# Pointcept/Pointcept

Measured on AMD Instinct MI355X. Metric: scenes/sec (fwd+bwd+optimizer) PTv3 ScanNet-semseg @ ~100k pts, higher is better.
Workload: dtype bf16; 1 GPU; PT-v3m1 base (46.2M params) + seg head + CE + Lovasz, fwd+bwd+AdamW, 8 scenes x 102400 voxels per GPU, patch 1024, 4 orders; global_batch=8, parallelism=dp1, params=46167572, amp=bf16 autocast, points_per_gpu=819200, loss=CrossEntropy(ignore_index=-1) + LovaszSoftmax

## Files before the change

include/ptcore.h:

```cpp
#ifndef PTCORE_H
#define PTCORE_H

#include <stddef.h>
#include <stdint.h>

#ifdef __cplusplus
extern "C" {
#endif

typedef void* ptc_stream_t;

enum ptc_status {
  PTC_OK = 0,
  PTC_EINVAL = -1,
  PTC_EUNSUPPORTED = -2,
  PTC_EHIP = -3,
  PTC_EWORKSPACE = -4
};

enum ptc_dtype { PTC_F32 = 0, PTC_F16 = 1, PTC_BF16 = 2 };

enum ptc_order { PTC_ORDER_Z = 0, PTC_ORDER_Z_TRANS = 1, PTC_ORDER_HILBERT = 2, PTC_ORDER_HILBERT_TRANS = 3 };

enum ptc_reduce { PTC_REDUCE_SUM = 0, PTC_REDUCE_MEAN = 1, PTC_REDUCE_MAX = 2, PTC_REDUCE_MIN = 3 };

const char* ptc_version(void);
const char* ptc_last_error(void);

int ptc_serialize_encode(const void* grid_coord, int coord_is_i64, const int64_t* batch, int64_t n,
                         int depth, const int* orders, int k, int64_t* code_out, ptc_stream_t stream);

size_t ptc_sort_keys_workspace_bytes(int64_t n, int k);
int ptc_sort_keys(const int64_t* keys, int64_t n, int k, int begin_bit, int end_bit, int64_t* order,
                  int64_t* inverse, void* workspace, size_t workspace_bytes, ptc_stream_t stream);

size_t ptc_exclusive_scan_workspace_bytes(int64_t n);
int ptc_exclusive_scan_i32(const int32_t* in, int64_t n, int64_t* out, void* workspace,
                           size_t workspace_bytes, ptc_stream_t stream);

int ptc_patch_pad_maps(const int64_t* offset, int B, int patch, int64_t n, int64_t n_pad,
                       int64_t n_seq, int64_t* pad, int64_t* unpad, int32_t* cu_seqlens,
                       int64_t* dup, ptc_stream_t stream);

int ptc_attn_tables(const int64_t* order, const int64_t* inverse, const int64_t* pad, const int64_t* unpad,
                    const int64_t* dup, int64_t n, int64_t n_pad, int32_t* t_qkv_fwd, int32_t* t_qkv_bwd,
                    int32_t* t_proj_fwd, int32_t* t_proj_bwd, ptc_stream_t stream);

size_t ptc_pool_maps_workspace_bytes(int64_t n);
int ptc_pool_maps_count(const int64_t* code0, const int64_t* order0, int64_t n, int shift,
                        int64_t* cluster, int64_t* n_cluster_out, void* workspace,
                        size_t workspace_bytes, ptc_stream_t stream);
int ptc_pool_maps_fill(const int64_t* order0, const int64_t* cluster, int64_t n, int64_t n_cluster,
                       int64_t* idx_ptr, int64_t* head, ptc_stream_t stream);
int ptc_pool_child_codes(const int64_t* code_in, int64_t n, int k, const int64_t* head,
                         int64_t n_cluster, int shift, int64_t* code_out, ptc_stream_t stream);

int ptc_pool_level_counts(const int64_t* code0, const int64_t* order0, int64_t n, int batch_shift, int n_batch,
                          const int* shifts, int n_levels, int64_t* counts, ptc_stream_t stream);

int ptc_gather_rows(const void* src, int64_t n_src, const int64_t* idx, const int64_t* idx2,
                    int64_t n_out, int c, int dtype, void* out, ptc_stream_t stream);
int ptc_gather_rows_add(const void* src, int64_t n_src, const int64_t* idx, const void* addend, int64_t n_out, int c, int dtype,
                        void* out, ptc_stream_t stream);
int ptc_segment_csr_fwd(const void* src, const int64_t* perm, const int64_t* indptr, int64_t n_seg,
                        int c, int dtype, int reduce, void* out, int32_t* arg_out,
                        ptc_stream_t stream);
int ptc_segment_csr_bwd(const void* grad_out, const int64_t* perm, const int64_t* indptr,
                        const int32_t* arg, int64_t n_seg, int64_t n_src, int c, int dtype,
                        int reduce, void* grad_src, ptc_stream_t stream);

int64_t ptc_hash_table_size(int64_t n);
size_t ptc_hash_table_bytes(int64_t n);
int ptc_hash_build(const int32_t* indices, int64_t n, void* table, size_t table_bytes, ptc_stream_t stream);
int ptc_rulebook_subm(const int32_t* indices, int64_t n, int ksize, const void* table, size_t table_bytes,
                      int32_t* nbr, ptc_stream_t stream);
size_t ptc_rulebook_down_workspace_bytes(int64_t n_in);
int ptc_rulebook_down_count(const int32_t* indices, int64_t n_in, int coord_bits, int batch_bits,
                            int32_t* out_of_in, int64_t* n_out_dev, void* workspace,
                            size_t workspace_bytes, ptc_stream_t stream);
int ptc_rulebook_down_fill(const int32_t* indices, int64_t n_in, const int32_t* out_of_in,
                           int64_t n_out, int32_t* out_indices, int32_t* nbr_down, int32_t* nbr_up,
                           ptc_stream_t stream);

int ptc_spconv_fwd(const void* in, int64_t n_in, const void* weight, const float* bias,
                   const int32_t* nbr, int64_t n_out, int kv, int c_in, int c_out, int dtype,
                   void* out, ptc_stream_t stream);
size_t ptc_rulebook_blocks_tab_bytes(int64_t n);
int ptc_rulebook_blocks(const int32_t* nbr, int kv, int64_t n, int bm, int hcap, void* tab, int32_t* hid,
                        int32_t* hcnt, int32_t* n_overflow, ptc_stream_t stream);
int ptc_spconv_fwd_blk(const void* in, int64_t n_in, const void* weight, const float* bias, const int32_t* nbr,
                       const void* tab, const int32_t* hid, const int32_t* hcnt, int bm, int hcap, int64_t n_out,
                       int kv, int c_in, int c_out, int dtype, void* out, ptc_stream_t stream);
size_t ptc_spconv_wgrad_blk_workspace_bytes(int64_t n_out, int kv, int c_in, int c_out);
int ptc_spconv_wgrad_blk(const void* in, int64_t n_in, const void* dout, const int32_t* nbr, const void* tab, const int32_t* hid,
                         const int32_t* hcnt, const int32_t* n_overflow, int bm, int hcap, int64_t n_out, int kv, int c_in,
                         int c_out, int dtype, float* dw, void* workspace, size_t workspace_bytes, ptc_stream_t stream);
int ptc_linear_supported_ex(int c_in, int c_out, int dtype);
int ptc_linear_fwd_ex(const void* in, int64_t n, const void* weight, const float* bias, int c_in, int c_out, int dtype,
                      int epilogue, const void* aux_in, void* out, void* aux_out, ptc_stream_t stream);
int ptc_linear_joint_supported(int c_in, int c_out, int dtype);
int ptc_linear_norm_joint_fwd(const void* in, int64_t n_in, const void* weight, const float* bias, int64_t n_out, int c_in, int c_out, int dtype,
                              const float* gA, const float* bA, float epsA, const void* a, int a_dtype, const float* gB, const float* bB, float epsB,
                              int normB, void* u_out, float* z, void* y, float* statA, float* statB, ptc_stream_t stream);
int ptc_linear_joint_fwd(const void* in, int64_t n_in, const void* weight, const float* bias, const int32_t* nbr, int64_t n_out, int c_in,
                         int c_out, int dtype, const float* a, const float* row_scale, const float* gB, const float* bB, float epsB,
                         int normB, float* z, void* y, float* statB, ptc_stream_t stream);

int ptc_mlp_supported(int c, int dtype);
int ptc_mlp_fwd(const void* x, int64_t n, int c, int dtype, const void* w1, const float* b1, const void* w2, const float* b2,
                const float* a, const float* row_scale, float* z, void* y, ptc_stream_t stream);
size_t ptc_mlp_bwd_workspace_bytes(int64_t n, int c);
int ptc_mlp_bwd(const void* dm, const void* x, int64_t n, int c, int dtype, const void* w1, const float* b1, const void* w2t, void* dx,
                float* dw1, float* db1, float* dw2, float* db2, void* workspace, size_t workspace_bytes, ptc_stream_t stream);

size_t ptc_spconv_wgrad_workspace_bytes(int64_t n_out, int kv, int c_in, int c_out);
int ptc_spconv_wgrad(const void* in, int64_t n_in, const void* dout, const int32_t* nbr,
                     int64_t n_out, int kv, int c_in, int c_out, int dtype, float* dw, float* dbias,
                     void* workspace, size_t workspace_bytes, ptc_stream_t stream);

int ptc_seg_eval_hist(const void* logits, int dtype, int64_t row_stride, int c, const int64_t* pred, const int64_t* inverse,
                      const int64_t* target, int64_t m, int64_t n_rows, int k, int64_t ignore_index, int64_t* hist3k,
                      ptc_stream_t stream);

int ptc_rope3d(void* tokens, int dtype, const int64_t* positions, int64_t n_tokens, int H, int D, float base, float fwd,
               ptc_stream_t stream);

int ptc_rope3d_xyz(const void* src, int src_dtype, void* dst, int dst_dtype, const float* xyz, const float* inv_freq,
                   int64_t n_tokens, int slabs, int rot_slabs, int H, int D, float sign, ptc_stream_t stream);

int ptc_layer_norm_supported(int c);
int ptc_layer_norm_fwd(const void* x, int64_t n, int c, int in_dtype, const float* gamma,
                       const float* beta, float eps, void* y, int out_dtype, float* mean, float* rstd,
                       ptc_stream_t stream);
size_t ptc_layer_norm_bwd_workspace_bytes(int64_t n, int c);
int ptc_layer_norm_bwd(const void* dy, int dy_dtype, const void* x, int x_dtype, const float* mean,
                       const float* rstd, const float* gamma, int64_t n, int c, void* dx,
                       float* dgamma, float* dbeta, void* workspace, size_t workspace_bytes,
                       ptc_stream_t stream);

int ptc_add_norm_fwd(const void* u, int u_dtype, const void* a, int a_dtype, const float* row_scale, int64_t n, int c,
                     const float* gA, const float* bA, float epsA, int normA, const float* gB,
                     const float* bB, float epsB, int normB, float* z, void* y, int y_dtype,
                     float* statA, float* statB, ptc_stream_t stream);
size_t ptc_add_norm_bwd_workspace_bytes(int64_t n, int c);
int ptc_add_norm_bwd(const float* dz_in, const void* dy, int dy_dtype, const float* z, const void* u,
                     int u_dtype, const float* row_scale, int64_t n, int c, const float* gA,
                     const float* statA, int normA, const float* gB, const float* statB, int normB,
                     void* da, int da_dtype, void* du, float* dgA, float* dbA, float* dgB, float* dbB,
                     void* workspace, size_t workspace_bytes, ptc_stream_t stream);

int ptc_attn_varlen_fwd(const void* qkv, const int32_t* cu_seqlens, int64_t n_seq, int64_t total,
                        int H, int max_seqlen, float softmax_scale, int dtype, void* out,
                        float* lse, ptc_stream_t stream);
size_t ptc_attn_varlen_bwd_workspace_bytes(int64_t total, int H);
int ptc_attn_varlen_bwd(const void* qkv, const void* out, const void* dout, const float* lse,
                        const int32_t* cu_seqlens, int64_t n_seq, int64_t total, int H,
                        int max_seqlen, float softmax_scale, int dtype, void* dqkv,
                        void* workspace, size_t workspace_bytes, ptc_stream_t stream);

int ptc_attn_varlen_dropout_fwd(const void* qkv, const int32_t* cu_seqlens, int64_t n_seq, int64_t total, int H, int max_seqlen,
                                float softmax_scale, int dtype, float dropout_p, uint64_t seed, void* out, float* lse,
                                ptc_stream_t stream);
int ptc_attn_varlen_dropout_bwd(const void* qkv, const void* out, const void* dout, const float* lse, const int32_t* cu_seqlens,
                                int64_t n_seq, int64_t total, int H, int max_seqlen, float softmax_scale, int dtype,
                                float dropout_p, uint64_t seed, void* dqkv, void* workspace, size_t workspace_bytes,
                                ptc_stream_t stream);

int ptc_attn_varlen_hd_supported(int head_dim, int max_seqlen);
int ptc_attn_varlen_hd_fwd(const void* qkv, const int32_t* cu_seqlens, int64_t n_seq, int64_t total,
                           int H, int head_dim, int max_seqlen, float softmax_scale, int dtype,
                           void* out, float* lse, ptc_stream_t stream);
int ptc_attn_varlen_hd_bwd(const void* qkv, const void* out, const void* dout, const float* lse,
                           const int32_t* cu_seqlens, int64_t n_seq, int64_t total, int H,
                           int head_dim, int max_seqlen, float softmax_scale, int dtype, void* dqkv,
                           void* workspace, size_t workspace_bytes, ptc_stream_t stream);
int ptc_attn_varlen_hd_rope_supported(int head_dim, int max_seqlen);
int ptc_attn_varlen_hd_rope_fwd(const void* qkv, const int32_t* cu_seqlens, const float* xyz, const float* inv_freq, int64_t n_seq,
                                int64_t total, int H, int head_dim, int max_seqlen, float softmax_scale, int dtype, void* out, float* lse,
                                ptc_stream_t stream);
int ptc_attn_varlen_hd_rope_bwd(const void* qkv, const void* out, const void* dout, const float* lse, const int32_t* cu_seqlens,
                                const float* xyz, const float* inv_freq, int64_t n_seq, int64_t total, int H, int head_dim, int max_seqlen,
                                float softmax_scale, int dtype, void* dqkv, void* workspace, size_t workspace_bytes, ptc_stream_t stream);


int ptc_attn_rpe_fwd(const void* qkv, const int32_t* cu_seqlens, const int32_t* grid_coord,
                     const float* rpe_table, int pos_bnd, int64_t n_seq, int64_t total, int H,
                     int max_seqlen, float softmax_scale, int dtype, void* out, float* lse,
                     ptc_stream_t stream);
size_t ptc_attn_rpe_bwd_workspace_bytes(int64_t total, int H, int pos_bnd);
int ptc_attn_rpe_bwd(const void* qkv, const void* out, const void* dout, const float* lse,
                     const int32_t* cu_seqlens, const int32_t* grid_coord, const float* rpe_table,
                     int pos_bnd, int64_t n_seq, int64_t total, int H, int max_seqlen,
                     float softmax_scale, int dtype, void* dqkv, float* d_rpe_table, void* workspace,
                     size_t workspace_bytes, ptc_stream_t stream);

int ptc_coord_max(const void* grid_coord, int coord_is_i64, int64_t n, int64_t* out3, ptc_stream_t stream);
int64_t ptc_cross_entropy_partials(int64_t n);
int ptc_cross_entropy_fwd(const void* logits, int64_t row_stride, const int64_t* target, int64_t n, int c, int dtype,
                          int64_t ignore_index, float* lse, float* partial, ptc_stream_t stream);
int ptc_cross_entropy_bwd(const void* logits, int64_t row_stride, const int64_t* target, const float* lse,
                          const float* scale, int64_t n, int c, int dtype, int64_t ignore_index, void* dlogits,
                          int64_t drow_stride, ptc_stream_t stream);

size_t ptc_lovasz_softmax_workspace_bytes(int64_t n, int c);
int ptc_lovasz_softmax(const void* logits, int64_t row_stride, const int64_t* target, int64_t n, int c, int dtype,
                       int64_t ignore_index, float* loss, float* dlogits, void* workspace, size_t workspace_bytes,
                       ptc_stream_t stream);

int ptc_voxel_keys(const float* coord, int64_t n, double grid_size, int64_t* grid_coord, int64_t* min_coord3,
                   int64_t* key, ptc_stream_t stream);

int ptc_knn_query(const float* xyz, const int32_t* offset, const float* new_xyz, const int32_t* new_offset, int b,
                  int64_t n, int64_t m, int nsample, int32_t* idx, float* dist, ptc_stream_t stream);
int ptc_farthest_point_sampling(const float* xyz, const int32_t* offset, const int32_t* new_offset, int b, int64_t n,
                                float* tmp, int32_t* idx, ptc_stream_t stream);
int ptc_ball_query(const float* xyz, const int32_t* offset, const float* new_xyz, const int32_t* new_offset, const int32_t* order,
                   int b, int64_t n, int64_t m, int nsample, float min_radius, float max_radius, int32_t* idx, float* dist2,
                   ptc_stream_t stream);
int ptc_edge_rows_fwd(int mode, const float* src, const float* a, const int32_t* idx, int64_t n_edges, int nsample, int c,
                      int64_t n_src, float* out, int64_t out_stride, int out_col0, ptc_stream_t stream);
int ptc_edge_reduce_fwd(int mode, const float* src, const float* pos, int64_t pos_stride, int pos_col0, const float* w,
                        const int32_t* idx, int64_t m, int nsample, int c, int w_c, int64_t n_src, float* out, ptc_stream_t stream);
int ptc_edge_csr_keys(const int32_t* idx, int64_t n_edges, int64_t n_src, int64_t* keys, ptc_stream_t stream);
int ptc_edge_csr_ptr(const int64_t* keys, const int64_t* order, int64_t n_edges, int64_t n_src, int64_t* indptr, ptc_stream_t stream);
int ptc_edge_scatter_bwd(int mode, const int64_t* order, const int64_t* indptr, const float* g, int64_t g_stride, int g_col0,
                         const float* w, int nsample, int c, int w_c, int64_t n_src, float* grad_src, ptc_stream_t stream);
int ptc_aggregation_edge_bwd(const float* src, const float* pos, const float* w, const int32_t* idx, const float* g, int64_t m,
                             int nsample, int c, int w_c, int64_t n_src, float* grad_pos, float* grad_w, ptc_stream_t stream);
int ptc_pair_dot_weighted(const float* a, const float* b, const float* w, const int32_t* ia, const int32_t* ib, int64_t m, int64_t n_a,
                          int64_t n_b, int g, int c, float* out, ptc_stream_t stream);
int ptc_pair_segment_sum(const float* s, const float* b, const float* w, const float* self, const int64_t* order, const int64_t* indptr,
                         const int32_t* oidx, int64_t n_rows, int64_t n_b, int g, int c, float* out, float* prod, ptc_stream_t stream);

int ptc_batch_norm_supported(int c, int dtype);
size_t ptc_batch_norm_workspace_bytes(int64_t n, int c);
int ptc_batch_norm_act_fwd(const void* x, int64_t n, int c, int dtype, const float* gamma, const float* beta, float eps,
                           float momentum, int training, float* running_mean, float* running_var, int act, void* y,
                           int y_dtype, float* save_mean, float* save_rstd, void* workspace, size_t workspace_bytes,
                           ptc_stream_t stream);
int ptc_column_sum(const void* x, int64_t n, int c, int dtype, float* out, void* workspace, size_t workspace_bytes,
                   ptc_stream_t stream);
int ptc_batch_norm_act_bwd(const void* dy, int dy_dtype, const void* x, int x_dtype, const float* gamma, const float* beta,
                           const float* save_mean, const float* save_rstd, int64_t n, int c, int training, int act,
                           void* dx, float* dgamma, float* dbeta, void* workspace, size_t workspace_bytes,
                           ptc_stream_t stream);
int ptc_batch_norm_add_act_fwd(const void* x, const void* res, int64_t n, int c, int dtype, const float* gamma, const float* beta, float eps,
                               float momentum, int training, float* running_mean, float* running_var, int act, void* y, int y_dtype,
                               float* save_mean, float* save_rstd, void* workspace, size_t workspace_bytes, ptc_stream_t stream);
int ptc_batch_norm_add_act_bwd(const void* dy, int dy_dtype, const void* x, const void* res, int x_dtype, const float* gamma, const float* beta,
                               const float* save_mean, const float* save_rstd, int64_t n, int c, int training, int act, void* dx, void* dres,
                               float* dgamma, float* dbeta, void* workspace, size_t workspace_bytes, ptc_stream_t stream);

int ptc_weight_layouts(const int64_t* desc, const int64_t* prefix, int n, int64_t total, ptc_stream_t stream);

int ptc_cast_many(const int64_t* desc, const int64_t* prefix, int n, int64_t total_units, int dst_dtype, ptc_stream_t stream);

int ptc_pair_dot_fwd(const float* q, const float* k, const int32_t* i0, const int32_t* i1, const float* table_q,
                     const float* table_k, const int32_t* rel_idx, int with_qk, int64_t M, int H, int d, float* out,
                     ptc_stream_t stream);
int ptc_pair_dot_bwd(const float* grad_out, const float* q, const float* k, const int32_t* i0, const int32_t* offsets,
                     const int32_t* i1, const float* table_q, const float* table_k, const int32_t* rel_idx, int with_qk,
                     int64_t M, int64_t Nq, int64_t Nk, int64_t L, int H, int d, float* dq, float* dk, float* dtable_q,
                     float* dtable_k, ptc_stream_t stream);
int ptc_pair_aggregate_fwd(const float* attn, const float* v, const int32_t* i0, const int32_t* offsets, const int32_t* i1,
                           const float* table_v, const int32_t* rel_idx, int64_t M, int64_t Nq, int H, int d, float* out,
                           ptc_stream_t stream);
int ptc_pair_aggregate_bwd(const float* grad_out, const float* attn, const float* v, const int32_t* i0, const int32_t* i1,
                           const float* table_v, const int32_t* rel_idx, int64_t M, int64_t Nv, int64_t L, int H, int d,
                           float* dattn, float* dv, float* dtable_v, ptc_stream_t stream);

#define PTC_BLK_ABI 2
// ... 107 lines not shown
```

pointcept_amd/_lib.py:

```python
from __future__ import annotations

import ctypes
import os

import torch

HERE = os.path.dirname(os.path.abspath(__file__))
LIB_PATH = os.path.join(HERE, "libptcore.so")
PROBE_PATH = os.path.join(HERE, "libptcore_hostprobe.so")

c_i64, c_int, c_f32, c_size, c_ptr = ctypes.c_int64, ctypes.c_int, ctypes.c_float, ctypes.c_size_t, ctypes.c_void_p

_SIGNATURES = {
    "ptc_version": (ctypes.c_char_p, []),
    "ptc_last_error": (ctypes.c_char_p, []),
    "ptc_serialize_encode": (c_int, [c_ptr, c_int, c_ptr, c_i64, c_int, c_ptr, c_int, c_ptr, c_ptr]),
    "ptc_sort_keys_workspace_bytes": (c_size, [c_i64, c_int]),
    "ptc_sort_keys": (c_int, [c_ptr, c_i64, c_int, c_int, c_int, c_ptr, c_ptr, c_ptr, c_size, c_ptr]),
    "ptc_exclusive_scan_workspace_bytes": (c_size, [c_i64]),
    "ptc_exclusive_scan_i32": (c_int, [c_ptr, c_i64, c_ptr, c_ptr, c_size, c_ptr]),
    "ptc_patch_pad_maps": (c_int, [c_ptr, c_int, c_int, c_i64, c_i64, c_i64, c_ptr, c_ptr, c_ptr, c_ptr, c_ptr]),
    "ptc_attn_tables": (c_int, [c_ptr, c_ptr, c_ptr, c_ptr, c_ptr, c_i64, c_i64, c_ptr, c_ptr, c_ptr, c_ptr, c_ptr]),
    "ptc_pool_maps_workspace_bytes": (c_size, [c_i64]),
    "ptc_pool_maps_count": (c_int, [c_ptr, c_ptr, c_i64, c_int, c_ptr, c_ptr, c_ptr, c_size, c_ptr]),
    "ptc_pool_maps_fill": (c_int, [c_ptr, c_ptr, c_i64, c_i64, c_ptr, c_ptr, c_ptr]),
    "ptc_pool_child_codes": (c_int, [c_ptr, c_i64, c_int, c_ptr, c_i64, c_int, c_ptr, c_ptr]),
    "ptc_pool_level_counts": (c_int, [c_ptr, c_ptr, c_i64, c_int, c_int, c_ptr, c_int, c_ptr, c_ptr]),
    "ptc_gather_rows": (c_int, [c_ptr, c_i64, c_ptr, c_ptr, c_i64, c_int, c_int, c_ptr, c_ptr]),
    "ptc_gather_rows_add": (c_int, [c_ptr, c_i64, c_ptr, c_ptr, c_i64, c_int, c_int, c_ptr, c_ptr]),
    "ptc_segment_csr_fwd": (c_int, [c_ptr, c_ptr, c_ptr, c_i64, c_int, c_int, c_int, c_ptr, c_ptr, c_ptr]),
    "ptc_segment_csr_bwd": (c_int, [c_ptr, c_ptr, c_ptr, c_ptr, c_i64, c_i64, c_int, c_int, c_int, c_ptr, c_ptr]),
    "ptc_hash_table_size": (c_i64, [c_i64]),
    "ptc_hash_table_bytes": (c_size, [c_i64]),
    "ptc_hash_build": (c_int, [c_ptr, c_i64, c_ptr, c_size, c_ptr]),
    "ptc_rulebook_subm": (c_int, [c_ptr, c_i64, c_int, c_ptr, c_size, c_ptr, c_ptr]),
    "ptc_rulebook_down_workspace_bytes": (c_size, [c_i64]),
    "ptc_rulebook_down_count": (c_int, [c_ptr, c_i64, c_int, c_int, c_ptr, c_ptr, c_ptr, c_size, c_ptr]),
    "ptc_rulebook_down_fill": (c_int, [c_ptr, c_i64, c_ptr, c_i64, c_ptr, c_ptr, c_ptr, c_ptr]),
    "ptc_spconv_fwd": (c_int, [c_ptr, c_i64, c_ptr, c_ptr, c_ptr, c_i64, c_int, c_int, c_int, c_int, c_ptr, c_ptr]),
    "ptc_ptv3_block_abi": (c_int, []),
    "ptc_ptv3_block_mlp_fused": (c_int, [c_int, c_int]),
    "ptc_ptv3_block_workspace_bytes": (c_size, [c_i64, c_i64, c_int, c_int]),
    "ptc_ptv3_block_fwd": (c_int, [c_ptr, c_ptr, c_ptr, c_ptr, c_ptr]),
    "ptc_ptv3_block_bwd": (c_int, [c_ptr, c_ptr, c_ptr, c_ptr, c_ptr, c_ptr, c_size, c_ptr]),
    "ptc_rulebook_blocks_tab_bytes": (c_size, [c_i64]),
    "ptc_rulebook_blocks": (c_int, [c_ptr, c_int, c_i64, c_int, c_int, c_ptr, c_ptr, c_ptr, c_ptr, c_ptr]),
    "ptc_spconv_fwd_blk": (c_int, [c_ptr, c_i64, c_ptr, c_ptr, c_ptr, c_ptr, c_ptr, c_ptr, c_int, c_int, c_i64, c_int, c_int, c_int, c_int,
                                   c_ptr, c_ptr]),
    "ptc_spconv_wgrad_blk_workspace_bytes": (c_size, [c_i64, c_int, c_int, c_int]),
    "ptc_spconv_wgrad_blk": (c_int, [c_ptr, c_i64, c_ptr, c_ptr, c_ptr, c_ptr, c_ptr, c_ptr, c_int, c_int, c_i64, c_int, c_int, c_int, c_int,
                                     c_ptr, c_ptr, c_size, c_ptr]),
    "ptc_linear_supported_ex": (c_int, [c_int, c_int, c_int]),
    "ptc_linear_joint_supported": (c_int, [c_int, c_int, c_int]),
    "ptc_linear_norm_joint_fwd": (c_int, [c_ptr, c_i64, c_ptr, c_ptr, c_i64, c_int, c_int, c_int, c_ptr, c_ptr, c_f32, c_ptr, c_int, c_ptr, c_ptr, c_f32, c_int,
                                          c_ptr, c_ptr, c_ptr, c_ptr, c_ptr, c_ptr]),
    "ptc_linear_joint_fwd": (c_int, [c_ptr, c_i64, c_ptr, c_ptr, c_ptr, c_i64, c_int, c_int, c_int, c_ptr, c_ptr, c_ptr, c_ptr, c_f32, c_int,
                                     c_ptr, c_ptr, c_ptr, c_ptr]),
    "ptc_linear_fwd_ex": (c_int, [c_ptr, c_i64, c_ptr, c_ptr, c_int, c_int, c_int, c_int, c_ptr, c_ptr, c_ptr, c_ptr]),
    "ptc_mlp_supported": (c_int, [c_int, c_int]),
    "ptc_mlp_fwd": (c_int, [c_ptr, c_i64, c_int, c_int, c_ptr, c_ptr, c_ptr, c_ptr, c_ptr, c_ptr, c_ptr, c_ptr, c_ptr]),
    "ptc_mlp_bwd_workspace_bytes": (c_size, [c_i64, c_int]),
    "ptc_mlp_bwd": (c_int, [c_ptr, c_ptr, c_i64, c_int, c_int, c_ptr, c_ptr, c_ptr, c_ptr, c_ptr, c_ptr, c_ptr, c_ptr, c_ptr, c_size, c_ptr]),
    "ptc_spconv_wgrad_workspace_bytes": (c_size, [c_i64, c_int, c_int, c_int]),
    "ptc_spconv_wgrad": (c_int, [c_ptr, c_i64, c_ptr, c_ptr, c_i64, c_int, c_int, c_int, c_int, c_ptr, c_ptr, c_ptr, c_size,
                                 c_ptr]),
    "ptc_seg_eval_hist": (c_int, [c_ptr, c_int, c_i64, c_int, c_ptr, c_ptr, c_ptr, c_i64, c_i64, c_int, c_i64, c_ptr, c_ptr]),
    "ptc_rope3d": (c_int, [c_ptr, c_int, c_ptr, c_i64, c_int, c_int, c_f32, c_f32, c_ptr]),
    "ptc_rope3d_xyz": (c_int, [c_ptr, c_int, c_ptr, c_int, c_ptr, c_ptr, c_i64, c_int, c_int, c_int, c_int, c_f32, c_ptr]),
    "ptc_layer_norm_supported": (c_int, [c_int]),
    "ptc_layer_norm_fwd": (c_int, [c_ptr, c_i64, c_int, c_int, c_ptr, c_ptr, c_f32, c_ptr, c_int, c_ptr, c_ptr, c_ptr]),
    "ptc_layer_norm_bwd_workspace_bytes": (c_size, [c_i64, c_int]),
    "ptc_layer_norm_bwd": (c_int, [c_ptr, c_int, c_ptr, c_int, c_ptr, c_ptr, c_ptr, c_i64, c_int, c_ptr, c_ptr, c_ptr, c_ptr,
                                   c_size, c_ptr]),
    "ptc_add_norm_fwd": (c_int, [c_ptr, c_int, c_ptr, c_int, c_ptr, c_i64, c_int, c_ptr, c_ptr, c_f32, c_int, c_ptr, c_ptr, c_f32, c_int,
                                 c_ptr, c_ptr, c_int, c_ptr, c_ptr, c_ptr]),
    "ptc_add_norm_bwd_workspace_bytes": (c_size, [c_i64, c_int]),
    "ptc_add_norm_bwd": (c_int, [c_ptr, c_ptr, c_int, c_ptr, c_ptr, c_int, c_ptr, c_i64, c_int, c_ptr, c_ptr, c_int, c_ptr, c_ptr,
                                 c_int, c_ptr, c_int, c_ptr, c_ptr, c_ptr, c_ptr, c_ptr, c_ptr, c_size, c_ptr]),
    "ptc_attn_varlen_fwd": (c_int, [c_ptr, c_ptr, c_i64, c_i64, c_int, c_int, c_f32, c_int, c_ptr, c_ptr, c_ptr]),
    "ptc_attn_varlen_bwd_workspace_bytes": (c_size, [c_i64, c_int]),
    "ptc_attn_varlen_dropout_fwd": (c_int, [c_ptr, c_ptr, c_i64, c_i64, c_int, c_int, c_f32, c_int, c_f32, ctypes.c_uint64, c_ptr, c_ptr, c_ptr]),
    "ptc_attn_varlen_dropout_bwd": (c_int, [c_ptr, c_ptr, c_ptr, c_ptr, c_ptr, c_i64, c_i64, c_int, c_int, c_f32, c_int, c_f32, ctypes.c_uint64,
                                            c_ptr, c_ptr, c_size, c_ptr]),
    "ptc_attn_varlen_hd_supported": (c_int, [c_int, c_int]),
    "ptc_attn_varlen_hd_rope_supported": (c_int, [c_int, c_int]),
    "ptc_attn_varlen_hd_rope_fwd": (c_int, [c_ptr, c_ptr, c_ptr, c_ptr, c_i64, c_i64, c_int, c_int, c_int, c_f32, c_int, c_ptr, c_ptr, c_ptr]),
    "ptc_attn_varlen_hd_rope_bwd": (c_int, [c_ptr, c_ptr, c_ptr, c_ptr, c_ptr, c_ptr, c_ptr, c_i64, c_i64, c_int, c_int, c_int, c_f32, c_int, c_ptr,
                                            c_ptr, c_size, c_ptr]),
    "ptc_weight_layouts": (c_int, [c_ptr, c_ptr, c_int, c_i64, c_ptr]),
    "ptc_cast_many": (c_int, [c_ptr, c_ptr, c_int, c_i64, c_int, c_ptr]),
    "ptc_pair_dot_fwd": (c_int, [c_ptr, c_ptr, c_ptr, c_ptr, c_ptr, c_ptr, c_ptr, c_int, c_i64, c_int, c_int, c_ptr, c_ptr]),
    "ptc_pair_dot_bwd": (c_int, [c_ptr, c_ptr, c_ptr, c_ptr, c_ptr, c_ptr, c_ptr, c_ptr, c_ptr, c_int, c_i64, c_i64, c_i64, c_i64, c_int,
                                 c_int, c_ptr, c_ptr, c_ptr, c_ptr, c_ptr]),
    "ptc_pair_aggregate_fwd": (c_int, [c_ptr, c_ptr, c_ptr, c_ptr, c_ptr, c_ptr, c_ptr, c_i64, c_i64, c_int, c_int, c_ptr, c_ptr]),
    "ptc_pair_aggregate_bwd": (c_int, [c_ptr, c_ptr, c_ptr, c_ptr, c_ptr, c_ptr, c_ptr, c_i64, c_i64, c_i64, c_int, c_int, c_ptr, c_ptr,
                                       c_ptr, c_ptr]),
    "ptc_attn_rpe_fwd": (c_int, [c_ptr, c_ptr, c_ptr, c_ptr, c_int, c_i64, c_i64, c_int, c_int, c_f32, c_int, c_ptr, c_ptr, c_ptr]),
    "ptc_attn_rpe_bwd_workspace_bytes": (c_size, [c_i64, c_int, c_int]),
    "ptc_attn_rpe_bwd": (c_int, [c_ptr, c_ptr, c_ptr, c_ptr, c_ptr, c_ptr, c_ptr, c_int, c_i64, c_i64, c_int, c_int, c_f32, c_int, c_ptr,
                                 c_ptr, c_ptr, c_size, c_ptr]),
    "ptc_attn_varlen_hd_fwd": (c_int, [c_ptr, c_ptr, c_i64, c_i64, c_int, c_int, c_int, c_f32, c_int, c_ptr, c_ptr, c_ptr]),
    "ptc_attn_varlen_hd_bwd": (c_int, [c_ptr, c_ptr, c_ptr, c_ptr, c_ptr, c_i64, c_i64, c_int, c_int, c_int, c_f32, c_int, c_ptr,
                                       c_ptr, c_size, c_ptr]),
    "ptc_attn_varlen_bwd": (c_int, [c_ptr, c_ptr, c_ptr, c_ptr, c_ptr, c_i64, c_i64, c_int, c_int, c_f32, c_int, c_ptr,
                                    c_ptr, c_size, c_ptr]),
    "ptc_batch_norm_supported": (c_int, [c_int, c_int]),
    "ptc_batch_norm_workspace_bytes": (c_size, [c_i64, c_int]),
    "ptc_batch_norm_act_fwd": (c_int, [c_ptr, c_i64, c_int, c_int, c_ptr, c_ptr, c_f32, c_f32, c_int, c_ptr, c_ptr, c_int, c_ptr, c_int,
                                       c_ptr, c_ptr, c_ptr, c_size, c_ptr]),
    "ptc_batch_norm_act_bwd": (c_int, [c_ptr, c_int, c_ptr, c_int, c_ptr, c_ptr, c_ptr, c_ptr, c_i64, c_int, c_int, c_int, c_ptr, c_ptr,
                                       c_ptr, c_ptr, c_size, c_ptr]),
    "ptc_batch_norm_add_act_fwd": (c_int, [c_ptr, c_ptr, c_i64, c_int, c_int, c_ptr, c_ptr, c_f32, c_f32, c_int, c_ptr, c_ptr, c_int, c_ptr, c_int,
                                           c_ptr, c_ptr, c_ptr, c_size, c_ptr]),
    "ptc_batch_norm_add_act_bwd": (c_int, [c_ptr, c_int, c_ptr, c_ptr, c_int, c_ptr, c_ptr, c_ptr, c_ptr, c_i64, c_int, c_int, c_int, c_ptr, c_ptr,
                                           c_ptr, c_ptr, c_ptr, c_size, c_ptr]),
    "ptc_column_sum": (c_int, [c_ptr, c_i64, c_int, c_int, c_ptr, c_ptr, c_size, c_ptr]),
    "ptc_coord_max": (c_int, [c_ptr, c_int, c_i64, c_ptr, c_ptr]),
    "ptc_cross_entropy_partials": (c_i64, [c_i64]),
    "ptc_cross_entropy_fwd": (c_int, [c_ptr, c_i64, c_ptr, c_i64, c_int, c_int, c_i64, c_ptr, c_ptr, c_ptr]),
    "ptc_cross_entropy_bwd": (c_int, [c_ptr, c_i64, c_ptr, c_ptr, c_ptr, c_i64, c_int, c_int, c_i64, c_ptr, c_i64, c_ptr]),
    "ptc_knn_query": (c_int, [c_ptr, c_ptr, c_ptr, c_ptr, c_int, c_i64, c_i64, c_int, c_ptr, c_ptr, c_ptr]),
    "ptc_ball_query": (c_int, [c_ptr, c_ptr, c_ptr, c_ptr, c_ptr, c_int, c_i64, c_i64, c_int, c_f32, c_f32, c_ptr, c_ptr, c_ptr]),
    "ptc_edge_rows_fwd": (c_int, [c_int, c_ptr, c_ptr, c_ptr, c_i64, c_int, c_int, c_i64, c_ptr, c_i64, c_int, c_ptr]),
    "ptc_edge_reduce_fwd": (c_int, [c_int, c_ptr, c_ptr, c_i64, c_int, c_ptr, c_ptr, c_i64, c_int, c_int, c_int, c_i64, c_ptr, c_ptr]),
    "ptc_edge_csr_keys": (c_int, [c_ptr, c_i64, c_i64, c_ptr, c_ptr]),
    "ptc_edge_csr_ptr": (c_int, [c_ptr, c_ptr, c_i64, c_i64, c_ptr, c_ptr]),
    "ptc_edge_scatter_bwd": (c_int, [c_int, c_ptr, c_ptr, c_ptr, c_i64, c_int, c_ptr, c_int, c_int, c_int, c_i64, c_ptr, c_ptr]),
    "ptc_pair_dot_weighted": (c_int, [c_ptr, c_ptr, c_ptr, c_ptr, c_ptr, c_i64, c_i64, c_i64, c_int, c_int, c_ptr, c_ptr]),
    "ptc_pair_segment_sum": (c_int, [c_ptr, c_ptr, c_ptr, c_ptr, c_ptr, c_ptr, c_ptr, c_i64, c_i64, c_int, c_int, c_ptr, c_ptr, c_ptr]),
    "ptc_aggregation_edge_bwd": (c_int, [c_ptr, c_ptr, c_ptr, c_ptr, c_ptr, c_i64, c_int, c_int, c_int, c_i64, c_ptr, c_ptr, c_ptr]),
    "ptc_farthest_point_sampling": (c_int, [c_ptr, c_ptr, c_ptr, c_int, c_i64, c_ptr, c_ptr, c_ptr]),
    "ptc_voxel_keys": (c_int, [c_ptr, c_i64, ctypes.c_double, c_ptr, c_ptr, c_ptr, c_ptr]),
    "ptc_grid_cluster_workspace_bytes": (c_size, [c_i64, c_int]),
    "ptc_grid_cluster_count": (c_int, [c_ptr, c_i64, c_ptr, c_int, c_ptr, c_int, c_ptr, c_ptr, c_ptr, c_ptr, c_size, c_ptr]),
    "ptc_cluster_center": (c_int, [c_ptr, c_ptr, c_ptr, c_ptr, c_int, c_i64, c_int, c_int, c_ptr, c_ptr]),
    "ptc_cluster_agg_state_bytes": (c_size, [c_i64, c_int]),
    "ptc_cluster_agg_workspace_bytes": (c_size, [c_i64]),
    "ptc_cluster_agg_fwd": (c_int, [c_ptr, c_ptr, c_ptr, c_ptr, c_ptr, c_ptr, c_ptr, c_int, c_i64, c_int, c_int, c_ptr, c_ptr, c_size,
                                    c_ptr]),
    "ptc_cluster_agg_bwd": (c_int, [c_ptr, c_ptr, c_ptr, c_ptr, c_ptr, c_ptr, c_ptr, c_ptr, c_int, c_i64, c_int, c_int, c_ptr, c_size,
                                    c_ptr, c_ptr, c_ptr, c_ptr, c_size, c_ptr]),
    "ptc_pg_ball_query_workspace_bytes": (c_size, [c_i64]),
    "ptc_pg_ball_query_count": (c_int, [c_ptr, c_ptr, c_i64, c_int, c_f32, c_ptr, c_ptr, c_ptr, c_size, c_ptr]),
    "ptc_pg_ball_query_fill": (c_int, [c_ptr, c_i64, c_f32, c_ptr, c_ptr, c_ptr, c_size, c_ptr]),
    "ptc_pg_cluster_workspace_bytes": (c_size, [c_i64]),
    "ptc_pg_cluster_count": (c_int, [c_ptr, c_ptr, c_ptr, c_i64, c_int, c_int, c_ptr, c_ptr, c_size, c_ptr]),
    "ptc_pg_cluster_fill": (c_int, [c_i64, c_i64, c_i64, c_ptr, c_ptr, c_ptr, c_size, c_ptr]),
    "ptc_pg_proposal_scores": (c_int, [c_ptr, c_int, c_i64, c_int, c_ptr, c_ptr, c_ptr, c_i64, c_ptr, c_ptr, c_ptr, c_ptr, c_ptr]),
    "ptc_pg_proposal_masks": (c_int, [c_ptr, c_i64, c_ptr, c_ptr, c_i64, c_i64, c_ptr, c_ptr]),
    "ptc_pg_bias_loss_workspace_bytes": (c_size, [c_i64]),
    "ptc_pg_bias_loss_fwd": (c_int, [c_ptr, c_int, c_ptr, c_ptr, c_ptr, c_i64, c_i64, c_ptr, c_ptr, c_size, c_ptr]),
    "ptc_pg_bias_loss_bwd": (c_int, [c_ptr, c_int, c_ptr, c_ptr, c_ptr, c_i64, c_i64, c_ptr, c_ptr, c_ptr, c_ptr]),
    "ptc_msc_match_workspace_bytes": (c_size, [c_i64]),
    "ptc_msc_match": (c_int, [c_ptr, c_ptr, c_ptr, c_ptr, c_int, c_i64, c_i64, c_int, c_f32, c_ptr, c_ptr, c_ptr, c_ptr, c_size, c_ptr]),
    "ptc_msc_select_workspace_bytes": (c_size, [c_i64]),
    "ptc_msc_select": (c_int, [c_ptr, c_ptr, c_i64, c_int, c_ptr, c_i64, c_ptr, c_ptr, c_size, c_ptr]),
    "ptc_msc_patch_workspace_bytes": (c_size, [c_i64]),
    "ptc_msc_patch_rank": (c_int, [c_ptr, c_ptr, c_i64, c_ptr, c_ptr, c_i64, c_int, c_ptr, c_ptr, c_ptr, c_size, c_ptr]),
    "ptc_msc_patch_masks": (c_int, [c_ptr, c_ptr, c_i64, c_i64, c_i64, c_ptr, c_ptr, c_ptr]),
    "ptc_msc_nce_workspace_bytes": (c_size, [c_i64, c_int]),
    "ptc_msc_nce_fwd": (c_int, [c_ptr, c_i64, c_ptr, c_i64, c_ptr, c_i64, c_int, c_f32, c_ptr, c_ptr, c_ptr, c_ptr, c_ptr, c_ptr, c_ptr,
                                c_size, c_ptr]),
    "ptc_msc_nce_bwd": (c_int, [c_ptr, c_ptr, c_ptr, c_ptr, c_ptr, c_ptr, c_i64, c_int, c_i64, c_i64, c_f32, c_ptr, c_ptr, c_ptr, c_ptr,
                                c_size, c_ptr]),
    "ptc_cac_supported": (c_int, [c_int, c_int]),
    "ptc_cac_pool_workspace_bytes": (c_size, [c_i64, c_int, c_int, c_int]),
    "ptc_cac_pool_fwd": (c_int, [c_ptr, c_ptr, c_ptr, c_ptr, c_i64, c_int, c_int, c_int, c_f32, c_f32, c_ptr, c_ptr, c_ptr, c_ptr, c_ptr, c_size,
                                 c_ptr]),
    "ptc_cac_pool_bwd": (c_int, [c_ptr, c_ptr, c_ptr, c_ptr, c_i64, c_int, c_int, c_int, c_f32, c_f32, c_ptr, c_ptr, c_ptr, c_ptr, c_ptr, c_ptr]),
    "ptc_cac_cos_workspace_bytes": (c_size, [c_i64, c_int, c_int, c_int]),
    "ptc_cac_cos_fwd": (c_int, [c_ptr, c_ptr, c_ptr, c_i64, c_int, c_int, c_int, c_f32, c_ptr, c_ptr, c_size, c_ptr]),
    "ptc_cac_cos_bwd": (c_int, [c_ptr, c_ptr, c_ptr, c_i64, c_int, c_int, c_int, c_f32, c_ptr, c_ptr, c_ptr, c_ptr, c_size, c_ptr]),
    "ptc_cac_distill_workspace_bytes": (c_size, [c_i64, c_int]),
    "ptc_cac_distill_fwd": (c_int, [c_ptr, c_ptr, c_ptr, c_i64, c_int, c_f32, c_f32, c_ptr, c_ptr, c_ptr, c_size, c_ptr]),
    "ptc_cac_distill_bwd": (c_int, [c_ptr, c_ptr, c_ptr, c_i64, c_int, c_f32, c_f32, c_ptr, c_ptr, c_ptr, c_ptr]),
    "ptc_lovasz_softmax_workspace_bytes": (c_size, [c_i64, c_int]),
    "ptc_lovasz_softmax": (c_int, [c_ptr, c_i64, c_ptr, c_i64, c_int, c_int, c_i64, c_ptr, c_ptr, c_ptr, c_size, c_ptr]),
}

PTC_F32, PTC_F16, PTC_BF16 = 0, 1, 2
REDUCE_CODES = {"sum": 0, "mean": 1, "max": 2, "min": 3}
ORDER_CODES = {"z": 0, "z-trans": 1, "hilbert": 2, "hilbert-trans": 3}

_lib = None


class PtcoreError(RuntimeError):
    pass


def exported_symbols():
    return sorted(_SIGNATURES)


def lib():
    global _lib
    if _lib is not None:
        return _lib
    from . import build as _build

    variant = os.environ.get("PTC_LIB_VARIANT", "")
    LIB_PATH = _build.build(variant=variant)
    try:
        L = ctypes.CDLL(LIB_PATH)
    except OSError as e:
        raise PtcoreError(f"cannot load {LIB_PATH}: {e}") from e
    for name, (res, args) in _SIGNATURES.items():
        fn = getattr(L, name)
        fn.restype = res
        fn.argtypes = args
    ver = L.ptc_version().decode()
    hdr = os.path.join(HERE, "..", "include", "ptcore.h")
    if os.path.exists(hdr) and "abi " in ver:
        import zlib

        want = f"{zlib.crc32(open(hdr, 'rb').read()) & 0xffffffff:08x}"
# ... 85 lines not shown
```

pointcept_amd/csrc/block_exec.hip:

```cpp
#include "ptc_common.h"
#ifndef PTC_BLK_JOINT_EPILOGUE
#define PTC_BLK_JOINT_EPILOGUE 1
#endif
#include "spconv_internal.h"

#define RUN(call)               \
  do {                          \
    const int rc__ = (call);    \
    if (rc__ != PTC_OK) return rc__; \
  } while (0)

static inline const void* P(const void* const* p, int i) { return p[i]; }
template <typename T> static inline T* M(void* const* p, int i) { return (T*)p[i]; }

extern "C" int ptc_ptv3_block_abi(void) { return PTC_BLK_ABI; }

extern "C" int ptc_ptv3_block_mlp_fused(int c, int dtype) {
  static const int off = [] { const char* e = getenv("PTC_BLK_MLP_FUSED"); return e && e[0] == '0'; }();
  return !off && ptc_mlp_supported(c, dtype);
}

struct BlkWs { size_t common; size_t wg[6]; size_t off[6]; size_t total; };
static BlkWs blk_ws(int64_t n, int64_t n_pad, int c, int heads) {
  const int hid = 4 * c;
  BlkWs w;
  w.common = 256;
  auto up = [&](size_t v) { if (v > w.common) w.common = v; };
  up(ptc_add_norm_bwd_workspace_bytes(n, c));
  up(ptc_attn_varlen_bwd_workspace_bytes(n_pad, heads));
  up(ptc_batch_norm_workspace_bytes(n, c));
  w.common = ptc_align_up(w.common, 256);
  w.wg[0] = ptc_spconv_wgrad_workspace_bytes(n, 1, hid, c);
  if (ptc_mlp_supported(c, PTC_BF16) && ptc_mlp_bwd_workspace_bytes(n, c) > w.wg[0]) w.wg[0] = ptc_mlp_bwd_workspace_bytes(n, c);
  w.wg[1] = ptc_spconv_wgrad_workspace_bytes(n, 1, c, hid);
  w.wg[2] = ptc_spconv_wgrad_workspace_bytes(n, 1, c, c);
  w.wg[3] = ptc_spconv_wgrad_workspace_bytes(n_pad, 1, c, 3 * c);
  w.wg[4] = ptc_spconv_wgrad_workspace_bytes(n, 1, c, c);
  w.wg[5] = ptc_spconv_wgrad_blk_workspace_bytes(n, 27, c, c);
  size_t o = w.common;
  for (int i = 0; i < 6; ++i) { w.off[i] = o; o += ptc_align_up(w.wg[i], 256); }
  w.total = o;
  return w;
}

extern "C" size_t ptc_ptv3_block_workspace_bytes(int64_t n, int64_t n_pad, int c, int heads) { return blk_ws(n, n_pad, c, heads).total; }

extern "C" int ptc_ptv3_block_fwd(const int64_t* iv, const float* fv, const void* const* in, void* const* out, ptc_stream_t s) {
  PTC_REQUIRE(iv && fv && in && out, PTC_EINVAL, "ptc_ptv3_block_fwd: null argument table");
  PTC_REQUIRE(iv[PTC_BLK_I_ABI] == PTC_BLK_ABI, PTC_EINVAL, "ptc_ptv3_block_fwd: argument tables of another ABI revision");
  const int64_t n = iv[PTC_BLK_I_N], np = iv[PTC_BLK_I_NPAD], n_seq = iv[PTC_BLK_I_NSEQ];
  const int c = (int)iv[PTC_BLK_I_C], H = (int)iv[PTC_BLK_I_HEADS], dt = (int)iv[PTC_BLK_I_DTYPE], hid = 4 * c;
  const int a_dt = (int)iv[PTC_BLK_I_A_DTYPE], patch = (int)iv[PTC_BLK_I_PATCH];
  PTC_REQUIRE(dt == PTC_BF16 || dt == PTC_F16, PTC_EUNSUPPORTED, "ptc_ptv3_block_fwd: 16-bit GEMM operands only");
  PTC_REQUIRE(c % 16 == 0 && H * 16 == c && (c <= 256 || (c <= 512 && ptc_linear_supported_ex(c, hid, dt))), PTC_EUNSUPPORTED,
              "ptc_ptv3_block_fwd: c=%d heads=%d (head_dim 16, c <= 256, or <= 512 with the wide GEMM kernels)", c, H);
  if (n == 0) return PTC_OK;
  const int32_t* nbr = (const int32_t*)P(in, PTC_BLK_P_NBR);
  RUN(ptc_spconv_fwd_blk(P(in, PTC_BLK_P_XC), n, P(in, PTC_BLK_P_W_CONV), (const float*)P(in, PTC_BLK_P_B_CONV), nbr, P(in, PTC_BLK_P_BLK_TAB),
                         (const int32_t*)P(in, PTC_BLK_P_BLK_HID), (const int32_t*)P(in, PTC_BLK_P_BLK_HCNT), (int)iv[PTC_BLK_I_BLK_BM],
                         (int)iv[PTC_BLK_I_BLK_HCAP], n, 27, c, c, dt, out[PTC_BLK_O_CONV], s));
  if (PTC_BLK_JOINT_EPILOGUE && ptc_linear_joint_supported(c, c, dt)) {
    RUN(ptc_linear_norm_joint_fwd(out[PTC_BLK_O_CONV], n, P(in, PTC_BLK_P_W_LIN), (const float*)P(in, PTC_BLK_P_B_LIN), n, c, c, dt,
                                  (const float*)P(in, PTC_BLK_P_G_CPE), (const float*)P(in, PTC_BLK_P_BE_CPE), fv[PTC_BLK_F_EPS_CPE], P(in, PTC_BLK_P_X0), a_dt,
                                  (const float*)P(in, PTC_BLK_P_G_N1), (const float*)P(in, PTC_BLK_P_BE_N1), fv[PTC_BLK_F_EPS_N1], 1, out[PTC_BLK_O_LIN],
                                  M<float>(out, PTC_BLK_O_X1), out[PTC_BLK_O_Y1], M<float>(out, PTC_BLK_O_ST_CPE), M<float>(out, PTC_BLK_O_ST_N1), s));
  } else {
  RUN(ptc_spconv_fwd(out[PTC_BLK_O_CONV], n, P(in, PTC_BLK_P_W_LIN), (const float*)P(in, PTC_BLK_P_B_LIN), nullptr, n, 1, c, c, dt, out[PTC_BLK_O_LIN], s));
  RUN(ptc_add_norm_fwd(out[PTC_BLK_O_LIN], dt, P(in, PTC_BLK_P_X0), a_dt, nullptr, n, c, (const float*)P(in, PTC_BLK_P_G_CPE),
                       (const float*)P(in, PTC_BLK_P_BE_CPE), fv[PTC_BLK_F_EPS_CPE], 1, (const float*)P(in, PTC_BLK_P_G_N1),
                       (const float*)P(in, PTC_BLK_P_BE_N1), fv[PTC_BLK_F_EPS_N1], 1, M<float>(out, PTC_BLK_O_X1), out[PTC_BLK_O_Y1], dt,
                       M<float>(out, PTC_BLK_O_ST_CPE), M<float>(out, PTC_BLK_O_ST_N1), s));
  }
  RUN(ptc_spconv_fwd(out[PTC_BLK_O_Y1], n, P(in, PTC_BLK_P_W_QKV), (const float*)P(in, PTC_BLK_P_B_QKV), (const int32_t*)P(in, PTC_BLK_P_T_QKV_FWD), np, 1, c,
                     3 * c, dt, out[PTC_BLK_O_QKV], s));
  RUN(ptc_attn_varlen_fwd(out[PTC_BLK_O_QKV], (const int32_t*)P(in, PTC_BLK_P_CU), n_seq, np, H, patch, fv[PTC_BLK_F_SCALE], dt, out[PTC_BLK_O_ATT],
                          M<float>(out, PTC_BLK_O_LSE), s));
  if (PTC_BLK_JOINT_EPILOGUE && ptc_linear_joint_supported(c, c, dt)) {
    RUN(ptc_linear_joint_fwd(out[PTC_BLK_O_ATT], np, P(in, PTC_BLK_P_W_PROJ), (const float*)P(in, PTC_BLK_P_B_PROJ), (const int32_t*)P(in, PTC_BLK_P_T_PROJ_FWD),
                             n, c, c, dt, M<float>(out, PTC_BLK_O_X1), (const float*)P(in, PTC_BLK_P_RS1), (const float*)P(in, PTC_BLK_P_G_N2),
                             (const float*)P(in, PTC_BLK_P_BE_N2), fv[PTC_BLK_F_EPS_N2], 1, M<float>(out, PTC_BLK_O_X2), out[PTC_BLK_O_Y2],
                             M<float>(out, PTC_BLK_O_ST_N2), s));
  } else {
    RUN(ptc_spconv_fwd(out[PTC_BLK_O_ATT], np, P(in, PTC_BLK_P_W_PROJ), (const float*)P(in, PTC_BLK_P_B_PROJ), (const int32_t*)P(in, PTC_BLK_P_T_PROJ_FWD), n, 1,
                       c, c, dt, out[PTC_BLK_O_A], s));
    RUN(ptc_add_norm_fwd(out[PTC_BLK_O_A], dt, out[PTC_BLK_O_X1], PTC_F32, (const float*)P(in, PTC_BLK_P_RS1), n, c, nullptr, nullptr, 0.f, 0,
                         (const float*)P(in, PTC_BLK_P_G_N2), (const float*)P(in, PTC_BLK_P_BE_N2), fv[PTC_BLK_F_EPS_N2], 1, M<float>(out, PTC_BLK_O_X2),
                         out[PTC_BLK_O_Y2], dt, nullptr, M<float>(out, PTC_BLK_O_ST_N2), s));
  }
  if (ptc_ptv3_block_mlp_fused(c, dt))
    return ptc_mlp_fwd(out[PTC_BLK_O_Y2], n, c, dt, P(in, PTC_BLK_P_W_FC1), (const float*)P(in, PTC_BLK_P_B_FC1), P(in, PTC_BLK_P_W_FC2),
                       (const float*)P(in, PTC_BLK_P_B_FC2), M<float>(out, PTC_BLK_O_X2), (const float*)P(in, PTC_BLK_P_RS2), M<float>(out, PTC_BLK_O_X3),
                       out[PTC_BLK_O_XB3], s);
  RUN(ptc_linear_fwd_ex(out[PTC_BLK_O_Y2], n, P(in, PTC_BLK_P_W_FC1), (const float*)P(in, PTC_BLK_P_B_FC1), c, hid, dt, 1, nullptr, out[PTC_BLK_O_H],
                        out[PTC_BLK_O_ACT], s));
  if (PTC_BLK_JOINT_EPILOGUE && ptc_linear_joint_supported(hid, c, dt)) {
    RUN(ptc_linear_joint_fwd(out[PTC_BLK_O_ACT], n, P(in, PTC_BLK_P_W_FC2), (const float*)P(in, PTC_BLK_P_B_FC2), nullptr, n, hid, c, dt,
                             M<float>(out, PTC_BLK_O_X2), (const float*)P(in, PTC_BLK_P_RS2), nullptr, nullptr, 0.f, 0, M<float>(out, PTC_BLK_O_X3),
                             out[PTC_BLK_O_XB3], nullptr, s));
  } else {
    RUN(ptc_spconv_fwd(out[PTC_BLK_O_ACT], n, P(in, PTC_BLK_P_W_FC2), (const float*)P(in, PTC_BLK_P_B_FC2), nullptr, n, 1, hid, c, dt, out[PTC_BLK_O_M], s));
    RUN(ptc_add_norm_fwd(out[PTC_BLK_O_M], dt, out[PTC_BLK_O_X2], PTC_F32, (const float*)P(in, PTC_BLK_P_RS2), n, c, nullptr, nullptr, 0.f, 0, nullptr,
                         nullptr, 0.f, 0, M<float>(out, PTC_BLK_O_X3), out[PTC_BLK_O_XB3], dt, nullptr, nullptr, s));
  }
  return PTC_OK;
}

extern "C" int ptc_ptv3_block_bwd(const int64_t* iv, const float* fv, const void* const* in, const void* const* sv, void* const* g,
                                  void* workspace, size_t workspace_bytes, ptc_stream_t s) {
  PTC_REQUIRE(iv && fv && in && sv && g && workspace, PTC_EINVAL, "ptc_ptv3_block_bwd: null argument table");
  PTC_REQUIRE(iv[PTC_BLK_I_ABI] == PTC_BLK_ABI, PTC_EINVAL, "ptc_ptv3_block_bwd: argument tables of another ABI revision");
  const int64_t n = iv[PTC_BLK_I_N], np = iv[PTC_BLK_I_NPAD], n_seq = iv[PTC_BLK_I_NSEQ];
  const int c = (int)iv[PTC_BLK_I_C], H = (int)iv[PTC_BLK_I_HEADS], dt = (int)iv[PTC_BLK_I_DTYPE], hid = 4 * c;
  const int a_dt = (int)iv[PTC_BLK_I_A_DTYPE], patch = (int)iv[PTC_BLK_I_PATCH];
  PTC_REQUIRE(workspace_bytes >= ptc_ptv3_block_workspace_bytes(n, np, c, H), PTC_EWORKSPACE, "ptc_ptv3_block_bwd: workspace too small");
  if (n == 0) return PTC_OK;
  const int32_t* nbr = (const int32_t*)P(in, PTC_BLK_P_NBR);
  const float* rs1 = (const float*)P(in, PTC_BLK_P_RS1);
  const float* rs2 = (const float*)P(in, PTC_BLK_P_RS2);
  const BlkWs W = blk_ws(n, np, c, H);
  void* ws = workspace;
  const size_t wb = W.common;
  PtcWgradJob jobs[6];
  PtcWgradCall calls[5];
  auto wgws = [&](int i) { return (void*)((char*)workspace + W.off[i]); };
  RUN(ptc_add_norm_bwd((const float*)P(in, PTC_BLK_P_DZ3), P(in, PTC_BLK_P_DYB3), dt, (const float*)P(sv, PTC_BLK_O_X3), P(sv, PTC_BLK_O_M), dt, rs2, n, c,
                       nullptr, nullptr, 0, nullptr, nullptr, 0, g[PTC_BLK_S_DX2], PTC_F32, g[PTC_BLK_S_DM], nullptr, nullptr, nullptr, nullptr, ws, wb, s));
  const bool mlp_fused = ptc_ptv3_block_mlp_fused(c, dt) != 0;
  if (mlp_fused) {
    RUN(ptc_mlp_bwd_deferred(g[PTC_BLK_S_DM], P(sv, PTC_BLK_O_Y2), n, c, dt, P(in, PTC_BLK_P_W_FC1), (const float*)P(in, PTC_BLK_P_B_FC1),
                             P(in, PTC_BLK_P_WT_FC2), g[PTC_BLK_S_DY2], M<float>(g, PTC_BLK_G_W_FC1), M<float>(g, PTC_BLK_G_B_FC1),
                             M<float>(g, PTC_BLK_G_W_FC2), M<float>(g, PTC_BLK_G_B_FC2), wgws(0), W.wg[0], s, &jobs[1], &jobs[0]));
  } else {
  calls[0] = PtcWgradCall{P(sv, PTC_BLK_O_ACT), n, g[PTC_BLK_S_DM], nullptr, n, 1, hid, c, dt, M<float>(g, PTC_BLK_G_W_FC2), M<float>(g, PTC_BLK_G_B_FC2), wgws(0), W.wg[0]};
  RUN(ptc_linear_fwd_ex(g[PTC_BLK_S_DM], n, P(in, PTC_BLK_P_WT_FC2), nullptr, c, hid, dt, 2, P(sv, PTC_BLK_O_H), g[PTC_BLK_S_DH], nullptr, s));
  calls[1] = PtcWgradCall{P(sv, PTC_BLK_O_Y2), n, g[PTC_BLK_S_DH], nullptr, n, 1, c, hid, dt, M<float>(g, PTC_BLK_G_W_FC1), M<float>(g, PTC_BLK_G_B_FC1), wgws(1), W.wg[1]};
  RUN(ptc_spconv_fwd(g[PTC_BLK_S_DH], n, P(in, PTC_BLK_P_WT_FC1), nullptr, nullptr, n, 1, hid, c, dt, g[PTC_BLK_S_DY2], s));
  }
  RUN(ptc_add_norm_bwd(M<float>(g, PTC_BLK_S_DX2), g[PTC_BLK_S_DY2], dt, (const float*)P(sv, PTC_BLK_O_X2), P(sv, PTC_BLK_O_A), dt, rs1, n, c, nullptr, nullptr, 0,
                       (const float*)P(in, PTC_BLK_P_G_N2), (const float*)P(sv, PTC_BLK_O_ST_N2), 1, g[PTC_BLK_S_DX1], PTC_F32, g[PTC_BLK_S_DA], nullptr, nullptr,
                       M<float>(g, PTC_BLK_G_G_N2), M<float>(g, PTC_BLK_G_BE_N2), ws, wb, s));
  calls[2] = PtcWgradCall{P(sv, PTC_BLK_O_ATT), np, g[PTC_BLK_S_DA], (const int32_t*)P(in, PTC_BLK_P_T_PROJ_FWD), n, 1, c, c, dt, M<float>(g, PTC_BLK_G_W_PROJ),
                          M<float>(g, PTC_BLK_G_B_PROJ), wgws(2), W.wg[2]};
  RUN(ptc_spconv_fwd(g[PTC_BLK_S_DA], n, P(in, PTC_BLK_P_WT_PROJ), nullptr, (const int32_t*)P(in, PTC_BLK_P_T_PROJ_BWD), np, 1, c, c, dt, g[PTC_BLK_S_DATT], s));
  RUN(ptc_attn_varlen_bwd(P(sv, PTC_BLK_O_QKV), P(sv, PTC_BLK_O_ATT), g[PTC_BLK_S_DATT], (const float*)P(sv, PTC_BLK_O_LSE), (const int32_t*)P(in, PTC_BLK_P_CU), n_seq,
                          np, H, patch, fv[PTC_BLK_F_SCALE], dt, g[PTC_BLK_S_DQKV], ws, wb, s));
  calls[3] = PtcWgradCall{P(sv, PTC_BLK_O_Y1), n, g[PTC_BLK_S_DQKV], (const int32_t*)P(in, PTC_BLK_P_T_QKV_FWD), np, 1, c, 3 * c, dt, M<float>(g, PTC_BLK_G_W_QKV),
                          M<float>(g, PTC_BLK_G_B_QKV), wgws(3), W.wg[3]};
  RUN(ptc_spconv_fwd(g[PTC_BLK_S_DQKV], np, P(in, PTC_BLK_P_WT_QKV), nullptr, (const int32_t*)P(in, PTC_BLK_P_T_QKV_BWD), n, 2, 3 * c, c, dt, g[PTC_BLK_S_DY1], s));
  RUN(ptc_add_norm_bwd(M<float>(g, PTC_BLK_S_DX1), g[PTC_BLK_S_DY1], dt, (const float*)P(sv, PTC_BLK_O_X1), P(sv, PTC_BLK_O_LIN), dt, nullptr, n, c,
                       (const float*)P(in, PTC_BLK_P_G_CPE), (const float*)P(sv, PTC_BLK_O_ST_CPE), 1, (const float*)P(in, PTC_BLK_P_G_N1),
                       (const float*)P(sv, PTC_BLK_O_ST_N1), 1, g[PTC_BLK_G_X0], a_dt, g[PTC_BLK_S_DLIN], M<float>(g, PTC_BLK_G_G_CPE), M<float>(g, PTC_BLK_G_BE_CPE),
                       M<float>(g, PTC_BLK_G_G_N1), M<float>(g, PTC_BLK_G_BE_N1), ws, wb, s));
  calls[4] = PtcWgradCall{P(sv, PTC_BLK_O_CONV), n, g[PTC_BLK_S_DLIN], nullptr, n, 1, c, c, dt, M<float>(g, PTC_BLK_G_W_LIN), M<float>(g, PTC_BLK_G_B_LIN), wgws(4), W.wg[4]};
  RUN(ptc_spconv_fwd(g[PTC_BLK_S_DLIN], n, P(in, PTC_BLK_P_WT_LIN), nullptr, nullptr, n, 1, c, c, dt, g[PTC_BLK_S_DCONV], s));
  RUN(ptc_spconv_wgrad_blk_deferred(P(in, PTC_BLK_P_XC), n, g[PTC_BLK_S_DCONV], nbr, P(in, PTC_BLK_P_BLK_TAB), (const int32_t*)P(in, PTC_BLK_P_BLK_HID),
                                    (const int32_t*)P(in, PTC_BLK_P_BLK_HCNT), (const int32_t*)P(in, PTC_BLK_P_BLK_NOVF), (int)iv[PTC_BLK_I_BLK_BM],
                                    (int)iv[PTC_BLK_I_BLK_HCAP], n, 27, c, c, dt, M<float>(g, PTC_BLK_G_W_CONV), wgws(5), W.wg[5], s, &jobs[5]));
  RUN(ptc_column_sum(g[PTC_BLK_S_DCONV], n, c, dt, M<float>(g, PTC_BLK_G_B_CONV), ws, wb, s));
  RUN(ptc_spconv_fwd_blk(g[PTC_BLK_S_DCONV], n, P(in, PTC_BLK_P_WT_CONV), nullptr, nbr, P(in, PTC_BLK_P_BLK_TAB), (const int32_t*)P(in, PTC_BLK_P_BLK_HID),
                         (const int32_t*)P(in, PTC_BLK_P_BLK_HCNT), (int)iv[PTC_BLK_I_BLK_BM], (int)iv[PTC_BLK_I_BLK_HCAP], n, 27, c, c, dt, g[PTC_BLK_G_XC], s));
  if (mlp_fused) RUN(ptc_spconv_wgrad_group(calls + 2, 3, jobs + 2, s));
  else RUN(ptc_spconv_wgrad_group(calls, 5, jobs, s));
  RUN(ptc_wgrad_reduce_jobs(jobs, 6, s));
  return PTC_OK;
}
```

pointcept_amd/csrc/spconv.hip:

```cpp
#include "ptc_common.h"
#include "spconv_internal.h"

#include "mma.h"
#include "wgrad2.h"

#define SC_ROWS 128
#define SC_LDS_BYTES 34816

template <int NTILES> struct TileGroups {
  static __host__ __device__ constexpr int gsize(int t) { return (NTILES - (t & ~3)) >= 4 ? 4 : (((NTILES & 3) - ((t & 3) & ~1)) >= 2 ? 2 : 1); }
  static __host__ __device__ constexpr int gstart(int t) { return (NTILES - (t & ~3)) >= 4 ? (t & ~3) : (((NTILES & 3) - ((t & 3) & ~1)) >= 2 ? ((t & ~3) + ((t & 3) & ~1)) : t); }
};

template <int NTILES>
__device__ __forceinline__ int lds_row_of_channel(int n) {
  const int t0 = n >> 4;
  const int gs = TileGroups<NTILES>::gstart(t0), G = TileGroups<NTILES>::gsize(t0);
  const int local = n - 16 * gs;
  const int gq = local / (4 * G), rem = local - gq * 4 * G;
  const int tt = rem >> 2, e = rem & 3;
  return 16 * (gs + tt) + 4 * gq + e;
}

template <int NTILES>
// ... 243 lines not shown
}
extern "C" int ptc_linear_norm_joint_fwd(const void* in, int64_t n_in, const void* weight, const float* bias, int64_t n_out, int c_in, int c_out, int dtype,
                                         const float* gA, const float* bA, float epsA, const void* a, int a_dtype, const float* gB, const float* bB, float epsB,
                                         int normB, void* u_out, float* z, void* y, float* statA, float* statB, ptc_stream_t stream) {
  PTC_REQUIRE(n_out == 0 || (u_out && statA), PTC_EINVAL, "ptc_linear_norm_joint_fwd: null buffer");
  PTC_REQUIRE((uintptr_t)u_out % 16 == 0, PTC_EINVAL, "ptc_linear_norm_joint_fwd: buffers must be 16-byte aligned");
  PTC_REQUIRE(a_dtype == PTC_F32 || a_dtype == PTC_BF16 || a_dtype == PTC_F16, PTC_EINVAL, "ptc_linear_norm_joint_fwd: a_dtype %d", a_dtype);
  const F2Joint J{(const float*)a, nullptr, gB, bB, epsB, normB, z, y, statB, gA, bA, epsA, 1, statA, u_out, a_dtype == PTC_BF16 ? 1 : (a_dtype == PTC_F16 ? 2 : 0)};
  return linear_joint_impl(in, n_in, weight, bias, nullptr, n_out, c_in, c_out, dtype, J, stream);
}
static int linear_joint_impl(const void* in, int64_t n_in, const void* weight, const float* bias, const int32_t* nbr, int64_t n_out, int c_in, int c_out,
                             int dtype, const F2Joint& J, ptc_stream_t stream) {
  const float* a = J.a;
  float* z = J.z;
  void* y = J.y;
  const int normB = J.normB;
  float* statB = J.statB;
  PTC_REQUIRE(n_out >= 0 && n_in >= 0 && linear_joint_supported(dtype, c_in, c_out), PTC_EUNSUPPORTED,
              "ptc_linear_joint_fwd: c_in=%d c_out=%d dtype=%d", c_in, c_out, dtype);
  PTC_REQUIRE((uint64_t)n_in * (uint64_t)c_in * 2 <= PTC_BUF_MAX_BYTES, PTC_EUNSUPPORTED, "ptc_linear_joint_fwd: input of 2 GiB or more");
  if (n_out == 0) return PTC_OK;
  PTC_REQUIRE(in && weight && a && z, PTC_EINVAL, "ptc_linear_joint_fwd: null buffer");
  PTC_REQUIRE(!(normB && y) || statB, PTC_EINVAL, "ptc_linear_joint_fwd: missing statistics buffer");
  PTC_REQUIRE(((uintptr_t)in % 16 == 0) && ((uintptr_t)weight % 16 == 0) && ((uintptr_t)a % 16 == 0) && ((uintptr_t)z % 16 == 0) &&
              ((uintptr_t)y % 16 == 0), PTC_EINVAL, "ptc_linear_joint_fwd: buffers must be 16-byte aligned");
  hipStream_t s = (hipStream_t)stream;
#define LJ_DISPATCH(T)                                                                             \
  if (c_out == 32) return launch_linear_joint<T, 2>(in, n_in, weight, bias, nbr, n_out, c_in, J, s);  \
  if (c_out == 64) return launch_linear_joint<T, 4>(in, n_in, weight, bias, nbr, n_out, c_in, J, s);  \
  return launch_linear_joint<T, 8>(in, n_in, weight, bias, nbr, n_out, c_in, J, s);
  if (dtype == PTC_BF16) { LJ_DISPATCH(bf16_t) }
  LJ_DISPATCH(f16_t)
#undef LJ_DISPATCH
}

#define WG_RO 64
#define WG_CT 64

template <typename T>
__global__ void __launch_bounds__(256)
spconv_wgrad_kernel(const T* __restrict__ in, const T* __restrict__ dout, const int32_t* __restrict__ nbr,
                    int64_t n_out, int kv, int c_in, int c_out, int64_t rows_per_split, int ci_tiles,
                    float* __restrict__ partial, float* __restrict__ bias_partial) {
  using M = Mma<T>;
  constexpr int EPL = M::EPL, KS = M::KS;
  constexpr int PITCH = WG_RO + EPL;
  __shared__ __attribute__((aligned(16))) unsigned char smem[2 * WG_CT * (WG_RO + 8) * 4];
  T* dT = reinterpret_cast<T*>(smem);
  T* iT = dT + WG_CT * PITCH;

  const int lane = ptc_lane(), wave = threadIdx.x >> 6;
  const int r = lane & 15, g = lane >> 4;
  const int k = blockIdx.y;
  const int co0 = (blockIdx.z / ci_tiles) * WG_CT, ci0 = (blockIdx.z % ci_tiles) * WG_CT;
  const int64_t begin = (int64_t)blockIdx.x * rows_per_split;
  int64_t end = begin + rows_per_split;
  if (end > n_out) end = n_out;

  f32x4 acc[4];
#pragma unroll
  for (int t = 0; t < 4; ++t) acc[t] = (f32x4){0.f, 0.f, 0.f, 0.f};
  const bool do_bias = bias_partial != nullptr && k == 0 && (blockIdx.z % ci_tiles) == 0;
  f32x4 acc_b = (f32x4){0.f, 0.f, 0.f, 0.f};
  typename M::frag ones;
#pragma unroll
  for (int e = 0; e < EPL; ++e) {
    if (sizeof(T) == 4) reinterpret_cast<float*>(&ones)[e] = 1.0f;
    else if (std::is_same<T, bf16_t>::value) reinterpret_cast<uint16_t*>(&ones)[e] = 0x3F80;
    else reinterpret_cast<uint16_t*>(&ones)[e] = 0x3C00;
  }

  for (int64_t chunk = begin; chunk < end; chunk += WG_RO) {
    __syncthreads();
    if (sizeof(T) == 2) {
      const int p = threadIdx.x & 31, cv = threadIdx.x >> 5;
      const int64_t ra = chunk + 2 * p, rb = ra + 1;
      uint4 da = {0, 0, 0, 0}, db = {0, 0, 0, 0}, xa = {0, 0, 0, 0}, xb = {0, 0, 0, 0};
      const bool cov = (co0 + cv * 8) < c_out, civ = (ci0 + cv * 8) < c_in;
      if (ra < end) {
        if (cov) da = *reinterpret_cast<const uint4*>(dout + ra * c_out + co0 + cv * 8);
        const int32_t j = nbr ? nbr[(int64_t)k * n_out + ra] : (int32_t)ra;
        if (civ && j >= 0) xa = *reinterpret_cast<const uint4*>(in + (int64_t)j * c_in + ci0 + cv * 8);
      }
      if (rb < end) {
        if (cov) db = *reinterpret_cast<const uint4*>(dout + rb * c_out + co0 + cv * 8);
        const int32_t j = nbr ? nbr[(int64_t)k * n_out + rb] : (int32_t)rb;
        if (civ && j >= 0) xb = *reinterpret_cast<const uint4*>(in + (int64_t)j * c_in + ci0 + cv * 8);
      }
      const uint16_t* pa = reinterpret_cast<const uint16_t*>(&da);
      const uint16_t* pb = reinterpret_cast<const uint16_t*>(&db);
      const uint16_t* qa = reinterpret_cast<const uint16_t*>(&xa);
      const uint16_t* qb = reinterpret_cast<const uint16_t*>(&xb);
      uint32_t* d32 = reinterpret_cast<uint32_t*>(dT);
      uint32_t* i32 = reinterpret_cast<uint32_t*>(iT);
#pragma unroll
      for (int e = 0; e < 8; ++e) {
        d32[((cv * 8 + e) * PITCH) / 2 + p] = (uint32_t)pa[e] | ((uint32_t)pb[e] << 16);
        i32[((cv * 8 + e) * PITCH) / 2 + p] = (uint32_t)qa[e] | ((uint32_t)qb[e] << 16);
      }
    } else {
      const int rr = threadIdx.x & 63;
      const int64_t row = chunk + rr;
      const int32_t j = row < end ? (nbr ? nbr[(int64_t)k * n_out + row] : (int32_t)row) : -1;
#pragma unroll
      for (int pass = 0; pass < 4; ++pass) {
        const int cv = (threadIdx.x >> 6) + pass * 4;
        float4 d = {0.f, 0.f, 0.f, 0.f}, x = {0.f, 0.f, 0.f, 0.f};
        if (row < end && (co0 + cv * 4) < c_out)
          d = *reinterpret_cast<const float4*>(reinterpret_cast<const float*>(dout) + row * c_out + co0 + cv * 4);
        if (j >= 0 && (ci0 + cv * 4) < c_in)
          x = *reinterpret_cast<const float4*>(reinterpret_cast<const float*>(in) + (int64_t)j * c_in + ci0 + cv * 4);
        float* df = reinterpret_cast<float*>(dT);
        float* xf = reinterpret_cast<float*>(iT);
        df[(cv * 4 + 0) * PITCH + rr] = d.x; df[(cv * 4 + 1) * PITCH + rr] = d.y;
        df[(cv * 4 + 2) * PITCH + rr] = d.z; df[(cv * 4 + 3) * PITCH + rr] = d.w;
        xf[(cv * 4 + 0) * PITCH + rr] = x.x; xf[(cv * 4 + 1) * PITCH + rr] = x.y;
        xf[(cv * 4 + 2) * PITCH + rr] = x.z; xf[(cv * 4 + 3) * PITCH + rr] = x.w;
      }
    }
    __syncthreads();
#pragma unroll
    for (int ks = 0; ks < WG_RO / KS; ++ks) {
      const int kk = ks * KS + g * EPL;
      const typename M::frag fa = ld_frag<T>(dT + (wave * 16 + r) * PITCH + kk);
      if (do_bias) acc_b = M::mma(fa, ones, acc_b);
#pragma unroll
      for (int t = 0; t < 4; ++t) {
        const typename M::frag fb = ld_frag<T>(iT + (t * 16 + r) * PITCH + kk);
        acc[t] = M::mma(fa, fb, acc[t]);
      }
    }
  }
  if (do_bias && r == 0) {
#pragma unroll
    for (int e = 0; e < 4; ++e) {
      const int co = co0 + wave * 16 + g * 4 + e;
      if (co < c_out) bias_partial[(int64_t)blockIdx.x * c_out + co] = acc_b[e];
    }
  }
  float* pout = partial + (int64_t)blockIdx.x * c_out * kv * c_in;
#pragma unroll
  for (int t = 0; t < 4; ++t) {
    const int ci = ci0 + t * 16 + r;
    if (ci >= c_in) continue;
#pragma unroll
    for (int e = 0; e < 4; ++e) {
      const int co = co0 + wave * 16 + g * 4 + e;
      if (co < c_out) pout[((int64_t)co * kv + k) * c_in + ci] = acc[t][e];
    }
  }
}

#define WG_REDUCE_FEW 8
__device__ __forceinline__ void wgrad_reduce_body(const float* __restrict__ partial, int splits, int64_t count, float* __restrict__ dw, int nb1,
                                                  const float* __restrict__ partial2, int64_t count2, float* __restrict__ out2, int bid, bool few) {
  __shared__ float4 red[16][16];
  if (few && bid < nb1) {
    const int64_t i = (int64_t)bid * 1024 + (int64_t)threadIdx.x * 4;
    if (i >= count) return;
    if ((i + 3 < count) && ((count & 3) == 0)) {
      float4 a = *reinterpret_cast<const float4*>(partial + i);
      for (int p = 1; p < splits; ++p) {
        const float4 v = *reinterpret_cast<const float4*>(partial + (int64_t)p * count + i);
        a.x += v.x; a.y += v.y; a.z += v.z; a.w += v.w;
      }
      *reinterpret_cast<float4*>(dw + i) = a;
    } else {
      for (int64_t j = i; j < count && j < i + 4; ++j) {
        float a = partial[j];
        for (int p = 1; p < splits; ++p) a += partial[(int64_t)p * count + j];
        dw[j] = a;
      }
    }
    return;
  }
  if (bid >= nb1) {
    partial = partial2; count = count2; dw = out2;
  }
  const int64_t blk = bid >= nb1 ? (int64_t)bid - nb1 : (int64_t)bid;
  const int lane = threadIdx.x & 15, pg = threadIdx.x >> 4;
  const int64_t i = blk * 64 + lane * 4;
  float4 acc[4];
#pragma unroll
  for (int u = 0; u < 4; ++u) acc[u] = make_float4(0.f, 0.f, 0.f, 0.f);
  if (i < count) {
    const bool vec = (i + 3 < count) && ((count & 3) == 0);
    for (int p0 = pg; p0 < splits; p0 += 64) {
      if (vec) {
        float4 v[4];
#pragma unroll
        for (int u = 0; u < 4; ++u) {
          const int p = p0 + 16 * u;
          v[u] = *reinterpret_cast<const float4*>(partial + (int64_t)(p < splits ? p : splits - 1) * count + i);
        }
#pragma unroll
        for (int u = 0; u < 4; ++u) {
          const bool live = p0 + 16 * u < splits;
          acc[u].x += live ? v[u].x : 0.f; acc[u].y += live ? v[u].y : 0.f; acc[u].z += live ? v[u].z : 0.f; acc[u].w += live ? v[u].w : 0.f;
        }
      } else {
#pragma unroll
        for (int u = 0; u < 4; ++u) {
          const int p = p0 + 16 * u;
          if (p < splits) {
            const float* src = partial + (int64_t)p * count + i;
            acc[u].x += src[0];
            acc[u].y += i + 1 < count ? src[1] : 0.f;
            acc[u].z += i + 2 < count ? src[2] : 0.f;
            acc[u].w += i + 3 < count ? src[3] : 0.f;
          }
        }
      }
    }
  }
  float4 t;
  t.x = (acc[0].x + acc[1].x) + (acc[2].x + acc[3].x);
  t.y = (acc[0].y + acc[1].y) + (acc[2].y + acc[3].y);
  t.z = (acc[0].z + acc[1].z) + (acc[2].z + acc[3].z);
  t.w = (acc[0].w + acc[1].w) + (acc[2].w + acc[3].w);
  red[pg][lane] = t;
  __syncthreads();
  if (pg == 0 && i < count) {
    float4 r = red[0][lane];
#pragma unroll
    for (int q = 1; q < 16; ++q) {
      const float4 v = red[q][lane];
      r.x += v.x; r.y += v.y; r.z += v.z; r.w += v.w;
    }
    dw[i] = r.x;
    if (i + 1 < count) dw[i + 1] = r.y;
    if (i + 2 < count) dw[i + 2] = r.z;
    if (i + 3 < count) dw[i + 3] = r.w;
  }
}

__global__ void __launch_bounds__(256)
wgrad_reduce_kernel(const float* __restrict__ partial, int splits, int64_t count, float* __restrict__ dw, int nb1,
                    const float* __restrict__ partial2, int64_t count2, float* __restrict__ out2, int few) {
  wgrad_reduce_body(partial, splits, count, dw, nb1, partial2, count2, out2, (int)blockIdx.x, few != 0);
}

struct WgradReduceMulti {
  int n;
  int start[PTC_WGRAD_JOBS_MAX + 1];
  int nb1[PTC_WGRAD_JOBS_MAX];
  int few[PTC_WGRAD_JOBS_MAX];
  PtcWgradJob job[PTC_WGRAD_JOBS_MAX];
};
__global__ void __launch_bounds__(256)
wgrad_reduce_multi_kernel(WgradReduceMulti m) {
  int j = 0;
#pragma unroll
  for (int q = 1; q < PTC_WGRAD_JOBS_MAX; ++q)
    if (q < m.n && (int)blockIdx.x >= m.start[q]) j = q;
  const PtcWgradJob& J = m.job[j];
  const bool alt = J.gate != nullptr && *J.gate != 0;
  wgrad_reduce_body(alt ? J.alt_partial : J.partial, alt ? J.alt_splits : J.splits, J.count, J.dw, m.nb1[j], J.bias_partial, J.c_out, J.dbias,
                    (int)blockIdx.x - m.start[j], m.few[j] != 0);
}

int ptc_wgrad_reduce_jobs(const PtcWgradJob* jobs, int n, ptc_stream_t stream) {
  PTC_REQUIRE(jobs && n >= 0 && n <= PTC_WGRAD_JOBS_MAX, PTC_EINVAL, "ptc_wgrad_reduce_jobs: %d jobs", n);
  WgradReduceMulti m;
  m.n = 0;
  int grid = 0;
  for (int q = 0; q < n; ++q) {
    if (jobs[q].splits <= 0) continue;
    const bool few = jobs[q].splits <= WG_REDUCE_FEW && (jobs[q].gate == nullptr || jobs[q].alt_splits <= WG_REDUCE_FEW);
    const int nb1 = (int)ptc_cdiv(jobs[q].count, few ? 1024 : 64), nb2 = jobs[q].dbias ? (int)ptc_cdiv(jobs[q].c_out, 64) : 0;
    m.start[m.n] = grid;
    m.nb1[m.n] = nb1;
    m.few[m.n] = few ? 1 : 0;
    m.job[m.n] = jobs[q];
    grid += nb1 + nb2;
    ++m.n;
  }
  if (m.n == 0) return PTC_OK;
  for (int q = m.n; q <= PTC_WGRAD_JOBS_MAX; ++q) m.start[q] = grid;
  hipLaunchKernelGGL(wgrad_reduce_multi_kernel, dim3((unsigned)grid), dim3(256), 0, (hipStream_t)stream, m);
  PTC_CHECK_LAUNCH("wgrad_reduce_multi_kernel");
  return PTC_OK;
}

static int launch_wgrad_reduce(const float* partial, int splits, int64_t count, float* dw, const float* bias_partial, int64_t c_out,
                               float* dbias, hipStream_t s) {
  const bool few = splits <= WG_REDUCE_FEW;
  const int nb1 = (int)ptc_cdiv(count, few ? 1024 : 64);
  const int nb2 = dbias ? (int)ptc_cdiv(c_out, 64) : 0;
  hipLaunchKernelGGL(wgrad_reduce_kernel, dim3((unsigned)(nb1 + nb2)), dim3(256), 0, s, partial, splits, count, dw, nb1, bias_partial,
                     c_out, dbias, few ? 1 : 0);
  PTC_CHECK_LAUNCH("wgrad_reduce_kernel");
  return PTC_OK;
}

static int wgrad_splits(int64_t n_out, int kv, int c_in, int c_out) {
  const int64_t tiles = ptc_cdiv(c_out, WG_CT) * ptc_cdiv(c_in, WG_CT);
  int64_t s = 2048 / (kv * tiles);
  const int64_t max_s = ptc_cdiv(n_out, 4 * WG_RO);
  if (s > max_s) s = max_s;
  if (s < 1) s = 1;
  if (s > 256) s = 256;
  return (int)s;
}

extern "C" size_t ptc_spconv_wgrad_workspace_bytes(int64_t n_out, int kv, int c_in, int c_out) {
  size_t splits = (size_t)wgrad_splits(n_out, kv, c_in, c_out);
  size_t gx = (size_t)w2_plan(n_out, kv, c_in, c_out, false).gx;
  const size_t gxb = (size_t)w2_plan(n_out, kv, c_in, c_out, true).gx;
  if (gxb > gx) gx = gxb;
  if (gx > splits) splits = gx;
  if (ptc_wgrad3_supported(PTC_BF16, kv, c_in, c_out, n_out)) {
    int s3, cps;
    ptc_wgrad3_plan(n_out, c_in, c_out, &s3, &cps);
    if ((size_t)s3 > splits) splits = (size_t)s3;
  }
  return ptc_align_up(splits * (size_t)c_out * kv * c_in * sizeof(float), 256) + ptc_align_up(splits * (size_t)c_out * sizeof(float), 256);
}

static size_t wgrad_blk_extra_bytes(int64_t n_out, int kv, int c_in, int c_out) {
  if (!wgrad7_supported(PTC_BF16, kv, c_in, c_out, C7_BM, C7_HCAP, n_out)) return 0;
  return ptc_align_up((size_t)wgrad7_splits(n_out, c_in, c_out) * (size_t)c_out * kv * c_in * sizeof(float), 256);
}
extern "C" size_t ptc_spconv_wgrad_blk_workspace_bytes(int64_t n_out, int kv, int c_in, int c_out) {
  return ptc_spconv_wgrad_workspace_bytes(n_out, kv, c_in, c_out) + wgrad_blk_extra_bytes(n_out, kv, c_in, c_out);
}

template <typename T>
static int launch_wgrad(const void* in, const void* dout, const int32_t* nbr, int64_t n_out, int kv, int c_in,
                        int c_out, float* dw, float* dbias, void* ws, hipStream_t s) {
  const int splits = wgrad_splits(n_out, kv, c_in, c_out);
  float* bias_partial = dbias ? (float*)((char*)ws + ptc_align_up((size_t)splits * (size_t)c_out * kv * c_in * sizeof(float), 256)) : nullptr;
  const int ci_tiles = (int)ptc_cdiv(c_in, WG_CT), co_tiles = (int)ptc_cdiv(c_out, WG_CT);
  int64_t rps = ptc_cdiv(ptc_cdiv(n_out, splits), WG_RO) * WG_RO;
  dim3 grid((unsigned)splits, (unsigned)kv, (unsigned)(ci_tiles * co_tiles));
  hipLaunchKernelGGL((spconv_wgrad_kernel<T>), grid, dim3(256), 0, s, (const T*)in, (const T*)dout, nbr, n_out, kv,
                     c_in, c_out, rps, ci_tiles, splits > 1 ? (float*)ws : dw, bias_partial);
  PTC_CHECK_LAUNCH("spconv_wgrad_kernel");
  const int64_t count = (int64_t)c_out * kv * c_in;
  if (splits > 1) return launch_wgrad_reduce((const float*)ws, splits, count, dw, bias_partial, c_out, dbias, s);
  if (dbias) {
    hipLaunchKernelGGL(wgrad_reduce_kernel, dim3((unsigned)ptc_cdiv(c_out, 64)), dim3(256), 0, s, (const float*)bias_partial, splits,
                       (int64_t)c_out, dbias, 1 << 30, (const float*)nullptr, (int64_t)0, (float*)nullptr, 0);
    PTC_CHECK_LAUNCH("wgrad_reduce_kernel(bias)");
  }
  return PTC_OK;
}

template <typename T, int COT, int CIT, int KG>
static int launch_wgrad2_inst(const W2Plan& p, const void* in, int64_t n_in, const void* dout, const int32_t* nbr, int64_t n_out, int kv,
                              int c_in, int c_out, float* partial, float* bias_partial, hipStream_t s, const int32_t* gate = nullptr) {
  auto kern = wgrad2_kernel<T, COT, CIT, KG>;
  if (p.lds > 48 * 1024)
    PTC_HIP(hipFuncSetAttribute(reinterpret_cast<const void*>(kern), hipFuncAttributeMaxDynamicSharedMemorySize, (int)p.lds));
  const int nblocks = p.co_blocks * p.ci_blocks, total = p.gx * p.groups * nblocks;
  hipLaunchKernelGGL(kern, dim3((unsigned)(8 * ((total + 7) / 8))), dim3(256), p.lds, s, (const T*)in, (const T*)dout, nbr, n_out, kv,
                     c_in, c_out, ptc_cdiv(n_out, W2_ROWS), p.ci_blocks, partial, bias_partial, p.gx, p.groups, nblocks,
                     (uint32_t)((uint64_t)n_in * c_in * sizeof(T)), (uint32_t)((uint64_t)n_out * c_out * sizeof(T)), gate);
  PTC_CHECK_LAUNCH("wgrad2_kernel");
  return PTC_OK;
}

template <typename T>
static int launch_wgrad2(const void* in, int64_t n_in, const void* dout, const int32_t* nbr, int64_t n_out, int kv, int c_in, int c_out,
                         float* dw, float* dbias, void* ws, hipStream_t s, PtcWgradJob* defer = nullptr, const int32_t* gate = nullptr) {
  const W2Plan p = w2_plan(n_out, kv, c_in, c_out, dbias != nullptr);
  const int64_t count = (int64_t)c_out * kv * c_in;
  float* partial = (p.gx > 1 || gate) ? (float*)ws : dw;
  float* bias_partial = nullptr;
  if (dbias) bias_partial = p.gx > 1 ? (float*)((char*)ws + ptc_align_up((size_t)p.gx * (size_t)count * sizeof(float), 256)) : dbias;
  int rc = PTC_EUNSUPPORTED;
#define W2_CASE(COT, CIT, KG)                                                                                         \
  if (p.cot == COT && p.cit == CIT && p.kg == KG)                                                                     \
    rc = launch_wgrad2_inst<T, COT, CIT, KG>(p, in, n_in, dout, nbr, n_out, kv, c_in, c_out, partial, bias_partial, s, gate);
  W2_CASE(2, 1, 1) W2_CASE(2, 2, 1) W2_CASE(2, 4, 1) W2_CASE(4, 1, 1) W2_CASE(4, 2, 1) W2_CASE(4, 4, 1)
  W2_CASE(6, 1, 1) W2_CASE(6, 2, 1) W2_CASE(6, 4, 1) W2_CASE(8, 1, 1) W2_CASE(8, 2, 1)
  W2_CASE(2, 1, 8) W2_CASE(2, 2, 4) W2_CASE(4, 2, 4) W2_CASE(2, 4, 4) W2_CASE(4, 4, 2) W2_CASE(6, 2, 2)
#undef W2_CASE
  if (rc != PTC_OK) {
    if (rc == PTC_EUNSUPPORTED) ptc_set_error("ptc_spconv_wgrad: no wgrad2 instance for tiles (%d,%d,%d)", p.cot, p.cit, p.kg);
    return rc;
  }
  if (defer) {
    *defer = PtcWgradJob{partial, (p.gx > 1 || gate) ? p.gx : 0, count, dw, bias_partial, (int64_t)c_out, dbias};
    return PTC_OK;
  }
  if (p.gx > 1) return launch_wgrad_reduce(partial, p.gx, count, dw, bias_partial, c_out, dbias, s);
  return PTC_OK;
}

static int spconv_wgrad_impl(const void* in, int64_t n_in, const void* dout, const int32_t* nbr, int64_t n_out, int kv, int c_in, int c_out,
                             int dtype, float* dw, float* dbias, void* workspace, size_t workspace_bytes, ptc_stream_t stream, PtcWgradJob* defer);

static bool wgrad3_eligible(const void* in, int64_t n_in, const void* dout, const int32_t* nbr, int64_t n_out, int kv, int c_in, int c_out, int dtype,
                            const float* dw, const void* workspace, size_t workspace_bytes) {
  return n_out > 0 && in && dout && dw && workspace && (dtype == PTC_BF16 || dtype == PTC_F16) && ptc_wgrad3_supported(dtype, kv, c_in, c_out, n_out) &&
         (nbr || n_in >= n_out) && (uint64_t)n_in * c_in * 2 <= PTC_BUF_MAX_BYTES && (uint64_t)n_out * c_out * 2 <= PTC_BUF_MAX_BYTES &&
         ((uintptr_t)in % 16 == 0) && ((uintptr_t)dout % 16 == 0) && workspace_bytes >= ptc_spconv_wgrad_workspace_bytes(n_out, kv, c_in, c_out);
}
static void wgrad3_add(W3Group& g, const void* in, int64_t n_in, const void* dout, const int32_t* nbr, int64_t n_out, int c_in, int c_out, float* dw,
                       float* dbias, void* workspace, PtcWgradJob* job) {
  int splits, cps;
  ptc_wgrad3_plan(n_out, c_in, c_out, &splits, &cps);
  const int64_t count = (int64_t)c_out * c_in;
  float* partial = (float*)workspace;
  float* bias_partial = dbias ? (float*)((char*)workspace + ptc_align_up((size_t)splits * (size_t)count * sizeof(float), 256)) : nullptr;
  const int tiles_i = c_in / 128, tiles = tiles_i * (c_out / 128);
  const int q = g.n++;
  g.p[q] = W3Problem{in, dout, nbr, n_out, c_in, c_out, partial, bias_partial, splits, cps, tiles, tiles_i, (uint32_t)((uint64_t)n_in * c_in * 2),
                     (uint32_t)((uint64_t)n_out * c_out * 2)};
  g.start[q + 1] = g.start[q] + splits * tiles;
  for (int k = q + 2; k <= W3_MAX; ++k) g.start[k] = g.start[q + 1];
  *job = PtcWgradJob{partial, splits, count, dw, bias_partial, (int64_t)c_out, dbias};
}

template <typename T>
static int launch_wgrad2_group(const PtcWgradCall* const* cs, int m, PtcWgradJob* const* jobs, hipStream_t s) {
  W2Group<T> g;
  g.n = m;
  int grid = 0;
  size_t lds = 0;
  for (int q = 0; q < m; ++q) {
    const PtcWgradCall& c = *cs[q];
    const W2Plan p = w2_plan(c.n_out, c.kv, c.c_in, c.c_out, c.dbias != nullptr);
    const int64_t count = (int64_t)c.c_out * c.kv * c.c_in;
    float* partial = p.gx > 1 ? (float*)c.workspace : c.dw;
    float* bias_partial = nullptr;
    if (c.dbias) bias_partial = p.gx > 1 ? (float*)((char*)c.workspace + ptc_align_up((size_t)p.gx * (size_t)count * sizeof(float), 256)) : c.dbias;
    const int nblocks = p.co_blocks * p.ci_blocks, total = p.gx * p.groups * nblocks;
    g.start[q] = grid;
    g.p[q] = W2Problem<T>{(const T*)c.in, (const T*)c.dout, c.nbr, c.n_out, c.kv, c.c_in, c.c_out, ptc_cdiv(c.n_out, W2_ROWS), p.ci_blocks, partial,
                          bias_partial, p.gx, p.groups, nblocks, (uint32_t)((uint64_t)c.n_in * c.c_in * sizeof(T)),
                          (uint32_t)((uint64_t)c.n_out * c.c_out * sizeof(T))};
    grid += 8 * ((total + 7) / 8);
    lds = p.lds;
    *jobs[q] = PtcWgradJob{partial, p.gx > 1 ? p.gx : 0, count, c.dw, bias_partial, (int64_t)c.c_out, c.dbias};
  }
  for (int q = m; q <= W2_GROUP_MAX; ++q) g.start[q] = grid;
  auto kern = wgrad2_group_kernel<T, 4, 4, 1>;
  if (lds > 48 * 1024) PTC_HIP(hipFuncSetAttribute(reinterpret_cast<const void*>(kern), hipFuncAttributeMaxDynamicSharedMemorySize, (int)lds));
  hipLaunchKernelGGL(kern, dim3((unsigned)grid), dim3(256), lds, s, g);
  PTC_CHECK_LAUNCH("wgrad2_group_kernel");
  return PTC_OK;
}

int ptc_spconv_wgrad_group(const PtcWgradCall* calls, int n, PtcWgradJob* jobs, ptc_stream_t stream) {
  PTC_REQUIRE(calls && jobs && n >= 0, PTC_EINVAL, "ptc_spconv_wgrad_group: null tables");
  const PtcWgradCall* grp[W2_GROUP_MAX];
  PtcWgradJob* gj[W2_GROUP_MAX];
  int m = 0, gdtype = -1;
  W3Group g3;
  g3.n = 0;
  for (int k = 0; k <= W3_MAX; ++k) g3.start[k] = 0;
  int g3dtype = -1;
  for (int i = 0; i < n; ++i) {
    const PtcWgradCall& c = calls[i];
    jobs[i] = PtcWgradJob{nullptr, 0, 0, nullptr, nullptr, 0, nullptr};
    bool grouped = false;
    if (g3.n < W3_MAX && (g3dtype < 0 || g3dtype == c.dtype) &&
        wgrad3_eligible(c.in, c.n_in, c.dout, c.nbr, c.n_out, c.kv, c.c_in, c.c_out, c.dtype, c.dw, c.workspace, c.workspace_bytes)) {
      wgrad3_add(g3, c.in, c.n_in, c.dout, c.nbr, c.n_out, c.c_in, c.c_out, c.dw, c.dbias, c.workspace, &jobs[i]);
      g3dtype = c.dtype;
      continue;
    }
    if (c.n_out > 0 && c.in && c.dout && c.dw && c.workspace && (c.dtype == PTC_BF16 || c.dtype == PTC_F16) && (c.nbr || (c.kv == 1 && c.n_in >= c.n_out)) &&
        c.c_in % 8 == 0 && c.c_out % 8 == 0 && (uint64_t)c.n_in * c.c_in * 2 <= PTC_BUF_MAX_BYTES && (uint64_t)c.n_out * c.c_out * 2 <= PTC_BUF_MAX_BYTES &&
        c.workspace_bytes >= ptc_spconv_wgrad_workspace_bytes(c.n_out, c.kv, c.c_in, c.c_out)) {
      const W2Plan p = w2_plan(c.n_out, c.kv, c.c_in, c.c_out, c.dbias != nullptr);
      if (p.cot == 4 && p.cit == 4 && p.kg == 1 && m < W2_GROUP_MAX && (gdtype < 0 || gdtype == c.dtype)) {
        grp[m] = &c; gj[m] = &jobs[i]; ++m; gdtype = c.dtype;
        grouped = true;
      }
    }
    if (!grouped) {
      const int rc = spconv_wgrad_impl(c.in, c.n_in, c.dout, c.nbr, c.n_out, c.kv, c.c_in, c.c_out, c.dtype, c.dw, c.dbias, c.workspace, c.workspace_bytes,
                                       stream, &jobs[i]);
      if (rc != PTC_OK) return rc;
    }
  }
  if (g3.n > 0) {
    const int rc = ptc_wgrad3_launch(g3dtype, g3, (hipStream_t)stream);
    if (rc != PTC_OK) return rc;
  }
  if (m == 1) {
    const PtcWgradCall& c = *grp[0];
    return spconv_wgrad_impl(c.in, c.n_in, c.dout, c.nbr, c.n_out, c.kv, c.c_in, c.c_out, c.dtype, c.dw, c.dbias, c.workspace, c.workspace_bytes, stream, gj[0]);
  }
  if (m > 1) return gdtype == PTC_BF16 ? launch_wgrad2_group<bf16_t>(grp, m, gj, (hipStream_t)stream) : launch_wgrad2_group<f16_t>(grp, m, gj, (hipStream_t)stream);
  return PTC_OK;
}

extern "C" int ptc_spconv_wgrad(const void* in, int64_t n_in, const void* dout, const int32_t* nbr, int64_t n_out,
                                int kv, int c_in, int c_out, int dtype, float* dw, float* dbias, void* workspace,
                                size_t workspace_bytes, ptc_stream_t stream) {
  return spconv_wgrad_impl(in, n_in, dout, nbr, n_out, kv, c_in, c_out, dtype, dw, dbias, workspace, workspace_bytes, stream, nullptr);
}

int ptc_spconv_wgrad_deferred(const void* in, int64_t n_in, const void* dout, const int32_t* nbr, int64_t n_out, int kv, int c_in, int c_out,
                              int dtype, float* dw, float* dbias, void* workspace, size_t workspace_bytes, ptc_stream_t stream,
                              PtcWgradJob* job) {
  PTC_REQUIRE(job != nullptr, PTC_EINVAL, "ptc_spconv_wgrad_deferred: null job");
  *job = PtcWgradJob{nullptr, 0, 0, nullptr, nullptr, 0, nullptr};
  return spconv_wgrad_impl(in, n_in, dout, nbr, n_out, kv, c_in, c_out, dtype, dw, dbias, workspace, workspace_bytes, stream, job);
}

int ptc_spconv_wgrad_blk_deferred(const void* in, int64_t n_in, const void* dout, const int32_t* nbr, const void* tab, const int32_t* hid,
                                  const int32_t* hcnt, const int32_t* n_overflow, int bm, int hcap, int64_t n_out, int kv, int c_in, int c_out,
                                  int dtype, float* dw, void* workspace, size_t workspace_bytes, ptc_stream_t stream, PtcWgradJob* job) {
  PTC_REQUIRE(job != nullptr, PTC_EINVAL, "ptc_spconv_wgrad_blk: null job");
  *job = PtcWgradJob{nullptr, 0, 0, nullptr, nullptr, 0, nullptr};
  const bool buf_ok = (uint64_t)n_in * c_in * 2 <= PTC_BUF_MAX_BYTES && (uint64_t)n_out * c_out * 2 <= PTC_BUF_MAX_BYTES;
  if (!buf_ok || !tab || !hid || !hcnt || !n_overflow || !nbr || n_in != n_out || !wgrad7_supported(dtype, kv, c_in, c_out, bm, hcap, n_out))
    return spconv_wgrad_impl(in, n_in, dout, nbr, n_out, kv, c_in, c_out, dtype, dw, nullptr, workspace, workspace_bytes, stream, job);
  PTC_REQUIRE(in && dout && dw && workspace, PTC_EINVAL, "ptc_spconv_wgrad_blk: null buffer");
  PTC_REQUIRE(workspace_bytes >= ptc_spconv_wgrad_blk_workspace_bytes(n_out, kv, c_in, c_out), PTC_EWORKSPACE, "ptc_spconv_wgrad_blk: workspace too small");
  PTC_REQUIRE(((uintptr_t)in % 16 == 0) && ((uintptr_t)dout % 16 == 0) && ((uintptr_t)tab % 16 == 0), PTC_EINVAL,
              "ptc_spconv_wgrad_blk: buffers must be 16-byte aligned");
  hipStream_t s = (hipStream_t)stream;
  float* p7 = (float*)((char*)workspace + ptc_spconv_wgrad_workspace_bytes(n_out, kv, c_in, c_out));
  int rc = ptc_wgrad7_launch(dtype, in, dout, (const uint16_t*)tab, hid, hcnt, n_overflow, n_out, c_in, c_out, p7, s);
  if (rc != PTC_OK) return rc;
  PtcWgradJob j2;
  rc = dtype == PTC_BF16 ? launch_wgrad2<bf16_t>(in, n_in, dout, nbr, n_out, kv, c_in, c_out, dw, nullptr, workspace, s, &j2, n_overflow)
                         : launch_wgrad2<f16_t>(in, n_in, dout, nbr, n_out, kv, c_in, c_out, dw, nullptr, workspace, s, &j2, n_overflow);
  if (rc != PTC_OK) return rc;
  *job = PtcWgradJob{p7, wgrad7_splits(n_out, c_in, c_out), (int64_t)c_out * kv * c_in, dw, nullptr, (int64_t)c_out, nullptr, n_overflow, j2.partial, j2.splits};
  return PTC_OK;
}

extern "C" int ptc_spconv_wgrad_blk(const void* in, int64_t n_in, const void* dout, const int32_t* nbr, const void* tab, const int32_t* hid,
                                    const int32_t* hcnt, const int32_t* n_overflow, int bm, int hcap, int64_t n_out, int kv, int c_in, int c_out,
                                    int dtype, float* dw, void* workspace, size_t workspace_bytes, ptc_stream_t stream) {
  PtcWgradJob job;
  const int rc = ptc_spconv_wgrad_blk_deferred(in, n_in, dout, nbr, tab, hid, hcnt, n_overflow, bm, hcap, n_out, kv, c_in, c_out, dtype, dw, workspace,
                                               workspace_bytes, stream, &job);
  if (rc != PTC_OK) return rc;
  return ptc_wgrad_reduce_jobs(&job, 1, stream);
}

static int spconv_wgrad_impl(const void* in, int64_t n_in, const void* dout, const int32_t* nbr, int64_t n_out, int kv, int c_in, int c_out,
                             int dtype, float* dw, float* dbias, void* workspace, size_t workspace_bytes, ptc_stream_t stream, PtcWgradJob* defer) {
  PTC_REQUIRE(n_in >= 0 && n_out >= 0 && kv >= 1, PTC_EINVAL, "ptc_spconv_wgrad: bad sizes");
  PTC_REQUIRE(c_in >= 8 && c_in % 8 == 0 && c_out >= 8 && c_out % 8 == 0, PTC_EUNSUPPORTED,
              "ptc_spconv_wgrad: c_in=%d c_out=%d must be multiples of 8", c_in, c_out);
  PTC_REQUIRE(dw && workspace, PTC_EINVAL, "ptc_spconv_wgrad: null buffer");
  PTC_REQUIRE(workspace_bytes >= ptc_spconv_wgrad_workspace_bytes(n_out, kv, c_in, c_out), PTC_EWORKSPACE,
              "ptc_spconv_wgrad: workspace too small");
  hipStream_t s = (hipStream_t)stream;
  if (n_out == 0) {
    PTC_HIP(hipMemsetAsync(dw, 0, (size_t)c_out * kv * c_in * sizeof(float), s));
    if (dbias) PTC_HIP(hipMemsetAsync(dbias, 0, (size_t)c_out * sizeof(float), s));
    return PTC_OK;
  }
  PTC_REQUIRE(in && dout, PTC_EINVAL, "ptc_spconv_wgrad: null buffer");
  PTC_REQUIRE(nbr || (kv == 1 && n_in >= n_out), PTC_EINVAL, "ptc_spconv_wgrad: nbr may be NULL only for kv == 1 (identity table)");
  const bool buf_ok = (uint64_t)n_in * c_in * 2 <= PTC_BUF_MAX_BYTES && (uint64_t)n_out * c_out * 2 <= PTC_BUF_MAX_BYTES;
  if (wgrad3_eligible(in, n_in, dout, nbr, n_out, kv, c_in, c_out, dtype, dw, workspace, workspace_bytes)) {
    W3Group g3;
    g3.n = 0;
    for (int k = 0; k <= W3_MAX; ++k) g3.start[k] = 0;
    PtcWgradJob job;
    wgrad3_add(g3, in, n_in, dout, nbr, n_out, c_in, c_out, dw, dbias, workspace, &job);
    const int rc = ptc_wgrad3_launch(dtype, g3, s);
    if (rc != PTC_OK) return rc;
    if (defer) { *defer = job; return PTC_OK; }
    return launch_wgrad_reduce(job.partial, job.splits, job.count, dw, job.bias_partial, c_out, dbias, s);
  }
  if (dtype == PTC_BF16 && buf_ok) return launch_wgrad2<bf16_t>(in, n_in, dout, nbr, n_out, kv, c_in, c_out, dw, dbias, workspace, s, defer);
  if (dtype == PTC_F16 && buf_ok) return launch_wgrad2<f16_t>(in, n_in, dout, nbr, n_out, kv, c_in, c_out, dw, dbias, workspace, s, defer);
  PTC_DISPATCH_DTYPE(dtype, T, return launch_wgrad<T>(in, dout, nbr, n_out, kv, c_in, c_out, dw, dbias, workspace, s));
  return PTC_OK;
}
```

pointcept_amd/csrc/spconv_internal.h:

```cpp
#pragma once
#include "ptc_common.h"

struct PtcWgradJob {
  const float* partial;
  int splits;
  int64_t count;
  float* dw;
  const float* bias_partial;
  int64_t c_out;
  float* dbias;
  const int32_t* gate = nullptr;
  const float* alt_partial = nullptr;
  int alt_splits = 0;
};

int ptc_spconv_wgrad_deferred(const void* in, int64_t n_in, const void* dout, const int32_t* nbr, int64_t n_out, int kv, int c_in, int c_out,
                              int dtype, float* dw, float* dbias, void* workspace, size_t workspace_bytes, ptc_stream_t stream,
                              PtcWgradJob* job);
int ptc_spconv_wgrad_blk_deferred(const void* in, int64_t n_in, const void* dout, const int32_t* nbr, const void* tab, const int32_t* hid,
                                  const int32_t* hcnt, const int32_t* n_overflow, int bm, int hcap, int64_t n_out, int kv, int c_in, int c_out,
                                  int dtype, float* dw, void* workspace, size_t workspace_bytes, ptc_stream_t stream, PtcWgradJob* job);
struct PtcWgradCall {
  const void* in; int64_t n_in; const void* dout; const int32_t* nbr; int64_t n_out; int kv, c_in, c_out, dtype;
  float* dw; float* dbias; void* workspace; size_t workspace_bytes;
};
int ptc_spconv_wgrad_group(const PtcWgradCall* calls, int n, PtcWgradJob* jobs, ptc_stream_t stream);
#define PTC_WGRAD_JOBS_MAX 8
int ptc_wgrad_reduce_jobs(const PtcWgradJob* jobs, int n, ptc_stream_t stream);

int ptc_mlp_bwd_deferred(const void* dm, const void* x, int64_t n, int c, int dtype, const void* w1, const float* b1, const void* w2t, void* dx,
                         float* dw1, float* db1, float* dw2, float* db2, void* workspace, size_t workspace_bytes, ptc_stream_t stream,
                         PtcWgradJob* job_fc1, PtcWgradJob* job_fc2);
```

pointcept_amd/csrc/wgrad3.h:

```cpp
#pragma once
#include "ptc_common.h"

#define W3_MAX 8
#ifndef W3_TARGET
#define W3_TARGET 96
#endif
struct W3Problem {
  const void* in; const void* dout; const int32_t* nbr; int64_t n_out; int c_in, c_out;
  float* partial; float* bias_partial;
  int splits, cps, tiles, tiles_i;
  uint32_t in_bytes, dout_bytes;
};
struct W3Group { int n; int start[W3_MAX + 1]; W3Problem p[W3_MAX]; };

bool ptc_wgrad3_supported(int dtype, int kv, int c_in, int c_out, int64_t n_out);
void ptc_wgrad3_plan(int64_t n_out, int c_in, int c_out, int* splits, int* cps);
int ptc_wgrad3_launch(int dtype, const W3Group& g, hipStream_t s);

#ifdef PTC_WGRAD3_IMPL
#include "wgrad2.h"

#define W3_IMG (8 * W2_PLANE)
#define W3_STAGE (4 * W3_IMG)
#define W3_LDS_BYTES (2 * W3_STAGE)

template <typename T>
__global__ void __launch_bounds__(256) PTC_WAVES_PER_EU(2, 2)
wgrad3_kernel(W3Group g) {
  using M = Mma<T>;
  extern __shared__ __attribute__((aligned(16))) unsigned char smem[];
  const int lane = ptc_lane(), wave = threadIdx.x >> 6;
  const int r = lane & 15, gq = lane >> 4;
  const int wo = wave & 1, wi = wave >> 1;

  const int nwg = (int)gridDim.x, id = (int)blockIdx.x;
  const int q8 = nwg >> 3, rem = nwg & 7, xcd = id & 7;
  const int logical = xcd * q8 + (xcd < rem ? xcd : rem) + (id >> 3);
  int pj = 0;
#pragma unroll
  for (int q = 1; q < W3_MAX; ++q)
    if (q < g.n && logical >= g.start[q]) pj = q;
  const W3Problem& P = g.p[pj];
  const int local = logical - g.start[pj];
  const int split = local / P.tiles, tile = local - split * P.tiles;
  const int to = tile / P.tiles_i, ti = tile - to * P.tiles_i;
  const int c_in = P.c_in, c_out = P.c_out;
  const int64_t n_out = P.n_out;
  const int32_t* __restrict__ nbr = P.nbr;
  const __amdgpu_buffer_rsrc_t in_buf = ptc_buf(P.in, P.in_bytes), dout_buf = ptc_buf(P.dout, P.dout_bytes);
  const int64_t n_chunks = (n_out + 63) >> 6;
  const int64_t ch0 = (int64_t)split * P.cps;
  int64_t ch1 = ch0 + P.cps;
  if (ch1 > n_chunks) ch1 = n_chunks;
  const int total = (int)(ch1 - ch0);
  const bool do_bias = P.bias_partial != nullptr && ti == 0 && wi == 0;

  const int piece = threadIdx.x & 15, rr = threadIdx.x >> 4;
  int lds_off[4];
#pragma unroll
  for (int i = 0; i < 4; ++i) {
    const int row = rr + 16 * i;
    lds_off[i] = (row >> 5) * W3_IMG + w2_off(row & 31, piece);
  }
  const uint32_t d_col = (uint32_t)(to * 128 + piece * 8) * 2u, x_col = (uint32_t)(ti * 128 + piece * 8) * 2u;

  ptc_i32x4 rd0[4], rx0[4], rd1[4], rx1[4];
  int32_t idx_next[4];
  auto request_idx = [&](int64_t ch) __attribute__((always_inline)) {
#pragma unroll
    for (int i = 0; i < 4; ++i) {
      int64_t row = (ch << 6) + rr + 16 * i;
      if (row >= n_out) row = n_out - 1;
      idx_next[i] = nbr ? nbr[row] : (int32_t)row;
    }
  };
  auto fetch = [&](int64_t ch, ptc_i32x4 (&rd)[4], ptc_i32x4 (&rx)[4]) __attribute__((always_inline)) {
    uint32_t xo[4], dofs[4];
#pragma unroll
    for (int i = 0; i < 4; ++i) {
      const int64_t row = (ch << 6) + rr + 16 * i;
      const bool ok = row < n_out;
      xo[i] = (ok && idx_next[i] >= 0) ? (uint32_t)idx_next[i] * (uint32_t)c_in * 2u + x_col : PTC_BUF_OOB;
      dofs[i] = ok ? (uint32_t)row * (uint32_t)c_out * 2u + d_col : PTC_BUF_OOB;
    }
    request_idx(ch + 1);
#pragma unroll
    for (int i = 0; i < 4; ++i) {
      rd[i] = __builtin_amdgcn_raw_buffer_load_b128(dout_buf, (int)dofs[i], 0, 0);
      rx[i] = __builtin_amdgcn_raw_buffer_load_b128(in_buf, (int)xo[i], 0, 0);
    }
  };
  auto store_chunk = [&](int st, const ptc_i32x4 (&rd)[4], const ptc_i32x4 (&rx)[4]) __attribute__((always_inline)) {
    unsigned char* base = smem + st * W3_STAGE;
#pragma unroll
    for (int i = 0; i < 4; ++i) {
      *reinterpret_cast<ptc_i32x4*>(base + lds_off[i]) = rd[i];
      *reinterpret_cast<ptc_i32x4*>(base + 2 * W3_IMG + lds_off[i]) = rx[i];
    }
  };

  f32x4 acc[4][4], accb[4];
#pragma unroll
  for (int t = 0; t < 4; ++t) {
    accb[t] = (f32x4){0.f, 0.f, 0.f, 0.f};
#pragma unroll
    for (int u = 0; u < 4; ++u) acc[t][u] = (f32x4){0.f, 0.f, 0.f, 0.f};
  }
  typename M::frag ones;
  {
    const short one = sizeof(T) == 2 && std::is_same<T, bf16_t>::value ? (short)0x3f80 : (short)0x3c00;
    s16x8 o = {one, one, one, one, one, one, one, one};
    __builtin_memcpy(&ones, &o, sizeof(ones));
  }

  request_idx(ch0);
  fetch(ch0, rd0, rx0);
  fetch(ch0 + 1, rd1, rx1);
  store_chunk(0, rd0, rx0);
  __syncthreads();

  auto half = [&](int it, ptc_i32x4 (&rdL)[4], ptc_i32x4 (&rxL)[4], const ptc_i32x4 (&rdS)[4], const ptc_i32x4 (&rxS)[4]) __attribute__((always_inline)) {
    fetch(ch0 + it + 2, rdL, rxL);
    const unsigned char* st = smem + (it & 1) * W3_STAGE;
#pragma unroll
    for (int ks = 0; ks < 2; ++ks) {
      typename M::frag fa[4], fb[4];
#pragma unroll
      for (int t = 0; t < 4; ++t) fa[t] = w2_frag<T>(st + ks * W3_IMG, wo * 4 + t, lane);
#pragma unroll
      for (int u = 0; u < 4; ++u) fb[u] = w2_frag<T>(st + 2 * W3_IMG + ks * W3_IMG, wi * 4 + u, lane);
#pragma unroll
      for (int t = 0; t < 4; ++t)
#pragma unroll
        for (int u = 0; u < 4; ++u) acc[t][u] = M::mma(fa[t], fb[u], acc[t][u]);
      if (do_bias) {
#pragma unroll
        for (int t = 0; t < 4; ++t) accb[t] = M::mma(fa[t], ones, accb[t]);
      }
    }
    if (it + 1 < total) store_chunk((it + 1) & 1, rdS, rxS);
    __syncthreads();
  };
  int it = 0;
#pragma unroll 1
  for (; it + 1 < total; it += 2) {
    half(it, rd0, rx0, rd1, rx1);
    half(it + 1, rd1, rx1, rd0, rx0);
  }
  if (it < total) half(it, rd0, rx0, rd1, rx1);

  float* __restrict__ part = P.partial + (int64_t)split * c_out * c_in;
#pragma unroll
  for (int t = 0; t < 4; ++t)
#pragma unroll
    for (int e = 0; e < 4; ++e) {
      const int co = to * 128 + wo * 64 + t * 16 + 4 * gq + e;
      float* dst = part + (int64_t)co * c_in + ti * 128 + wi * 64 + r;
#pragma unroll
      for (int u = 0; u < 4; ++u) dst[16 * u] = acc[t][u][e];
    }
  if (do_bias && r == 0) {
    float* bp = P.bias_partial + (int64_t)split * c_out + to * 128 + wo * 64 + 4 * gq;
#pragma unroll
    for (int t = 0; t < 4; ++t)
#pragma unroll
      for (int e = 0; e < 4; ++e) bp[16 * t + e] = accb[t][e];
  }
}

static inline bool wgrad3_enabled() {
  static const bool on = [] { const char* e = getenv("PTC_WGRAD3"); return !(e && e[0] == '0'); }();
  return on;
}
bool ptc_wgrad3_supported(int dtype, int kv, int c_in, int c_out, int64_t n_out) {
  return wgrad3_enabled() && dtype != PTC_F32 && kv == 1 && c_in >= 128 && c_in % 128 == 0 && c_out % 128 == 0 && n_out >= 1;
}
void ptc_wgrad3_plan(int64_t n_out, int c_in, int c_out, int* splits, int* cps) {
  const int64_t n_chunks = (n_out + 63) >> 6;
  const int tiles = (c_in / 128) * (c_out / 128);
  int64_t s = (W3_TARGET + tiles - 1) / tiles;
  const int64_t min_s = (n_chunks + 127) / 128;
  if (s < min_s) s = min_s;
  if (s > 64) s = 64;
  const int64_t max_s = (n_chunks + 3) / 4;
  if (s > max_s) s = max_s;
  if (s < 1) s = 1;
  const int64_t c = (n_chunks + s - 1) / s;
  *cps = (int)c;
  *splits = (int)((n_chunks + c - 1) / c);
}

int ptc_wgrad3_launch(int dtype, const W3Group& g, hipStream_t s) {
  const int grid = g.start[g.n];
  if (grid <= 0) return PTC_OK;
  if (dtype == PTC_BF16) {
    auto kern = wgrad3_kernel<bf16_t>;
    PTC_HIP(hipFuncSetAttribute(reinterpret_cast<const void*>(kern), hipFuncAttributeMaxDynamicSharedMemorySize, W3_LDS_BYTES));
    hipLaunchKernelGGL(kern, dim3((unsigned)grid), dim3(256), W3_LDS_BYTES, s, g);
  } else {
    auto kern = wgrad3_kernel<f16_t>;
    PTC_HIP(hipFuncSetAttribute(reinterpret_cast<const void*>(kern), hipFuncAttributeMaxDynamicSharedMemorySize, W3_LDS_BYTES));
    hipLaunchKernelGGL(kern, dim3((unsigned)grid), dim3(256), W3_LDS_BYTES, s, g);
  }
  PTC_CHECK_LAUNCH("wgrad3_kernel");
  return PTC_OK;
}
#endif
```

pointcept_amd/functional.py:

```python
from __future__ import annotations

import os
import weakref
from typing import Optional

import torch
import torch.nn.functional as F
from torch.autograd import Function
from torch.autograd.function import once_differentiable

from . import _lib, config, ops
from ._lib import PtcoreError


class _CastCache:

    def __init__(self, cuda_only: bool = True):
        self.entries = {}
        self.cuda_only = cuda_only
        self.by_shadow = {}
        self.layouts = {}
        self._desc = None
        self._cast_desc = None

# ... 702 lines not shown
             ws=None)
    if len(_blk_plans) > 256:
        _blk_plans.clear()
    _blk_plans[key] = p
    return p


def _blk_tables(E, x0, meta):
    import ctypes

    n, c = x0.shape
    blk = meta["blk"]
    iv = (ctypes.c_int64 * E["I_COUNT"])()
    iv[E["I_ABI"]], iv[E["I_N"]], iv[E["I_NPAD"]], iv[E["I_NSEQ"]], iv[E["I_C"]] = E["ABI"], n, meta["n_pad"], meta["n_seq"], c
    iv[E["I_HEADS"]], iv[E["I_DTYPE"]], iv[E["I_A_DTYPE"]], iv[E["I_PATCH"]] = (meta["heads"], _lib.PTC_F16 if meta["dt"] == torch.float16 else _lib.PTC_BF16,
                                                                              _lib.dtype_code(x0), meta["patch"])
    iv[E["I_BLK_BM"]], iv[E["I_BLK_HCAP"]] = (0, 0) if blk is None else (blk.bm, blk.hcap)
    fv = (ctypes.c_float * E["F_COUNT"])()
    fv[E["F_SCALE"]], fv[E["F_EPS_CPE"]], fv[E["F_EPS_N1"]], fv[E["F_EPS_N2"]] = meta["scale"], meta["eps_cpe"], meta["eps_n1"], meta["eps_n2"]
    pin = (ctypes.c_void_p * E["P_COUNT"])()
    tabs = meta["tabs"]
    pin[E["P_NBR"]], pin[E["P_CU"]] = meta["nbr"].data_ptr(), meta["cu"].data_ptr()
    pin[E["P_T_QKV_FWD"]], pin[E["P_T_QKV_BWD"]] = tabs[0].data_ptr(), tabs[1].data_ptr()
    pin[E["P_T_PROJ_FWD"]], pin[E["P_T_PROJ_BWD"]] = tabs[2].data_ptr(), tabs[3].data_ptr()
    if blk is not None:
        pin[E["P_BLK_TAB"]], pin[E["P_BLK_HID"]], pin[E["P_BLK_HCNT"]] = blk.tab.data_ptr(), blk.hid.data_ptr(), blk.hcnt.data_ptr()
        if config.WGRAD_BLK:
            pin[E["P_BLK_NOVF"]] = blk.n_overflow.data_ptr()
    return iv, fv, pin


class _BlockFn(Function):

    @staticmethod
    def forward(ctx, x0, xc, rs1, rs2, meta, *params):
        dt = meta["dt"]
        n, c = x0.shape
        npad, heads = meta["n_pad"], meta["heads"]
        dev = x0.device
        x0 = x0.contiguous()
        xc = xc.contiguous()
        plan = _blk_plan(n, npad, c, heads, x0.dtype == torch.float32, dt)
        E = plan["E"]
        iv, fv, pin = _blk_tables(E, x0, meta)
        keep = []
        for k, p in zip(_BLK_PARAMS, params):
            if p is None:
                continue
            if k in _BLK_WEIGHTS:
                t = _cast_cache.get(p.reshape(p.shape[0], -1, p.shape[-1]) if p.dim() == 5 else p, dt)
            else:
                t = p if p.dtype == torch.float32 else p.float()
            if not t.is_contiguous():
                t = t.contiguous()
            keep.append(t)
            pin[E["P_" + k]] = t.data_ptr()
        pin[E["P_X0"]], pin[E["P_XC"]] = x0.data_ptr(), xc.data_ptr()
        if rs1 is not None:
            pin[E["P_RS1"]] = rs1.data_ptr()
        if rs2 is not None:
            pin[E["P_RS2"]] = rs2.data_ptr()
        buf16 = torch.empty(plan["t16"], dtype=dt, device=dev)
        buf32 = torch.empty(plan["t32"], dtype=torch.float32, device=dev)
        x3 = torch.empty((n, c), dtype=torch.float32, device=dev)
        xb3 = torch.empty((n, c), dtype=dt, device=dev)
        import ctypes

        pout = (ctypes.c_void_p * E["O_COUNT"])()
        b16, b32 = buf16.data_ptr(), buf32.data_ptr()
        for idx, off in plan["o16"]:
            pout[idx] = b16 + off
        for idx, off in plan["o32"]:
            pout[idx] = b32 + off
        pout[E["O_X3"]], pout[E["O_XB3"]] = x3.data_ptr(), xb3.data_ptr()
        _lib.check(ops.lib().ptc_ptv3_block_fwd(iv, fv, pin, pout, ops.stream_ptr()), "ptc_ptv3_block_fwd")
        ctx.save_for_backward(x0, xc, rs1, rs2, buf16, buf32, x3, xb3, *keep)
        ctx.meta, ctx.plan = meta, plan
        ctx.present = [p is not None for p in params]
        ctx.param_dtypes = [None if p is None else p.dtype for p in params]
        ctx.param_shapes = [None if p is None else p.shape for p in params]
        ctx.set_materialize_grads(False)
        return x3, xb3

    @staticmethod
    @once_differentiable
    def backward(ctx, dz3, dyb3):
        import ctypes

        n_par = len(_BLK_PARAMS)
        if dz3 is None and dyb3 is None:
            return (None,) * (5 + n_par)
        sv = ctx.saved_tensors
        x0, xc, rs1, rs2, buf16, buf32, x3, xb3 = sv[:8]
        meta, plan = ctx.meta, ctx.plan
        E = plan["E"]
        dt = meta["dt"]
        n, c = x0.shape
        npad, heads = meta["n_pad"], meta["heads"]
        dev = x0.device
        iv, fv, pin = _blk_tables(E, x0, meta)
        it = iter(sv[8:])
        sh = {}
        keep_wt = []
        for k, present in zip(_BLK_PARAMS, ctx.present):
            if present:
                t = next(it)
                pin[E["P_" + k]] = t.data_ptr()
                if k in _BLK_WEIGHTS:
                    sh[k] = t
        for k, mode, slots in (("CONV", "mirror", 0), ("LIN", "mirror", 0), ("QKV", "repeat", 2), ("PROJ", "mirror", 0), ("FC1", "mirror", 0),
                               ("FC2", "mirror", 0)):
            w = sh["W_" + k]
            wt = _cast_cache.layout(w, mode, slots)
            if wt is None:
                w3 = w if w.dim() == 3 else w[:, None, :]
                wt = (w3.flip(1).permute(2, 1, 0) if mode == "mirror" else w3.permute(2, 1, 0).expand(-1, slots, -1)).contiguous()
                keep_wt.append(wt)
            pin[E["P_WT_" + k]] = wt.data_ptr()
        pin[E["P_X0"]], pin[E["P_XC"]] = x0.data_ptr(), xc.data_ptr()
        if rs1 is not None:
            pin[E["P_RS1"]] = rs1.data_ptr()
        if rs2 is not None:
            pin[E["P_RS2"]] = rs2.data_ptr()
        dz3c = None if dz3 is None else (dz3 if dz3.dtype == torch.float32 and dz3.is_contiguous() else dz3.float().contiguous())
        dyb3c = None if dyb3 is None else (dyb3 if dyb3.dtype == dt and dyb3.is_contiguous() else dyb3.to(dt).contiguous())
        if dz3c is not None:
            pin[E["P_DZ3"]] = dz3c.data_ptr()
        if dyb3c is not None:
            pin[E["P_DYB3"]] = dyb3c.data_ptr()
        psv = (ctypes.c_void_p * E["O_COUNT"])()
        b16, b32 = buf16.data_ptr(), buf32.data_ptr()
        for idx, off in plan["o16"]:
            psv[idx] = b16 + off
        for idx, off in plan["o32"]:
            psv[idx] = b32 + off
        psv[E["O_X3"]], psv[E["O_XB3"]] = x3.data_ptr(), xb3.data_ptr()
        gbuf = torch.empty(plan["tg"], dtype=torch.float32, device=dev)
        gscr = torch.empty(plan["tgs"], dtype=torch.float32, device=dev)
        sbuf = torch.empty(plan["ts"], dtype=dt, device=dev)
        pg = (ctypes.c_void_p * E["GS_COUNT"])()
        bg, bgs, bs = gbuf.data_ptr(), gscr.data_ptr(), sbuf.data_ptr()
        for idx, off in plan["g32"]:
            pg[idx] = bg + off
        for idx, off in plan["g32s"]:
            pg[idx] = bgs + off
        for idx, off in plan["g16"]:
            pg[idx] = bs + off
        for k, present in zip(_BLK_PARAMS, ctx.present):
            if not present:
                pg[E["G_" + k]] = None
        if plan["ws"] is None:
            plan["ws"] = int(ops.lib().ptc_ptv3_block_workspace_bytes(n, npad, c, heads))
        nbytes = plan["ws"]
        ws = torch.empty(nbytes, dtype=torch.uint8, device=dev)
        _lib.check(ops.lib().ptc_ptv3_block_bwd(iv, fv, pin, psv, pg, ws.data_ptr(), nbytes, ops.stream_ptr()), "ptc_ptv3_block_bwd")
        dx0 = (gscr if x0.dtype == torch.float32 else sbuf)[plan["gx0"]:plan["gx0"] + n * c].view(n, c)
        dxc = sbuf[plan["gxc"]:plan["gxc"] + n * c].view(n, c)
        grads = []
        for k, present, pdt, shp in zip(_BLK_PARAMS, ctx.present, ctx.param_dtypes, ctx.param_shapes):
            if not present:
                grads.append(None)
                continue
            off, cnt = plan["gparam"][k]
            g = gbuf[off:off + cnt].view(shp)
            grads.append(g if pdt == torch.float32 else g.to(pdt))
        return (dx0, dxc, None, None, None, *grads)


def ptv3_block(x0, xc, rs1, rs2, meta, params):
    return _BlockFn.apply(x0, xc, rs1, rs2, meta, *params)


class _MLP(Function):

    @staticmethod
    def forward(ctx, x, w1, b1, w2, b2):
        dt = torch.get_autocast_dtype("cuda") if _autocast_on() else x.dtype
        xp = x.to(dt).contiguous()
        w1c, w2c = _cast_cache.get(w1, dt).contiguous(), _cast_cache.get(w2, dt).contiguous()
        ctx.dtypes = (x.dtype, w1.dtype, None if b1 is None else b1.dtype, w2.dtype, None if b2 is None else b2.dtype)
        ctx.one_kernel = config.MLP_ONE_KERNEL and w1.shape[0] == 4 * w1.shape[1] and w2.shape[0] == w1.shape[1] and ops.mlp_supported(w1.shape[1], dt)
        if ctx.one_kernel:
            ctx.save_for_backward(xp, w1c, w2c, b1)
            return ops.mlp_fwd(xp, w1c, b1, w2c, b2)
        h, a = ops.linear_gelu_fwd(xp, w1c, b1)
        out = ops.spconv_fwd(a, w2c[:, None, :], None if b2 is None else b2.float(), None)
        ctx.save_for_backward(xp, h, a, w1c, w2c)
        return out

    @staticmethod
    @once_differentiable
    def backward(ctx, dout):
        x_dt, w1_dt, b1_dt, w2_dt, b2_dt = ctx.dtypes
        if ctx.one_kernel:
            xp, w1c, w2c, b1 = ctx.saved_tensors
            w2t = _cast_cache.layout(w2c, "mirror")
            dx, dw1, db1, dw2, db2 = ops.mlp_bwd(dout.to(xp.dtype).contiguous(), xp, w1c, b1, w2c.t().contiguous() if w2t is None else w2t[:, 0, :],
                                                 want_b1=b1_dt is not None, want_b2=b2_dt is not None)
            return (dx.to(x_dt) if ctx.needs_input_grad[0] else None, dw1.to(w1_dt), None if db1 is None else db1.to(b1_dt), dw2.to(w2_dt),
                    None if db2 is None else db2.to(b2_dt))
        xp, h, a, w1c, w2c = ctx.saved_tensors
        g = dout.to(xp.dtype).contiguous()
        n = g.shape[0]
        res = ops.spconv_wgrad(a, g, None, want_bias=b2_dt is not None)
        dw2, db2 = res if b2_dt is not None else (res, None)
        dw2 = dw2[:, 0, :]
        dw2 = dw2.to(w2_dt)
        db2 = None if db2 is None else db2.to(b2_dt)
        w2t = _cast_cache.layout(w2c, "mirror")
        dh = ops.linear_gelu_bwd_input(g, w2c.t().contiguous() if w2t is None else w2t[:, 0, :], h)
        res = ops.spconv_wgrad(xp, dh, None, want_bias=b1_dt is not None)
        dw1, db1 = res if b1_dt is not None else (res, None)
        dw1 = dw1[:, 0, :]
        dw1 = dw1.to(w1_dt)
        db1 = None if db1 is None else db1.to(b1_dt)
        dx = None
        if ctx.needs_input_grad[0]:
            w1t = _cast_cache.layout(w1c, "mirror")
            dx = ops.spconv_fwd(dh, w1c.t().contiguous()[:, None, :] if w1t is None else w1t, None, None).to(x_dt)
        return dx, dw1, db1, dw2, db2


def mlp_gelu_supported(x: torch.Tensor, w1: torch.Tensor, w2: torch.Tensor) -> bool:
    if not (x.is_cuda and x.dim() == 2 and x.shape[0] > 0):
        return False
    dt = torch.get_autocast_dtype("cuda") if _autocast_on() else x.dtype
    hidden, c = w1.shape
    return (dt in (torch.bfloat16, torch.float16) and c % 16 == 0 and hidden % 16 == 0 and w2.shape[0] % 16 == 0
            and ops.linear_supported_ex(c, hidden, dt) and ops.linear_supported_ex(w2.shape[0], hidden, dt)
            and _own_gemm(0, hidden, dt, w2.shape[0]) and _own_gemm(0, hidden, dt, c))


def mlp_gelu(x, w1, b1, w2, b2):
    return _MLP.apply(x, w1, b1, w2, b2)


class _ClusterCenter(Function):
    @staticmethod
    def forward(ctx, gc, *xs):
        ctx.gc = gc
        return tuple(ops.cluster_center(list(xs), gc))

    @staticmethod
    @once_differentiable
    def backward(ctx, *gys):
        gys = [g.contiguous() if g is not None else None for g in gys]
        if any(g is None for g in gys):
            ref = next(g for g in gys if g is not None)
            gys = [torch.zeros_like(ref) if g is None else g for g in gys]
        return (None, *ops.cluster_center(gys, ctx.gc))


def cluster_center(xs, gc: "ops.GridClusters") -> list:
    dt = xs[0].dtype
    return list(_ClusterCenter.apply(gc, *[x.to(dt).contiguous() for x in xs]))


class _ClusterAgg(Function):
    @staticmethod
    def forward(ctx, gc, a, *uv):
        L = gc.levels
        us, vs = list(uv[:L]), list(uv[L:])
        out, state = ops.cluster_agg_fwd(us, vs, a, gc)
        ctx.gc = gc
        ctx.save_for_backward(a, state, *us, *vs)
        return out

    @staticmethod
    @once_differentiable
    def backward(ctx, dout):
        a, state, *uv = ctx.saved_tensors
        L = ctx.gc.levels
        du, dv, da = ops.cluster_agg_bwd(uv[:L], uv[L:], a, dout, state, ctx.gc)
        return (None, da, *du, *dv)


def cluster_agg(us, vs, a: torch.Tensor, gc: "ops.GridClusters") -> torch.Tensor:
    dt = us[0].dtype
    c = lambda t: t.to(dt).contiguous()
    return _ClusterAgg.apply(gc, c(a), *[c(u) for u in us], *[c(v) for v in vs])


def cluster_center_torch(xs, gc: "ops.GridClusters") -> list:
    out = []
    for x, cl, n_c in zip(xs, gc.cluster, gc.n_cluster):
        s = x.new_zeros((n_c, x.shape[1])).index_add(0, cl, x)
        cnt = torch.bincount(cl, minlength=n_c).clamp(min=1).to(x.dtype)
        out.append(x - (s / cnt[:, None])[cl])
    return out


def cluster_agg_torch(us, vs, a: torch.Tensor, gc: "ops.GridClusters") -> torch.Tensor:
    feats = []
    for u, v, cl, n_c in zip(us, vs, gc.cluster, gc.n_cluster):
        pw = torch.exp(u - u.max())
        pw = pw / (pw.new_zeros((n_c, pw.shape[1])).index_add(0, cl, pw)[cl] + 1e-6)
        pf = v * pw
        feats.append(pf.new_zeros((n_c, pf.shape[1])).index_add(0, cl, pf)[cl])
    adp = torch.softmax(a, dim=1)
    return torch.einsum("l n, l n c -> l c", adp, torch.stack(feats, dim=1))


class _PGBiasLoss(Function):
    @staticmethod
    def forward(ctx, bias_pred, coord, centroid, instance, ignore_index):
        out = ops.pg_bias_loss_fwd(bias_pred, coord, centroid, instance, ignore_index)
        ctx.save_for_backward(bias_pred, coord, centroid, instance, out)
# ... 318 lines not shown
```

pointcept_amd/ops.py:

```python
from __future__ import annotations

import ctypes
from typing import Optional, Sequence

import torch

from . import _lib
from ._lib import PtcoreError, check, dtype_code, lib, ptr, require_cuda, stream_ptr


def _ws(nbytes: int, device) -> torch.Tensor:
    return torch.empty(max(int(nbytes), 1), dtype=torch.uint8, device=device)


def serialize_encode(grid_coord: torch.Tensor, batch: Optional[torch.Tensor], depth: int,
                     orders: Sequence[str]) -> torch.Tensor:
    require_cuda(grid_coord, batch)
    if grid_coord.dtype not in (torch.int64, torch.int32):
        raise PtcoreError(f"grid_coord must be int32/int64, got {grid_coord.dtype}")
    gc = grid_coord.contiguous()
    n = gc.shape[0]
    b = None if batch is None else batch.to(torch.int64).contiguous()
    k = len(orders)
    oc = (ctypes.c_int * k)(*[_lib.ORDER_CODES[o] for o in orders])
    out = torch.empty((k, n), dtype=torch.int64, device=gc.device)
    check(lib().ptc_serialize_encode(ptr(gc), 1 if gc.dtype == torch.int64 else 0, ptr(b), n, int(depth),
                                     ctypes.cast(oc, ctypes.c_void_p), k, ptr(out), stream_ptr()),
          "ptc_serialize_encode")
    return out


def sort_keys(keys: torch.Tensor, begin_bit: int, end_bit: int, want_inverse: bool = True):
    require_cuda(keys)
    if keys.dtype != torch.int64:
        raise PtcoreError("keys must be int64")
    squeeze = keys.dim() == 1
    k2 = keys.reshape(1, -1) if squeeze else keys
    k2 = k2.contiguous()
    k, n = k2.shape
    order = torch.empty_like(k2)
    inverse = torch.empty_like(k2) if want_inverse else None
    nbytes = lib().ptc_sort_keys_workspace_bytes(n, k)
    ws = _ws(nbytes, k2.device)
    check(lib().ptc_sort_keys(ptr(k2), n, k, int(begin_bit), int(end_bit), ptr(order), ptr(inverse), ptr(ws), nbytes,
                              stream_ptr()), "ptc_sort_keys")
    if squeeze:
        return order[0], (inverse[0] if want_inverse else None)
    return order, inverse


def exclusive_scan_i32(x: torch.Tensor) -> torch.Tensor:
    require_cuda(x)
    x = x.to(torch.int32).contiguous()
    n = x.numel()
    out = torch.empty(n, dtype=torch.int64, device=x.device)
    nbytes = lib().ptc_exclusive_scan_workspace_bytes(n)
    ws = _ws(nbytes, x.device)
    check(lib().ptc_exclusive_scan_i32(ptr(x), n, ptr(out), ptr(ws), nbytes, stream_ptr()), "ptc_exclusive_scan_i32")
    return out


def pad_sizes(offset_host: Sequence[int], patch: int):
    prev, n_pad, n_seq = 0, 0, 0
    for o in offset_host:
        ni = int(o) - prev
        prev = int(o)
        p = ((ni + patch - 1) // patch) * patch if ni > patch else ni
        n_pad += p
        n_seq += (p + patch - 1) // patch
    return prev, n_pad, n_seq


def patch_pad_maps(offset: torch.Tensor, offset_host: Sequence[int], patch: int):
    require_cuda(offset)
    off = offset.to(torch.int64).contiguous()
    n, n_pad, n_seq = pad_sizes(offset_host, patch)
    dev = off.device
    pad = torch.empty(n_pad, dtype=torch.int64, device=dev)
    unpad = torch.empty(n, dtype=torch.int64, device=dev)
    cu = torch.empty(n_seq + 1, dtype=torch.int32, device=dev)
    dup = torch.empty(n, dtype=torch.int64, device=dev)
    check(lib().ptc_patch_pad_maps(ptr(off), off.numel(), int(patch), n, n_pad, n_seq, ptr(pad), ptr(unpad), ptr(cu),
                                   ptr(dup), stream_ptr()), "ptc_patch_pad_maps")
    return pad, unpad, cu, dup


def attn_tables(order: torch.Tensor, inverse: torch.Tensor, pad: torch.Tensor, unpad: torch.Tensor, dup: torch.Tensor):
    require_cuda(order, inverse, pad, unpad, dup)
    n, n_pad = order.numel(), pad.numel()
    dev = order.device
    t1 = torch.empty((1, n_pad), dtype=torch.int32, device=dev)
    t2 = torch.empty((2, n), dtype=torch.int32, device=dev)
    t3 = torch.empty((1, n), dtype=torch.int32, device=dev)
    t4 = torch.empty((1, n_pad), dtype=torch.int32, device=dev)
    check(lib().ptc_attn_tables(ptr(order.contiguous()), ptr(inverse.contiguous()), ptr(pad), ptr(unpad), ptr(dup), n, n_pad,
                                ptr(t1), ptr(t2), ptr(t3), ptr(t4), stream_ptr()), "ptc_attn_tables")
    return t1, t2, t3, t4


def pool_level_counts(code0: torch.Tensor, order0: torch.Tensor, batch_shift: int, n_batch: int, shifts: Sequence[int]):
    require_cuda(code0, order0)
    import ctypes

    counts = torch.empty((len(shifts), n_batch), dtype=torch.int64, device=code0.device)
    arr = (ctypes.c_int * len(shifts))(*[int(v) for v in shifts])
    check(lib().ptc_pool_level_counts(ptr(code0.contiguous()), ptr(order0.contiguous()), code0.numel(), int(batch_shift), int(n_batch),
                                      ctypes.cast(arr, ctypes.c_void_p), len(shifts), ptr(counts), stream_ptr()),
          "ptc_pool_level_counts")
    return counts


def pool_maps(code0: torch.Tensor, order0: torch.Tensor, shift: int, n_cluster: Optional[int] = None):
    require_cuda(code0, order0)
    code0 = code0.contiguous()
    order0 = order0.contiguous()
    n = code0.numel()
    dev = code0.device
    cluster = torch.empty(n, dtype=torch.int64, device=dev)
    ncl = torch.empty(1, dtype=torch.int64, device=dev)
    nbytes = lib().ptc_pool_maps_workspace_bytes(n)
    ws = _ws(nbytes, dev)
    check(lib().ptc_pool_maps_count(ptr(code0), ptr(order0), n, int(shift), ptr(cluster), ptr(ncl), ptr(ws), nbytes,
                                    stream_ptr()), "ptc_pool_maps_count")
    if n_cluster is None:
        n_cluster = int(ncl.item())
    idx_ptr = torch.empty(n_cluster + 1, dtype=torch.int64, device=dev)
    head = torch.empty(n_cluster, dtype=torch.int64, device=dev)
    check(lib().ptc_pool_maps_fill(ptr(order0), ptr(cluster), n, n_cluster, ptr(idx_ptr), ptr(head), stream_ptr()),
          "ptc_pool_maps_fill")
    return cluster, idx_ptr, head


def pool_child_codes(code: torch.Tensor, head: torch.Tensor, shift: int) -> torch.Tensor:
    require_cuda(code, head)
    code = code.contiguous()
    head = head.contiguous()
    k, n = code.shape
    nc = head.numel()
    out = torch.empty((k, nc), dtype=torch.int64, device=code.device)
    check(lib().ptc_pool_child_codes(ptr(code), n, k, ptr(head), nc, int(shift), ptr(out), stream_ptr()),
          "ptc_pool_child_codes")
    return out


def voxel_keys(coord: torch.Tensor, grid_size: float):
    require_cuda(coord)
    if coord.dtype != torch.float32 or coord.dim() != 2 or coord.shape[1] != 3:
        raise PtcoreError("coord must be float32 [N,3]")
    c = coord.contiguous()
    n = c.shape[0]
    grid = torch.empty((n, 3), dtype=torch.int64, device=c.device)
    mn = torch.empty(3, dtype=torch.int64, device=c.device)
    key = torch.empty(n, dtype=torch.int64, device=c.device)
    check(lib().ptc_voxel_keys(ptr(c), n, float(grid_size), ptr(grid), ptr(mn), ptr(key), stream_ptr()), "ptc_voxel_keys")
    return grid, mn, key


def _xyz(t: torch.Tensor, name: str) -> torch.Tensor:
    if t.dtype != torch.float32 or t.dim() != 2 or t.shape[1] != 3:
        raise PtcoreError(f"{name} must be float32 [N,3]")
    return t.contiguous()


def knn_query(nsample: int, xyz, offset, new_xyz, new_offset):
    require_cuda(xyz, offset, new_xyz, new_offset)
# ... 226 lines not shown
                              "coordinate in the input)")
        if spatial_shape is not None and m >= int(spatial_shape[a]):
            raise PtcoreError(f"grid_coord axis {a}: maximum {m} outside the declared spatial_shape {list(spatial_shape)}")
    if int(batch_size) > BATCH_MAX:
        raise PtcoreError(f"batch size {batch_size} exceeds the {BATCH_MAX} batch items the voxel key can hold")


class HashTable:
    def __init__(self, indices: torch.Tensor):
        require_cuda(indices)
        if indices.dtype != torch.int32 or indices.dim() != 2 or indices.shape[1] != 4:
            raise PtcoreError("indices must be int32 [N,4] (batch,x,y,z)")
        self.indices = indices.contiguous()
        n = self.indices.shape[0]
        self.size = int(lib().ptc_hash_table_size(n))
        self.nbytes = int(lib().ptc_hash_table_bytes(n))
        self.buf = torch.empty(self.nbytes // 8, dtype=torch.int64, device=indices.device)
        check(lib().ptc_hash_build(ptr(self.indices), n, ptr(self.buf), self.nbytes, stream_ptr()), "ptc_hash_build")


def rulebook_subm(indices: torch.Tensor, ksize: int, table: Optional[HashTable] = None) -> torch.Tensor:
    if table is None:
        table = HashTable(indices)
    ind = table.indices
    n = ind.shape[0]
    nbr = torch.empty((ksize ** 3, n), dtype=torch.int32, device=ind.device)
    check(lib().ptc_rulebook_subm(ptr(ind), n, int(ksize), ptr(table.buf), table.nbytes, ptr(nbr), stream_ptr()),
          "ptc_rulebook_subm")
    return nbr


BLOCK_BM, BLOCK_HCAP = 128, 416


class BlockTables:

    def __init__(self, nbr: torch.Tensor, bm: int = BLOCK_BM, hcap: int = BLOCK_HCAP):
        require_cuda(nbr)
        if nbr.dtype != torch.int32 or nbr.dim() != 2 or nbr.shape[0] != 27:
            raise PtcoreError("nbr must be int32 [27, n]")
        self.nbr = nbr.contiguous()
        kv, n = self.nbr.shape
        self.bm, self.hcap = int(bm), int(hcap)
        nblk = max(1, (n + self.bm - 1) // self.bm)
        dev = nbr.device
        self.tab = torch.empty(int(lib().ptc_rulebook_blocks_tab_bytes(n)) // 2, dtype=torch.int16, device=dev).view(2, nblk, 28, 32, 4)
        self.hid = torch.empty((nblk, self.hcap), dtype=torch.int32, device=dev)
        self.hcnt = torch.empty(nblk, dtype=torch.int32, device=dev)
        self.n_overflow = torch.empty(1, dtype=torch.int32, device=dev)
        check(lib().ptc_rulebook_blocks(ptr(self.nbr), kv, n, self.bm, self.hcap, ptr(self.tab), ptr(self.hid), ptr(self.hcnt),
                                        ptr(self.n_overflow), stream_ptr()), "ptc_rulebook_blocks")


def block_plan(c_in: int, c_out: int, kv: int, dtype: torch.dtype, n_rows: int = 1 << 30):
    if dtype == torch.float32 or kv != 27:
        return None
    if c_in == c_out and c_in in (32, 64):
        return (BLOCK_BM, BLOCK_HCAP) if n_rows >= 4096 else None
    if c_in % 32 == 0 and c_out % 32 == 0 and c_in <= 1024 and c_out <= 1024 and (c_in // (64 if c_in % 64 == 0 else 32)) * (c_out // 32) <= 256 \
            and n_rows >= 1024:
        return (BLOCK_BM, BLOCK_HCAP)
    return None


class BlockProvider:

    def __init__(self, nbr: torch.Tensor):
        self.nbr = nbr
        self.tables = {}

    def get(self, c_in: int, c_out: int, dtype: torch.dtype, conv: bool = False):
        plan = block_plan(c_in, c_out, self.nbr.shape[0], dtype, self.nbr.shape[1])
        from . import config

        conv_kernel = (c_in == c_out and c_in in (32, 64)) or (config.CONV8 and c_in >= 96)
        if plan is None or not self.nbr.is_cuda or (conv and not conv_kernel):
            return None
        t = self.tables.get(plan)
        if t is None:
            t = self.tables[plan] = BlockTables(self.nbr, *plan)
        return t


def rulebook_down(indices: torch.Tensor, coord_bits: int, batch_bits: int):
    require_cuda(indices)
    ind = indices.contiguous()
    n = ind.shape[0]
    dev = ind.device
    out_of_in = torch.empty(n, dtype=torch.int32, device=dev)
    n_out_dev = torch.empty(1, dtype=torch.int64, device=dev)
    nbytes = lib().ptc_rulebook_down_workspace_bytes(n)
    ws = _ws(nbytes, dev)
    check(lib().ptc_rulebook_down_count(ptr(ind), n, int(coord_bits), int(batch_bits), ptr(out_of_in), ptr(n_out_dev),
                                        ptr(ws), nbytes, stream_ptr()), "ptc_rulebook_down_count")
    n_out = int(n_out_dev.item())
    out_indices = torch.empty((n_out, 4), dtype=torch.int32, device=dev)
    nbr_down = torch.empty((8, n_out), dtype=torch.int32, device=dev)
    nbr_up = torch.empty((8, n), dtype=torch.int32, device=dev)
    check(lib().ptc_rulebook_down_fill(ptr(ind), n, ptr(out_of_in), n_out, ptr(out_indices), ptr(nbr_down), ptr(nbr_up),
                                       stream_ptr()), "ptc_rulebook_down_fill")
    return out_indices, nbr_down, nbr_up


def spconv_fwd(feat: torch.Tensor, weight: torch.Tensor, bias: Optional[torch.Tensor],
               nbr: Optional[torch.Tensor], blk: Optional["BlockTables"] = None) -> torch.Tensor:
    require_cuda(feat, weight, bias, nbr)
    feat = feat.contiguous()
    weight = weight.contiguous()
    if weight.dtype != feat.dtype:
        raise PtcoreError("weight dtype must match feature dtype")
    c_out, kv, c_in = weight.shape
    if nbr is not None:
        nbr = nbr.contiguous()
        if nbr.shape[0] != kv or nbr.dtype != torch.int32:
            raise PtcoreError(f"table mismatch: weight {tuple(weight.shape)} nbr {tuple(nbr.shape)} {nbr.dtype}")
    elif kv != 1:
        raise PtcoreError("nbr=None needs kv == 1")
    if feat.shape[1] != c_in:
        raise PtcoreError(f"shape mismatch: feat {tuple(feat.shape)} weight {tuple(weight.shape)}")
    if bias is not None:
        bias = bias.to(torch.float32).contiguous()
    n_out = nbr.shape[1] if nbr is not None else feat.shape[0]
    out = torch.empty((n_out, c_out), dtype=feat.dtype, device=feat.device)
    if blk is not None and nbr is not None:
        if blk.nbr.data_ptr() != nbr.data_ptr() or tuple(blk.nbr.shape) != tuple(nbr.shape):
            raise PtcoreError("blk was built from another gather table")
        check(lib().ptc_spconv_fwd_blk(ptr(feat), feat.shape[0], ptr(weight), ptr(bias), ptr(nbr), ptr(blk.tab), ptr(blk.hid),
                                       ptr(blk.hcnt), blk.bm, blk.hcap, n_out, kv, c_in, c_out, dtype_code(feat), ptr(out),
                                       stream_ptr()), "ptc_spconv_fwd_blk")
        return out
    check(lib().ptc_spconv_fwd(ptr(feat), feat.shape[0], ptr(weight), ptr(bias), ptr(nbr), n_out, kv, c_in, c_out,
                               dtype_code(feat), ptr(out), stream_ptr()), "ptc_spconv_fwd")
    return out


def spconv_wgrad(feat: torch.Tensor, dout: torch.Tensor, nbr: Optional[torch.Tensor], want_bias: bool = False,
                 blk: Optional["BlockTables"] = None):
    require_cuda(feat, dout, nbr)
    feat = feat.contiguous()
    dout = dout.contiguous()
    if feat.dtype != dout.dtype:
        raise PtcoreError("feat / dout dtype mismatch")
    if nbr is not None:
        nbr = nbr.contiguous()
        kv, n_out = nbr.shape
    else:
        kv, n_out = 1, dout.shape[0]
    c_in, c_out = feat.shape[1], dout.shape[1]
    dw = torch.empty((c_out, kv, c_in), dtype=torch.float32, device=feat.device)
    if blk is not None and nbr is not None and not want_bias:
        if blk.nbr.data_ptr() != nbr.data_ptr() or tuple(blk.nbr.shape) != tuple(nbr.shape):
            raise PtcoreError("blk was built from another gather table")
        nbytes = lib().ptc_spconv_wgrad_blk_workspace_bytes(n_out, kv, c_in, c_out)
        ws = _ws(nbytes, feat.device)
        check(lib().ptc_spconv_wgrad_blk(ptr(feat), feat.shape[0], ptr(dout), ptr(nbr), ptr(blk.tab), ptr(blk.hid), ptr(blk.hcnt),
                                         ptr(blk.n_overflow), blk.bm, blk.hcap, n_out, kv, c_in, c_out, dtype_code(feat), ptr(dw), ptr(ws),
                                         nbytes, stream_ptr()), "ptc_spconv_wgrad_blk")
        return dw
    db = torch.empty(c_out, dtype=torch.float32, device=feat.device) if want_bias else None
    nbytes = lib().ptc_spconv_wgrad_workspace_bytes(n_out, kv, c_in, c_out)
    ws = _ws(nbytes, feat.device)
    check(lib().ptc_spconv_wgrad(ptr(feat), feat.shape[0], ptr(dout), ptr(nbr), n_out, kv, c_in, c_out,
                                 dtype_code(feat), ptr(dw), ptr(db), ptr(ws), nbytes, stream_ptr()), "ptc_spconv_wgrad")
    return (dw, db) if want_bias else dw


def seg_eval_hist(logits: Optional[torch.Tensor], target: torch.Tensor, k: int, ignore_index: int = -1,
                  inverse: Optional[torch.Tensor] = None, pred: Optional[torch.Tensor] = None):
    require_cuda(logits, target, inverse, pred)
    if (logits is None) == (pred is None):
        raise PtcoreError("give logits or pred")
    target = target.reshape(-1).to(torch.int64).contiguous()
    m = target.numel()
    hist = torch.empty((3, int(k)), dtype=torch.int64, device=target.device)
    if pred is not None:
        pred = pred.reshape(-1).to(torch.int64).contiguous()
        if pred.numel() != m:
            raise PtcoreError("pred / target size mismatch")
        check(lib().ptc_seg_eval_hist(0, 0, 0, 0, ptr(pred), 0, ptr(target), m, 0, int(k), int(ignore_index), ptr(hist), stream_ptr()),
              "ptc_seg_eval_hist")
    else:
        if logits.dim() != 2 or logits.stride(1) != 1:
            raise PtcoreError("logits must be [N, C] with unit column stride")
        if inverse is not None:
            inverse = inverse.reshape(-1).to(torch.int64).contiguous()
            if inverse.numel() != m:
                raise PtcoreError("inverse / target size mismatch")
        elif logits.shape[0] != m:
            raise PtcoreError("logits / target size mismatch")
        check(lib().ptc_seg_eval_hist(ptr(logits), dtype_code(logits), logits.stride(0), logits.shape[1], 0, ptr(inverse), ptr(target), m,
                                      logits.shape[0], int(k), int(ignore_index), ptr(hist), stream_ptr()), "ptc_seg_eval_hist")
    return hist[0], hist[1] + hist[2] - hist[0], hist[2]


def rope3d_(tokens: torch.Tensor, positions: torch.Tensor, base: float, fwd: float) -> torch.Tensor:
    require_cuda(tokens, positions)
    if tokens.dim() < 3 or not tokens.is_contiguous():
        raise PtcoreError("tokens must be contiguous [..., H, D]")
    if positions.dtype != torch.int64 or not positions.is_contiguous() or positions.shape[-1] != 3:
        raise PtcoreError("positions must be contiguous int64 [..., 3]")
    H, D = tokens.shape[-2], tokens.shape[-1]
    n = tokens.numel() // (H * D) if H * D > 0 else 0
    if positions.numel() != 3 * n:
        raise PtcoreError(f"positions {tuple(positions.shape)} do not match tokens {tuple(tokens.shape)}")
    check(lib().ptc_rope3d(ptr(tokens), dtype_code(tokens), ptr(positions), n, H, D, float(base), float(fwd), stream_ptr()), "ptc_rope3d")
    return tokens


def rope3d_xyz(qkv: torch.Tensor, xyz: torch.Tensor, inv_freq: torch.Tensor, rot_slabs: int, sign: float,
               out_dtype: Optional[torch.dtype] = None) -> torch.Tensor:
    require_cuda(qkv, xyz, inv_freq)
    if qkv.dim() != 4 or not qkv.is_contiguous():
        raise PtcoreError("rope3d_xyz: qkv must be contiguous [n, slabs, H, D]")
    n, S, H, D = qkv.shape
    if D % 6 != 0:
        raise PtcoreError(f"rope3d_xyz: head dim {D} must be a multiple of 6")
    if xyz.dtype != torch.float32 or tuple(xyz.shape) != (n, 3) or not xyz.is_contiguous():
        raise PtcoreError("rope3d_xyz: xyz must be contiguous fp32 [n, 3]")
    if inv_freq.dtype != torch.float32 or inv_freq.numel() != D // 6 or not inv_freq.is_contiguous():
        raise PtcoreError(f"rope3d_xyz: inv_freq must be contiguous fp32 [{D // 6}]")
    out = torch.empty(qkv.shape, dtype=out_dtype or qkv.dtype, device=qkv.device)
    check(lib().ptc_rope3d_xyz(ptr(qkv), dtype_code(qkv), ptr(out), dtype_code(out), ptr(xyz), ptr(inv_freq), n, S, int(rot_slabs), H, D,
                               float(sign), stream_ptr()), "ptc_rope3d_xyz")
    return out


_DT = {torch.float32: _lib.PTC_F32, torch.float16: _lib.PTC_F16, torch.bfloat16: _lib.PTC_BF16}


def layer_norm_supported(c: int) -> bool:
    return lib().ptc_layer_norm_supported(int(c)) == 1


def layer_norm_joint_available(c: int) -> bool:
    return lib().ptc_layer_norm_supported(int(c)) != 0


def layer_norm_available(c: int) -> bool:
    return lib().ptc_layer_norm_supported(int(c)) != 0


def layer_norm_fwd(x: torch.Tensor, gamma, beta, eps: float, out_dtype: torch.dtype):
    require_cuda(x, gamma, beta)
    x = x.contiguous()
    n, c = x.shape
    g = None if gamma is None else gamma.to(torch.float32).contiguous()
    b = None if beta is None else beta.to(torch.float32).contiguous()
    y = torch.empty((n, c), dtype=out_dtype, device=x.device)
    mean = torch.empty(n, dtype=torch.float32, device=x.device)
    rstd = torch.empty(n, dtype=torch.float32, device=x.device)
    check(lib().ptc_layer_norm_fwd(ptr(x), n, c, dtype_code(x), ptr(g), ptr(b), float(eps), ptr(y), _DT[out_dtype],
                                   ptr(mean), ptr(rstd), stream_ptr()), "ptc_layer_norm_fwd")
    return y, mean, rstd


def layer_norm_bwd(dy: torch.Tensor, x: torch.Tensor, mean, rstd, gamma, want_affine: bool = True):
    require_cuda(dy, x, mean, rstd, gamma)
    dy = dy.contiguous()
    x = x.contiguous()
    n, c = x.shape
    g = None if gamma is None else gamma.to(torch.float32).contiguous()
    dx = torch.empty_like(x)
    dg = torch.empty(c, dtype=torch.float32, device=x.device) if want_affine else None
    db = torch.empty(c, dtype=torch.float32, device=x.device) if want_affine else None
    nbytes = lib().ptc_layer_norm_bwd_workspace_bytes(n, c)
    ws = _ws(nbytes, x.device)
    check(lib().ptc_layer_norm_bwd(ptr(dy), dtype_code(dy), ptr(x), dtype_code(x), ptr(mean), ptr(rstd), ptr(g), n, c,
                                   ptr(dx), ptr(dg), ptr(db), ptr(ws), nbytes, stream_ptr()), "ptc_layer_norm_bwd")
    return dx, dg, db


def add_norm_fwd(u, a, row_scale, norm_a, norm_b, y_dtype):
    require_cuda(u, a, row_scale)
    u = u.contiguous()
    a = a.contiguous()
    if a.dtype not in (torch.float32, torch.bfloat16, torch.float16):
        raise PtcoreError("add_norm: the residual operand `a` must be fp32, bf16 or f16")
    n, c = u.shape
    dev = u.device
    z = torch.empty((n, c), dtype=torch.float32, device=dev)
    y = torch.empty((n, c), dtype=y_dtype, device=dev) if y_dtype is not None else None
    st_a = torch.empty((2, n), dtype=torch.float32, device=dev) if norm_a is not None else None
    st_b = torch.empty((2, n), dtype=torch.float32, device=dev) if (norm_b is not None and y is not None) else None
    ga, ba, ea = norm_a if norm_a is not None else (None, None, 0.0)
    gb, bb, eb = norm_b if norm_b is not None else (None, None, 0.0)
    rs = None if row_scale is None else row_scale.to(torch.float32).contiguous()
    check(lib().ptc_add_norm_fwd(ptr(u), dtype_code(u), ptr(a), dtype_code(a), ptr(rs), n, c, ptr(ga), ptr(ba), float(ea),
                                 int(norm_a is not None), ptr(gb), ptr(bb), float(eb), int(norm_b is not None), ptr(z), ptr(y),
                                 _DT[y_dtype] if y_dtype is not None else 0, ptr(st_a), ptr(st_b), stream_ptr()),
          "ptc_add_norm_fwd")
    return z, y, st_a, st_b


def linear_joint_supported(c_in: int, c_out: int, dtype: torch.dtype) -> bool:
    return dtype in (torch.bfloat16, torch.float16) and bool(lib().ptc_linear_joint_supported(int(c_in), int(c_out), _DT[dtype]))


def linear_joint_fwd(x, weight, bias, table, a, row_scale, norm_b, y_dtype, n_out=None):
    require_cuda(x, weight, bias, table, a, row_scale)
    x, weight, a = x.contiguous(), weight.contiguous(), a.contiguous()
    c_out, c_in = weight.shape[0], weight.shape[-1]
    if a.dtype != torch.float32 or x.dtype != weight.dtype or not linear_joint_supported(c_in, c_out, x.dtype):
        raise PtcoreError("linear_joint_fwd: unsupported shape / dtype")
    n = int(a.shape[0]) if n_out is None else int(n_out)
    tab = None if table is None else table.reshape(-1).to(torch.int32).contiguous()
    dev = x.device
    z = torch.empty((n, c_out), dtype=torch.float32, device=dev)
    y = torch.empty((n, c_out), dtype=y_dtype, device=dev) if y_dtype is not None else None
    st_b = torch.empty((2, n), dtype=torch.float32, device=dev) if (norm_b is not None and y is not None) else None
    gb, bb, eb = norm_b if norm_b is not None else (None, None, 0.0)
    rs = None if row_scale is None else row_scale.to(torch.float32).contiguous()
    b = None if bias is None else bias.float().contiguous()
    check(lib().ptc_linear_joint_fwd(ptr(x), x.shape[0], ptr(weight), ptr(b), ptr(tab), n, c_in, c_out, dtype_code(x), ptr(a), ptr(rs), ptr(gb), ptr(bb),
                                     float(eb), int(norm_b is not None), ptr(z), ptr(y), ptr(st_b), stream_ptr()), "ptc_linear_joint_fwd")
    return z, y, st_b


# ... 951 lines not shown
```

Measured before the change: 232.1 scenes/s.

## Fuse wgrad3 split-K reduction into GEMM via last-block atomic counters

The split-K weight-gradient kernel now keeps per-tile arrival counters in a zeroed header of a persistent workspace. The last split block to finish a tile sums the partials (and bias partials) directly into dw, so the separate reduction pass is no longer needed. It also adds a grouped linear wgrad entry point and a cached, pre-zeroed workspace allocator that the counters depend on. The risks are extra threadfence and atomic cost, and correctness hinging on counters being reset and the workspace staying zeroed across calls.

Measured after the change: 217.5 scenes/s. -6.3%, worse.

```diff
diff --git a/include/ptcore.h b/include/ptcore.h
--- a/include/ptcore.h
+++ b/include/ptcore.h
@@ -117,6 +117,11 @@
 int ptc_spconv_wgrad(const void* in, int64_t n_in, const void* dout, const int32_t* nbr,
                      int64_t n_out, int kv, int c_in, int c_out, int dtype, float* dw, float* dbias,
                      void* workspace, size_t workspace_bytes, ptc_stream_t stream);
+int ptc_wgrad3_tune(int fused, int target, int min_chunks);
+int ptc_wgrad3_splits(int64_t n_out, int c_in, int c_out);
+size_t ptc_linear_wgrad_group_workspace_bytes(int n, int64_t rows, const int* c_in, const int* c_out);
+int ptc_linear_wgrad_group(int n, int64_t rows, const void* const* in, const void* const* dout, const int* c_in, const int* c_out, int dtype,
+                           float* const* dw, float* const* dbias, void* workspace, size_t workspace_bytes, ptc_stream_t stream);
 
 int ptc_seg_eval_hist(const void* logits, int dtype, int64_t row_stride, int c, const int64_t* pred, const int64_t* inverse,
                       const int64_t* target, int64_t m, int64_t n_rows, int k, int64_t ignore_index, int64_t* hist3k,
diff --git a/pointcept_amd/_lib.py b/pointcept_amd/_lib.py
--- a/pointcept_amd/_lib.py
+++ b/pointcept_amd/_lib.py
@@ -62,6 +62,10 @@
     "ptc_mlp_bwd_workspace_bytes": (c_size, [c_i64, c_int]),
     "ptc_mlp_bwd": (c_int, [c_ptr, c_ptr, c_i64, c_int, c_int, c_ptr, c_ptr, c_ptr, c_ptr, c_ptr, c_ptr, c_ptr, c_ptr, c_ptr, c_size, c_ptr]),
     "ptc_spconv_wgrad_workspace_bytes": (c_size, [c_i64, c_int, c_int, c_int]),
+    "ptc_wgrad3_tune": (c_int, [c_int, c_int, c_int]),
+    "ptc_wgrad3_splits": (c_int, [c_i64, c_int, c_int]),
+    "ptc_linear_wgrad_group_workspace_bytes": (c_size, [c_int, c_i64, c_ptr, c_ptr]),
+    "ptc_linear_wgrad_group": (c_int, [c_int, c_i64, c_ptr, c_ptr, c_ptr, c_ptr, c_int, c_ptr, c_ptr, c_ptr, c_size, c_ptr]),
     "ptc_spconv_wgrad": (c_int, [c_ptr, c_i64, c_ptr, c_ptr, c_i64, c_int, c_int, c_int, c_int, c_ptr, c_ptr, c_ptr, c_size,
                                  c_ptr]),
     "ptc_seg_eval_hist": (c_int, [c_ptr, c_int, c_i64, c_int, c_ptr, c_ptr, c_ptr, c_i64, c_i64, c_int, c_i64, c_ptr, c_ptr]),
diff --git a/pointcept_amd/csrc/block_exec.hip b/pointcept_amd/csrc/block_exec.hip
--- a/pointcept_amd/csrc/block_exec.hip
+++ b/pointcept_amd/csrc/block_exec.hip
@@ -30,14 +30,14 @@
   up(ptc_attn_varlen_bwd_workspace_bytes(n_pad, heads));
   up(ptc_batch_norm_workspace_bytes(n, c));
   w.common = ptc_align_up(w.common, 256);
-  w.wg[0] = ptc_spconv_wgrad_workspace_bytes(n, 1, hid, c);
+  w.wg[0] = ptc_spconv_wgrad_body_bytes(n, 1, hid, c);
   if (ptc_mlp_supported(c, PTC_BF16) && ptc_mlp_bwd_workspace_bytes(n, c) > w.wg[0]) w.wg[0] = ptc_mlp_bwd_workspace_bytes(n, c);
-  w.wg[1] = ptc_spconv_wgrad_workspace_bytes(n, 1, c, hid);
-  w.wg[2] = ptc_spconv_wgrad_workspace_bytes(n, 1, c, c);
-  w.wg[3] = ptc_spconv_wgrad_workspace_bytes(n_pad, 1, c, 3 * c);
-  w.wg[4] = ptc_spconv_wgrad_workspace_bytes(n, 1, c, c);
-  w.wg[5] = ptc_spconv_wgrad_blk_workspace_bytes(n, 27, c, c);
-  size_t o = w.common;
+  w.wg[1] = ptc_spconv_wgrad_body_bytes(n, 1, c, hid);
+  w.wg[2] = ptc_spconv_wgrad_body_bytes(n, 1, c, c);
+  w.wg[3] = ptc_spconv_wgrad_body_bytes(n_pad, 1, c, 3 * c);
+  w.wg[4] = ptc_spconv_wgrad_body_bytes(n, 1, c, c);
+  w.wg[5] = ptc_spconv_wgrad_blk_body_bytes(n, 27, c, c);
+  size_t o = PTC_WGRAD_HDR_BYTES + w.common;
   for (int i = 0; i < 6; ++i) { w.off[i] = o; o += ptc_align_up(w.wg[i], 256); }
   w.total = o;
   return w;
@@ -118,11 +118,12 @@
   const float* rs1 = (const float*)P(in, PTC_BLK_P_RS1);
   const float* rs2 = (const float*)P(in, PTC_BLK_P_RS2);
   const BlkWs W = blk_ws(n, np, c, H);
-  void* ws = workspace;
+  void* ws = (char*)workspace + PTC_WGRAD_HDR_BYTES;
   const size_t wb = W.common;
   PtcWgradJob jobs[6];
   PtcWgradCall calls[5];
   auto wgws = [&](int i) { return (void*)((char*)workspace + W.off[i]); };
+  auto wgcnt = [&](int i) { return (uint32_t*)((char*)workspace + (size_t)i * PTC_WGRAD_CNT_BYTES); };
   RUN(ptc_add_norm_bwd((const float*)P(in, PTC_BLK_P_DZ3), P(in, PTC_BLK_P_DYB3), dt, (const float*)P(sv, PTC_BLK_O_X3), P(sv, PTC_BLK_O_M), dt, rs2, n, c,
                        nullptr, nullptr, 0, nullptr, nullptr, 0, g[PTC_BLK_S_DX2], PTC_F32, g[PTC_BLK_S_DM], nullptr, nullptr, nullptr, nullptr, ws, wb, s));
   const bool mlp_fused = ptc_ptv3_block_mlp_fused(c, dt) != 0;
@@ -131,31 +132,31 @@
                              P(in, PTC_BLK_P_WT_FC2), g[PTC_BLK_S_DY2], M<float>(g, PTC_BLK_G_W_FC1), M<float>(g, PTC_BLK_G_B_FC1),
                              M<float>(g, PTC_BLK_G_W_FC2), M<float>(g, PTC_BLK_G_B_FC2), wgws(0), W.wg[0], s, &jobs[1], &jobs[0]));
   } else {
-  calls[0] = PtcWgradCall{P(sv, PTC_BLK_O_ACT), n, g[PTC_BLK_S_DM], nullptr, n, 1, hid, c, dt, M<float>(g, PTC_BLK_G_W_FC2), M<float>(g, PTC_BLK_G_B_FC2), wgws(0), W.wg[0]};
+  calls[0] = PtcWgradCall{P(sv, PTC_BLK_O_ACT), n, g[PTC_BLK_S_DM], nullptr, n, 1, hid, c, dt, M<float>(g, PTC_BLK_G_W_FC2), M<float>(g, PTC_BLK_G_B_FC2), wgws(0), W.wg[0], wgcnt(0)};
   RUN(ptc_linear_fwd_ex(g[PTC_BLK_S_DM], n, P(in, PTC_BLK_P_WT_FC2), nullptr, c, hid, dt, 2, P(sv, PTC_BLK_O_H), g[PTC_BLK_S_DH], nullptr, s));
-  calls[1] = PtcWgradCall{P(sv, PTC_BLK_O_Y2), n, g[PTC_BLK_S_DH], nullptr, n, 1, c, hid, dt, M<float>(g, PTC_BLK_G_W_FC1), M<float>(g, PTC_BLK_G_B_FC1), wgws(1), W.wg[1]};
+  calls[1] = PtcWgradCall{P(sv, PTC_BLK_O_Y2), n, g[PTC_BLK_S_DH], nullptr, n, 1, c, hid, dt, M<float>(g, PTC_BLK_G_W_FC1), M<float>(g, PTC_BLK_G_B_FC1), wgws(1), W.wg[1], wgcnt(1)};
   RUN(ptc_spconv_fwd(g[PTC_BLK_S_DH], n, P(in, PTC_BLK_P_WT_FC1), nullptr, nullptr, n, 1, hid, c, dt, g[PTC_BLK_S_DY2], s));
   }
   RUN(ptc_add_norm_bwd(M<float>(g, PTC_BLK_S_DX2), g[PTC_BLK_S_DY2], dt, (const float*)P(sv, PTC_BLK_O_X2), P(sv, PTC_BLK_O_A), dt, rs1, n, c, nullptr, nullptr, 0,
                        (const float*)P(in, PTC_BLK_P_G_N2), (const float*)P(sv, PTC_BLK_O_ST_N2), 1, g[PTC_BLK_S_DX1], PTC_F32, g[PTC_BLK_S_DA], nullptr, nullptr,
                        M<float>(g, PTC_BLK_G_G_N2), M<float>(g, PTC_BLK_G_BE_N2), ws, wb, s));
   calls[2] = PtcWgradCall{P(sv, PTC_BLK_O_ATT), np, g[PTC_BLK_S_DA], (const int32_t*)P(in, PTC_BLK_P_T_PROJ_FWD), n, 1, c, c, dt, M<float>(g, PTC_BLK_G_W_PROJ),
-                          M<float>(g, PTC_BLK_G_B_PROJ), wgws(2), W.wg[2]};
+                          M<float>(g, PTC_BLK_G_B_PROJ), wgws(2), W.wg[2], wgcnt(2)};
   RUN(ptc_spconv_fwd(g[PTC_BLK_S_DA], n, P(in, PTC_BLK_P_WT_PROJ), nullptr, (const int32_t*)P(in, PTC_BLK_P_T_PROJ_BWD), np, 1, c, c, dt, g[PTC_BLK_S_DATT], s));
   RUN(ptc_attn_varlen_bwd(P(sv, PTC_BLK_O_QKV), P(sv, PTC_BLK_O_ATT), g[PTC_BLK_S_DATT], (const float*)P(sv, PTC_BLK_O_LSE), (const int32_t*)P(in, PTC_BLK_P_CU), n_seq,
                           np, H, patch, fv[PTC_BLK_F_SCALE], dt, g[PTC_BLK_S_DQKV], ws, wb, s));
   calls[3] = PtcWgradCall{P(sv, PTC_BLK_O_Y1), n, g[PTC_BLK_S_DQKV], (const int32_t*)P(in, PTC_BLK_P_T_QKV_FWD), np, 1, c, 3 * c, dt, M<float>(g, PTC_BLK_G_W_QKV),
-                          M<float>(g, PTC_BLK_G_B_QKV), wgws(3), W.wg[3]};
+                          M<float>(g, PTC_BLK_G_B_QKV), wgws(3), W.wg[3], wgcnt(3)};
   RUN(ptc_spconv_fwd(g[PTC_BLK_S_DQKV], np, P(in, PTC_BLK_P_WT_QKV), nullptr, (const int32_t*)P(in, PTC_BLK_P_T_QKV_BWD), n, 2, 3 * c, c, dt, g[PTC_BLK_S_DY1], s));
   RUN(ptc_add_norm_bwd(M<float>(g, PTC_BLK_S_DX1), g[PTC_BLK_S_DY1], dt, (const float*)P(sv, PTC_BLK_O_X1), P(sv, PTC_BLK_O_LIN), dt, nullptr, n, c,
                        (const float*)P(in, PTC_BLK_P_G_CPE), (const float*)P(sv, PTC_BLK_O_ST_CPE), 1, (const float*)P(in, PTC_BLK_P_G_N1),
                        (const float*)P(sv, PTC_BLK_O_ST_N1), 1, g[PTC_BLK_G_X0], a_dt, g[PTC_BLK_S_DLIN], M<float>(g, PTC_BLK_G_G_CPE), M<float>(g, PTC_BLK_G_BE_CPE),
                        M<float>(g, PTC_BLK_G_G_N1), M<float>(g, PTC_BLK_G_BE_N1), ws, wb, s));
-  calls[4] = PtcWgradCall{P(sv, PTC_BLK_O_CONV), n, g[PTC_BLK_S_DLIN], nullptr, n, 1, c, c, dt, M<float>(g, PTC_BLK_G_W_LIN), M<float>(g, PTC_BLK_G_B_LIN), wgws(4), W.wg[4]};
+  calls[4] = PtcWgradCall{P(sv, PTC_BLK_O_CONV), n, g[PTC_BLK_S_DLIN], nullptr, n, 1, c, c, dt, M<float>(g, PTC_BLK_G_W_LIN), M<float>(g, PTC_BLK_G_B_LIN), wgws(4), W.wg[4], wgcnt(4)};
   RUN(ptc_spconv_fwd(g[PTC_BLK_S_DLIN], n, P(in, PTC_BLK_P_WT_LIN), nullptr, nullptr, n, 1, c, c, dt, g[PTC_BLK_S_DCONV], s));
   RUN(ptc_spconv_wgrad_blk_deferred(P(in, PTC_BLK_P_XC), n, g[PTC_BLK_S_DCONV], nbr, P(in, PTC_BLK_P_BLK_TAB), (const int32_t*)P(in, PTC_BLK_P_BLK_HID),
                                     (const int32_t*)P(in, PTC_BLK_P_BLK_HCNT), (const int32_t*)P(in, PTC_BLK_P_BLK_NOVF), (int)iv[PTC_BLK_I_BLK_BM],
-                                    (int)iv[PTC_BLK_I_BLK_HCAP], n, 27, c, c, dt, M<float>(g, PTC_BLK_G_W_CONV), wgws(5), W.wg[5], s, &jobs[5]));
+                                    (int)iv[PTC_BLK_I_BLK_HCAP], n, 27, c, c, dt, M<float>(g, PTC_BLK_G_W_CONV), wgws(5), W.wg[5], nullptr, s, &jobs[5]));
   RUN(ptc_column_sum(g[PTC_BLK_S_DCONV], n, c, dt, M<float>(g, PTC_BLK_G_B_CONV), ws, wb, s));
   RUN(ptc_spconv_fwd_blk(g[PTC_BLK_S_DCONV], n, P(in, PTC_BLK_P_WT_CONV), nullptr, nbr, P(in, PTC_BLK_P_BLK_TAB), (const int32_t*)P(in, PTC_BLK_P_BLK_HID),
                          (const int32_t*)P(in, PTC_BLK_P_BLK_HCNT), (int)iv[PTC_BLK_I_BLK_BM], (int)iv[PTC_BLK_I_BLK_HCAP], n, 27, c, c, dt, g[PTC_BLK_G_XC], s));
diff --git a/pointcept_amd/csrc/spconv.hip b/pointcept_amd/csrc/spconv.hip
--- a/pointcept_amd/csrc/spconv.hip
+++ b/pointcept_amd/csrc/spconv.hip
@@ -419,6 +419,8 @@
 }
 
 #define WG_REDUCE_FEW 8
+static_assert(WG_REDUCE_FEW == W3_REDUCE_FEW, "wgrad3.h repeats this reduction's order in its tail");
+static_assert(W3_CNT_TILES * sizeof(uint32_t) == PTC_WGRAD_CNT_BYTES && W3_MAX * PTC_WGRAD_CNT_BYTES == PTC_WGRAD_HDR_BYTES, "one counter slot per weight of a group");
 __device__ __forceinline__ void wgrad_reduce_body(const float* __restrict__ partial, int splits, int64_t count, float* __restrict__ dw, int nb1,
                                                   const float* __restrict__ partial2, int64_t count2, float* __restrict__ out2, int bid, bool few) {
   __shared__ float4 red[16][16];
@@ -570,7 +572,7 @@
   return (int)s;
 }
 
-extern "C" size_t ptc_spconv_wgrad_workspace_bytes(int64_t n_out, int kv, int c_in, int c_out) {
+size_t ptc_spconv_wgrad_body_bytes(int64_t n_out, int kv, int c_in, int c_out) {
   size_t splits = (size_t)wgrad_splits(n_out, kv, c_in, c_out);
   size_t gx = (size_t)w2_plan(n_out, kv, c_in, c_out, false).gx;
   const size_t gxb = (size_t)w2_plan(n_out, kv, c_in, c_out, true).gx;
@@ -588,8 +590,14 @@
   if (!wgrad7_supported(PTC_BF16, kv, c_in, c_out, C7_BM, C7_HCAP, n_out)) return 0;
   return ptc_align_up((size_t)wgrad7_splits(n_out, c_in, c_out) * (size_t)c_out * kv * c_in * sizeof(float), 256);
 }
+size_t ptc_spconv_wgrad_blk_body_bytes(int64_t n_out, int kv, int c_in, int c_out) {
+  return ptc_spconv_wgrad_body_bytes(n_out, kv, c_in, c_out) + wgrad_blk_extra_bytes(n_out, kv, c_in, c_out);
+}
+extern "C" size_t ptc_spconv_wgrad_workspace_bytes(int64_t n_out, int kv, int c_in, int c_out) {
+  return PTC_WGRAD_HDR_BYTES + ptc_spconv_wgrad_body_bytes(n_out, kv, c_in, c_out);
+}
 extern "C" size_t ptc_spconv_wgrad_blk_workspace_bytes(int64_t n_out, int kv, int c_in, int c_out) {
-  return ptc_spconv_wgrad_workspace_bytes(n_out, kv, c_in, c_out) + wgrad_blk_extra_bytes(n_out, kv, c_in, c_out);
+  return PTC_WGRAD_HDR_BYTES + ptc_spconv_wgrad_blk_body_bytes(n_out, kv, c_in, c_out);
 }
 
 template <typename T>
@@ -656,16 +664,17 @@
 }
 
 static int spconv_wgrad_impl(const void* in, int64_t n_in, const void* dout, const int32_t* nbr, int64_t n_out, int kv, int c_in, int c_out,
-                             int dtype, float* dw, float* dbias, void* workspace, size_t workspace_bytes, ptc_stream_t stream, PtcWgradJob* defer);
+                             int dtype, float* dw, float* dbias, void* workspace, size_t workspace_bytes, uint32_t* counters, ptc_stream_t stream,
+                             PtcWgradJob* defer);
 
 static bool wgrad3_eligible(const void* in, int64_t n_in, const void* dout, const int32_t* nbr, int64_t n_out, int kv, int c_in, int c_out, int dtype,
                             const float* dw, const void* workspace, size_t workspace_bytes) {
   return n_out > 0 && in && dout && dw && workspace && (dtype == PTC_BF16 || dtype == PTC_F16) && ptc_wgrad3_supported(dtype, kv, c_in, c_out, n_out) &&
          (nbr || n_in >= n_out) && (uint64_t)n_in * c_in * 2 <= PTC_BUF_MAX_BYTES && (uint64_t)n_out * c_out * 2 <= PTC_BUF_MAX_BYTES &&
-         ((uintptr_t)in % 16 == 0) && ((uintptr_t)dout % 16 == 0) && workspace_bytes >= ptc_spconv_wgrad_workspace_bytes(n_out, kv, c_in, c_out);
+         ((uintptr_t)in % 16 == 0) && ((uintptr_t)dout % 16 == 0) && workspace_bytes >= ptc_spconv_wgrad_body_bytes(n_out, kv, c_in, c_out);
 }
 static void wgrad3_add(W3Group& g, const void* in, int64_t n_in, const void* dout, const int32_t* nbr, int64_t n_out, int c_in, int c_out, float* dw,
-                       float* dbias, void* workspace, PtcWgradJob* job) {
+                       float* dbias, void* workspace, uint32_t* counters, PtcWgradJob* job) {
   int splits, cps;
   ptc_wgrad3_plan(n_out, c_in, c_out, &splits, &cps);
   const int64_t count = (int64_t)c_out * c_in;
@@ -673,11 +682,12 @@
   float* bias_partial = dbias ? (float*)((char*)workspace + ptc_align_up((size_t)splits * (size_t)count * sizeof(float), 256)) : nullptr;
   const int tiles_i = c_in / 128, tiles = tiles_i * (c_out / 128);
   const int q = g.n++;
+  const bool fused = counters != nullptr && ptc_wgrad3_fused() && tiles <= W3_CNT_TILES && splits <= W3_MAX_SPLITS;
   g.p[q] = W3Problem{in, dout, nbr, n_out, c_in, c_out, partial, bias_partial, splits, cps, tiles, tiles_i, (uint32_t)((uint64_t)n_in * c_in * 2),
-                     (uint32_t)((uint64_t)n_out * c_out * 2)};
+                     (uint32_t)((uint64_t)n_out * c_out * 2), fused ? counters : nullptr, dw, dbias};
   g.start[q + 1] = g.start[q] + splits * tiles;
   for (int k = q + 2; k <= W3_MAX; ++k) g.start[k] = g.start[q + 1];
-  *job = PtcWgradJob{partial, splits, count, dw, bias_partial, (int64_t)c_out, dbias};
+  *job = fused ? PtcWgradJob{nullptr, 0, 0, nullptr, nullptr, 0, nullptr} : PtcWgradJob{partial, splits, count, dw, bias_partial, (int64_t)c_out, dbias};
 }
 
 template <typename T>
@@ -725,13 +735,13 @@
     bool grouped = false;
     if (g3.n < W3_MAX && (g3dtype < 0 || g3dtype == c.dtype) &&
         wgrad3_eligible(c.in, c.n_in, c.dout, c.nbr, c.n_out, c.kv, c.c_in, c.c_out, c.dtype, c.dw, c.workspace, c.workspace_bytes)) {
-      wgrad3_add(g3, c.in, c.n_in, c.dout, c.nbr, c.n_out, c.c_in, c.c_out, c.dw, c.dbias, c.workspace, &jobs[i]);
+      wgrad3_add(g3, c.in, c.n_in, c.dout, c.nbr, c.n_out, c.c_in, c.c_out, c.dw, c.dbias, c.workspace, c.counters, &jobs[i]);
       g3dtype = c.dtype;
       continue;
     }
     if (c.n_out > 0 && c.in && c.dout && c.dw && c.workspace && (c.dtype == PTC_BF16 || c.dtype == PTC_F16) && (c.nbr || (c.kv == 1 && c.n_in >= c.n_out)) &&
         c.c_in % 8 == 0 && c.c_out % 8 == 0 && (uint64_t)c.n_in * c.c_in * 2 <= PTC_BUF_MAX_BYTES && (uint64_t)c.n_out * c.c_out * 2 <= PTC_BUF_MAX_BYTES &&
-        c.workspace_bytes >= ptc_spconv_wgrad_workspace_bytes(c.n_out, c.kv, c.c_in, c.c_out)) {
+        c.workspace_bytes >= ptc_spconv_wgrad_body_bytes(c.n_out, c.kv, c.c_in, c.c_out)) {
       const W2Plan p = w2_plan(c.n_out, c.kv, c.c_in, c.c_out, c.dbias != nullptr);
       if (p.cot == 4 && p.cit == 4 && p.kg == 1 && m < W2_GROUP_MAX && (gdtype < 0 || gdtype == c.dtype)) {
         grp[m] = &c; gj[m] = &jobs[i]; ++m; gdtype = c.dtype;
@@ -740,7 +750,7 @@
     }
     if (!grouped) {
       const int rc = spconv_wgrad_impl(c.in, c.n_in, c.dout, c.nbr, c.n_out, c.kv, c.c_in, c.c_out, c.dtype, c.dw, c.dbias, c.workspace, c.workspace_bytes,
-                                       stream, &jobs[i]);
+                                       c.counters, stream, &jobs[i]);
       if (rc != PTC_OK) return rc;
     }
   }
@@ -750,7 +760,7 @@
   }
   if (m == 1) {
     const PtcWgradCall& c = *grp[0];
-    return spconv_wgrad_impl(c.in, c.n_in, c.dout, c.nbr, c.n_out, c.kv, c.c_in, c.c_out, c.dtype, c.dw, c.dbias, c.workspace, c.workspace_bytes, stream, gj[0]);
+    return spconv_wgrad_impl(c.in, c.n_in, c.dout, c.nbr, c.n_out, c.kv, c.c_in, c.c_out, c.dtype, c.dw, c.dbias, c.workspace, c.workspace_bytes, c.counters, stream, gj[0]);
   }
   if (m > 1) return gdtype == PTC_BF16 ? launch_wgrad2_group<bf16_t>(grp, m, gj, (hipStream_t)stream) : launch_wgrad2_group<f16_t>(grp, m, gj, (hipStream_t)stream);
   return PTC_OK;
@@ -759,31 +769,59 @@
 extern "C" int ptc_spconv_wgrad(const void* in, int64_t n_in, const void* dout, const int32_t* nbr, int64_t n_out,
                                 int kv, int c_in, int c_out, int dtype, float* dw, float* dbias, void* workspace,
                                 size_t workspace_bytes, ptc_stream_t stream) {
-  return spconv_wgrad_impl(in, n_in, dout, nbr, n_out, kv, c_in, c_out, dtype, dw, dbias, workspace, workspace_bytes, stream, nullptr);
+  PTC_REQUIRE(workspace, PTC_EINVAL, "ptc_spconv_wgrad: null buffer");
+  PTC_REQUIRE(workspace_bytes >= PTC_WGRAD_HDR_BYTES, PTC_EWORKSPACE, "ptc_spconv_wgrad: workspace too small");
+  return spconv_wgrad_impl(in, n_in, dout, nbr, n_out, kv, c_in, c_out, dtype, dw, dbias, (char*)workspace + PTC_WGRAD_HDR_BYTES,
+                           workspace_bytes - PTC_WGRAD_HDR_BYTES, (uint32_t*)workspace, stream, nullptr);
+}
+
+extern "C" size_t ptc_linear_wgrad_group_workspace_bytes(int n, int64_t rows, const int* c_in, const int* c_out) {
+  size_t b = PTC_WGRAD_HDR_BYTES;
+  for (int i = 0; i < n && i < W3_MAX; ++i) b += ptc_align_up(ptc_spconv_wgrad_body_bytes(rows, 1, c_in[i], c_out[i]), 256);
+  return b;
+}
+extern "C" int ptc_linear_wgrad_group(int n, int64_t rows, const void* const* in, const void* const* dout, const int* c_in, const int* c_out, int dtype,
+                                      float* const* dw, float* const* dbias, void* workspace, size_t workspace_bytes, ptc_stream_t stream) {
+  PTC_REQUIRE(n >= 0 && n <= W3_MAX && n <= PTC_WGRAD_JOBS_MAX && in && dout && c_in && c_out && dw && dbias && workspace, PTC_EINVAL,
+              "ptc_linear_wgrad_group: %d weights", n);
+  PTC_REQUIRE(workspace_bytes >= ptc_linear_wgrad_group_workspace_bytes(n, rows, c_in, c_out), PTC_EWORKSPACE, "ptc_linear_wgrad_group: workspace too small");
+  PtcWgradCall calls[W3_MAX];
+  PtcWgradJob jobs[W3_MAX];
+  size_t o = PTC_WGRAD_HDR_BYTES;
+  for (int i = 0; i < n; ++i) {
+    const size_t b = ptc_spconv_wgrad_body_bytes(rows, 1, c_in[i], c_out[i]);
+    calls[i] = PtcWgradCall{in[i], rows, dout[i], nullptr, rows, 1, c_in[i], c_out[i], dtype, dw[i], dbias[i], (char*)workspace + o, b,
+                            (uint32_t*)((char*)workspace + (size_t)i * PTC_WGRAD_CNT_BYTES)};
+    o += ptc_align_up(b, 256);
+  }
+  const int rc = ptc_spconv_wgrad_group(calls, n, jobs, stream);
+  if (rc != PTC_OK) return rc;
+  return ptc_wgrad_reduce_jobs(jobs, n, stream);
 }
 
 int ptc_spconv_wgrad_deferred(const void* in, int64_t n_in, const void* dout, const int32_t* nbr, int64_t n_out, int kv, int c_in, int c_out,
-                              int dtype, float* dw, float* dbias, void* workspace, size_t workspace_bytes, ptc_stream_t stream,
-                              PtcWgradJob* job) {
+                              int dtype, float* dw, float* dbias, void* workspace, size_t workspace_bytes, uint32_t* counters,
+                              ptc_stream_t stream, PtcWgradJob* job) {
   PTC_REQUIRE(job != nullptr, PTC_EINVAL, "ptc_spconv_wgrad_deferred: null job");
   *job = PtcWgradJob{nullptr, 0, 0, nullptr, nullptr, 0, nullptr};
-  return spconv_wgrad_impl(in, n_in, dout, nbr, n_out, kv, c_in, c_out, dtype, dw, dbias, workspace, workspace_bytes, stream, job);
+  return spconv_wgrad_impl(in, n_in, dout, nbr, n_out, kv, c_in, c_out, dtype, dw, dbias, workspace, workspace_bytes, counters, stream, job);
 }
 
 int ptc_spconv_wgrad_blk_deferred(const void* in, int64_t n_in, const void* dout, const int32_t* nbr, const void* tab, const int32_t* hid,
                                   const int32_t* hcnt, const int32_t* n_overflow, int bm, int hcap, int64_t n_out, int kv, int c_in, int c_out,
-                                  int dtype, float* dw, void* workspace, size_t workspace_bytes, ptc_stream_t stream, PtcWgradJob* job) {
+                                  int dtype, float* dw, void* workspace, size_t workspace_bytes, uint32_t* counters, ptc_stream_t stream,
+                                  PtcWgradJob* job) {
   PTC_REQUIRE(job != nullptr, PTC_EINVAL, "ptc_spconv_wgrad_blk: null job");
   *job = PtcWgradJob{nullptr, 0, 0, nullptr, nullptr, 0, nullptr};
   const bool buf_ok = (uint64_t)n_in * c_in * 2 <= PTC_BUF_MAX_BYTES && (uint64_t)n_out * c_out * 2 <= PTC_BUF_MAX_BYTES;
   if (!buf_ok || !tab || !hid || !hcnt || !n_overflow || !nbr || n_in != n_out || !wgrad7_supported(dtype, kv, c_in, c_out, bm, hcap, n_out))
-    return spconv_wgrad_impl(in, n_in, dout, nbr, n_out, kv, c_in, c_out, dtype, dw, nullptr, workspace, workspace_bytes, stream, job);
+    return spconv_wgrad_impl(in, n_in, dout, nbr, n_out, kv, c_in, c_out, dtype, dw, nullptr, workspace, workspace_bytes, counters, stream, job);
   PTC_REQUIRE(in && dout && dw && workspace, PTC_EINVAL, "ptc_spconv_wgrad_blk: null buffer");
-  PTC_REQUIRE(workspace_bytes >= ptc_spconv_wgrad_blk_workspace_bytes(n_out, kv, c_in, c_out), PTC_EWORKSPACE, "ptc_spconv_wgrad_blk: workspace too small");
+  PTC_REQUIRE(workspace_bytes >= ptc_spconv_wgrad_blk_body_bytes(n_out, kv, c_in, c_out), PTC_EWORKSPACE, "ptc_spconv_wgrad_blk: workspace too small");
   PTC_REQUIRE(((uintptr_t)in % 16 == 0) && ((uintptr_t)dout % 16 == 0) && ((uintptr_t)tab % 16 == 0), PTC_EINVAL,
               "ptc_spconv_wgrad_blk: buffers must be 16-byte aligned");
   hipStream_t s = (hipStream_t)stream;
-  float* p7 = (float*)((char*)workspace + ptc_spconv_wgrad_workspace_bytes(n_out, kv, c_in, c_out));
+  float* p7 = (float*)((char*)workspace + ptc_spconv_wgrad_body_bytes(n_out, kv, c_in, c_out));
   int rc = ptc_wgrad7_launch(dtype, in, dout, (const uint16_t*)tab, hid, hcnt, n_overflow, n_out, c_in, c_out, p7, s);
   if (rc != PTC_OK) return rc;
   PtcWgradJob j2;
@@ -798,19 +836,23 @@
                                     const int32_t* hcnt, const int32_t* n_overflow, int bm, int hcap, int64_t n_out, int kv, int c_in, int c_out,
                                     int dtype, float* dw, void* workspace, size_t workspace_bytes, ptc_stream_t stream) {
   PtcWgradJob job;
-  const int rc = ptc_spconv_wgrad_blk_deferred(in, n_in, dout, nbr, tab, hid, hcnt, n_overflow, bm, hcap, n_out, kv, c_in, c_out, dtype, dw, workspace,
-                                               workspace_bytes, stream, &job);
+  PTC_REQUIRE(workspace, PTC_EINVAL, "ptc_spconv_wgrad_blk: null buffer");
+  PTC_REQUIRE(workspace_bytes >= PTC_WGRAD_HDR_BYTES, PTC_EWORKSPACE, "ptc_spconv_wgrad_blk: workspace too small");
+  const int rc = ptc_spconv_wgrad_blk_deferred(in, n_in, dout, nbr, tab, hid, hcnt, n_overflow, bm, hcap, n_out, kv, c_in, c_out, dtype, dw,
+                                               (char*)workspace + PTC_WGRAD_HDR_BYTES, workspace_bytes - PTC_WGRAD_HDR_BYTES, (uint32_t*)workspace,
+                                               stream, &job);
   if (rc != PTC_OK) return rc;
   return ptc_wgrad_reduce_jobs(&job, 1, stream);
 }
 
 static int spconv_wgrad_impl(const void* in, int64_t n_in, const void* dout, const int32_t* nbr, int64_t n_out, int kv, int c_in, int c_out,
-                             int dtype, float* dw, float* dbias, void* workspace, size_t workspace_bytes, ptc_stream_t stream, PtcWgradJob* defer) {
+                             int dtype, float* dw, float* dbias, void* workspace, size_t workspace_bytes, uint32_t* counters, ptc_stream_t stream,
+                             PtcWgradJob* defer) {
   PTC_REQUIRE(n_in >= 0 && n_out >= 0 && kv >= 1, PTC_EINVAL, "ptc_spconv_wgrad: bad sizes");
   PTC_REQUIRE(c_in >= 8 && c_in % 8 == 0 && c_out >= 8 && c_out % 8 == 0, PTC_EUNSUPPORTED,
               "ptc_spconv_wgrad: c_in=%d c_out=%d must be multiples of 8", c_in, c_out);
   PTC_REQUIRE(dw && workspace, PTC_EINVAL, "ptc_spconv_wgrad: null buffer");
-  PTC_REQUIRE(workspace_bytes >= ptc_spconv_wgrad_workspace_bytes(n_out, kv, c_in, c_out), PTC_EWORKSPACE,
+  PTC_REQUIRE(workspace_bytes >= ptc_spconv_wgrad_body_bytes(n_out, kv, c_in, c_out), PTC_EWORKSPACE,
               "ptc_spconv_wgrad: workspace too small");
   hipStream_t s = (hipStream_t)stream;
   if (n_out == 0) {
@@ -826,10 +868,11 @@
     g3.n = 0;
     for (int k = 0; k <= W3_MAX; ++k) g3.start[k] = 0;
     PtcWgradJob job;
-    wgrad3_add(g3, in, n_in, dout, nbr, n_out, c_in, c_out, dw, dbias, workspace, &job);
+    wgrad3_add(g3, in, n_in, dout, nbr, n_out, c_in, c_out, dw, dbias, workspace, counters, &job);
     const int rc = ptc_wgrad3_launch(dtype, g3, s);
     if (rc != PTC_OK) return rc;
     if (defer) { *defer = job; return PTC_OK; }
+    if (job.splits == 0) return PTC_OK;
     return launch_wgrad_reduce(job.partial, job.splits, job.count, dw, job.bias_partial, c_out, dbias, s);
   }
   if (dtype == PTC_BF16 && buf_ok) return launch_wgrad2<bf16_t>(in, n_in, dout, nbr, n_out, kv, c_in, c_out, dw, dbias, workspace, s, defer);
diff --git a/pointcept_amd/csrc/spconv_internal.h b/pointcept_amd/csrc/spconv_internal.h
--- a/pointcept_amd/csrc/spconv_internal.h
+++ b/pointcept_amd/csrc/spconv_internal.h
@@ -14,15 +14,22 @@
   int alt_splits = 0;
 };
 
+#define PTC_WGRAD_CNT_BYTES 4096
+#define PTC_WGRAD_HDR_BYTES (8 * PTC_WGRAD_CNT_BYTES)
+size_t ptc_spconv_wgrad_body_bytes(int64_t n_out, int kv, int c_in, int c_out);
+size_t ptc_spconv_wgrad_blk_body_bytes(int64_t n_out, int kv, int c_in, int c_out);
+
 int ptc_spconv_wgrad_deferred(const void* in, int64_t n_in, const void* dout, const int32_t* nbr, int64_t n_out, int kv, int c_in, int c_out,
-                              int dtype, float* dw, float* dbias, void* workspace, size_t workspace_bytes, ptc_stream_t stream,
-                              PtcWgradJob* job);
+                              int dtype, float* dw, float* dbias, void* workspace, size_t workspace_bytes, uint32_t* counters,
+                              ptc_stream_t stream, PtcWgradJob* job);
 int ptc_spconv_wgrad_blk_deferred(const void* in, int64_t n_in, const void* dout, const int32_t* nbr, const void* tab, const int32_t* hid,
                                   const int32_t* hcnt, const int32_t* n_overflow, int bm, int hcap, int64_t n_out, int kv, int c_in, int c_out,
-                                  int dtype, float* dw, void* workspace, size_t workspace_bytes, ptc_stream_t stream, PtcWgradJob* job);
+                                  int dtype, float* dw, void* workspace, size_t workspace_bytes, uint32_t* counters, ptc_stream_t stream,
+                                  PtcWgradJob* job);
 struct PtcWgradCall {
   const void* in; int64_t n_in; const void* dout; const int32_t* nbr; int64_t n_out; int kv, c_in, c_out, dtype;
   float* dw; float* dbias; void* workspace; size_t workspace_bytes;
+  uint32_t* counters;
 };
 int ptc_spconv_wgrad_group(const PtcWgradCall* calls, int n, PtcWgradJob* jobs, ptc_stream_t stream);
 #define PTC_WGRAD_JOBS_MAX 8
diff --git a/pointcept_amd/csrc/wgrad3.h b/pointcept_amd/csrc/wgrad3.h
--- a/pointcept_amd/csrc/wgrad3.h
+++ b/pointcept_amd/csrc/wgrad3.h
@@ -5,15 +5,20 @@
 #ifndef W3_TARGET
 #define W3_TARGET 96
 #endif
+#define W3_MAX_SPLITS 64
+#define W3_REDUCE_FEW 8
+#define W3_CNT_TILES 1024
 struct W3Problem {
   const void* in; const void* dout; const int32_t* nbr; int64_t n_out; int c_in, c_out;
   float* partial; float* bias_partial;
   int splits, cps, tiles, tiles_i;
   uint32_t in_bytes, dout_bytes;
+  uint32_t* cnt; float* dw; float* dbias;
 };
 struct W3Group { int n; int start[W3_MAX + 1]; W3Problem p[W3_MAX]; };
 
 bool ptc_wgrad3_supported(int dtype, int kv, int c_in, int c_out, int64_t n_out);
+bool ptc_wgrad3_fused();
 void ptc_wgrad3_plan(int64_t n_out, int c_in, int c_out, int* splits, int* cps);
 int ptc_wgrad3_launch(int dtype, const W3Group& g, hipStream_t s);
 
@@ -23,6 +28,70 @@
 #define W3_IMG (8 * W2_PLANE)
 #define W3_STAGE (4 * W3_IMG)
 #define W3_LDS_BYTES (2 * W3_STAGE)
+
+__device__ __forceinline__ void w3_sum_few(const float* __restrict__ src, int64_t count, int64_t jstep, int splits, float* __restrict__ dst) {
+#pragma unroll 1
+  for (int jb = 0; jb < 16; jb += 4) {
+    float4 v[W3_REDUCE_FEW][4];
+#pragma unroll
+    for (int p = 0; p < W3_REDUCE_FEW; ++p)
+      if (p < splits) {
+#pragma unroll
+        for (int j = 0; j < 4; ++j) v[p][j] = *reinterpret_cast<const float4*>(src + (int64_t)p * count + (jb + j) * jstep);
+      }
+#pragma unroll
+    for (int j = 0; j < 4; ++j) {
+      float4 a = v[0][j];
+#pragma unroll
+      for (int p = 1; p < W3_REDUCE_FEW; ++p)
+        if (p < splits) { a.x += v[p][j].x; a.y += v[p][j].y; a.z += v[p][j].z; a.w += v[p][j].w; }
+      *reinterpret_cast<float4*>(dst + (jb + j) * jstep) = a;
+    }
+  }
+}
+template <int U, int Q>
+__device__ __forceinline__ void w3_sum_tree(const float* __restrict__ src, int64_t count, int64_t jstep, int splits, float* __restrict__ dst) {
+#pragma unroll 1
+  for (int jb = 0; jb < 16; jb += 4) {
+    float4 r[4];
+#pragma unroll 1
+    for (int pb = 0; pb < 16; pb += Q) {
+      float4 v[Q][U][4];
+#pragma unroll
+      for (int q = 0; q < Q; ++q)
+#pragma unroll
+        for (int u = 0; u < U; ++u) {
+          const int p = pb + q + 16 * u;
+#pragma unroll
+          for (int j = 0; j < 4; ++j) v[q][u][j] = make_float4(0.f, 0.f, 0.f, 0.f);
+          if (p < splits) {
+#pragma unroll
+            for (int j = 0; j < 4; ++j) v[q][u][j] = *reinterpret_cast<const float4*>(src + (int64_t)p * count + (jb + j) * jstep);
+          }
+        }
+#pragma unroll
+      for (int q = 0; q < Q; ++q)
+#pragma unroll
+        for (int j = 0; j < 4; ++j) {
+          float4 a[4];
+#pragma unroll
+          for (int u = 0; u < 4; ++u) {
+            a[u] = make_float4(0.f, 0.f, 0.f, 0.f);
+            if (u < U) { a[u].x += v[q][u < U ? u : 0][j].x; a[u].y += v[q][u < U ? u : 0][j].y; a[u].z += v[q][u < U ? u : 0][j].z; a[u].w += v[q][u < U ? u : 0][j].w; }
+          }
+          float4 t;
+          t.x = (a[0].x + a[1].x) + (a[2].x + a[3].x);
+          t.y = (a[0].y + a[1].y) + (a[2].y + a[3].y);
+          t.z = (a[0].z + a[1].z) + (a[2].z + a[3].z);
+          t.w = (a[0].w + a[1].w) + (a[2].w + a[3].w);
+          if (pb + q == 0) r[j] = t;
+          else { r[j].x += t.x; r[j].y += t.y; r[j].z += t.z; r[j].w += t.w; }
+        }
+    }
+#pragma unroll
+    for (int j = 0; j < 4; ++j) *reinterpret_cast<float4*>(dst + (jb + j) * jstep) = r[j];
+  }
+}
 
 template <typename T>
 __global__ void __launch_bounds__(256) PTC_WAVES_PER_EU(2, 2)
@@ -166,6 +235,50 @@
 #pragma unroll
       for (int e = 0; e < 4; ++e) bp[16 * t + e] = accb[t][e];
   }
+  if (P.cnt == nullptr) return;
+
+  __threadfence();
+  __syncthreads();
+  int* const last_flag = reinterpret_cast<int*>(smem);
+  if (threadIdx.x == 0) {
+    __threadfence();
+    const unsigned arrived = atomicAdd(P.cnt + tile, 1u) + 1u;
+    const int last = arrived == (unsigned)P.splits;
+    if (last) atomicExch(P.cnt + tile, 0u);
+    *last_flag = last;
+  }
+  __syncthreads();
+  if (*last_flag == 0) return;
+  __threadfence();
+  const int splits = P.splits;
+  const int64_t count = (int64_t)c_out * c_in;
+  const int col4 = threadIdx.x & 31, row0 = threadIdx.x >> 5;
+  const int64_t base = (int64_t)(to * 128 + row0) * c_in + ti * 128 + col4 * 4;
+  const float* __restrict__ src = P.partial + base;
+  float* __restrict__ dst = P.dw + base;
+  const int64_t jstep = (int64_t)8 * c_in;
+  if (splits <= W3_REDUCE_FEW) w3_sum_few(src, count, jstep, splits, dst);
+  else if (splits <= 16) w3_sum_tree<1, 8>(src, count, jstep, splits, dst);
+  else if (splits <= 32) w3_sum_tree<2, 4>(src, count, jstep, splits, dst);
+  else if (splits <= 48) w3_sum_tree<3, 2>(src, count, jstep, splits, dst);
+  else w3_sum_tree<4, 2>(src, count, jstep, splits, dst);
+  if (P.dbias != nullptr && ti == 0 && threadIdx.x < 128) {
+    const int co = to * 128 + threadIdx.x;
+    float rsum = 0.f;
+#pragma unroll 1
+    for (int pg = 0; pg < 16; ++pg) {
+      float a[4];
+#pragma unroll
+      for (int u = 0; u < 4; ++u) {
+        const int p = pg + 16 * u;
+        a[u] = 0.f;
+        if (p < splits) a[u] += P.bias_partial[(int64_t)p * c_out + co];
+      }
+      const float tsum = (a[0] + a[1]) + (a[2] + a[3]);
+      rsum = pg == 0 ? tsum : rsum + tsum;
+    }
+    P.dbias[co] = rsum;
+  }
 }
 
 static inline bool wgrad3_enabled() {
@@ -175,19 +288,39 @@
 bool ptc_wgrad3_supported(int dtype, int kv, int c_in, int c_out, int64_t n_out) {
   return wgrad3_enabled() && dtype != PTC_F32 && kv == 1 && c_in >= 128 && c_in % 128 == 0 && c_out % 128 == 0 && n_out >= 1;
 }
+static int w3_env_int(const char* name, int dflt) {
+  const char* e = getenv(name);
+  return e && e[0] ? atoi(e) : dflt;
+}
+static int w3_dflt_fused() { static const int v = w3_env_int("PTC_WGRAD3_FUSED", 1) != 0; return v; }
+static int w3_dflt_target() { static const int v = [] { const int t = w3_env_int("PTC_WGRAD3_TARGET", W3_TARGET); return t >= 1 ? t : W3_TARGET; }(); return v; }
+static int w3_fused = -1, w3_target = -1, w3_min_chunks = -1;
+extern "C" int ptc_wgrad3_tune(int fused, int target, int min_chunks) {
+  w3_fused = fused < 0 ? -1 : (fused != 0);
+  w3_target = target < 1 ? -1 : target;
+  w3_min_chunks = min_chunks < 1 ? -1 : min_chunks;
+  return PTC_OK;
+}
+bool ptc_wgrad3_fused() { return (w3_fused < 0 ? w3_dflt_fused() : w3_fused) != 0; }
 void ptc_wgrad3_plan(int64_t n_out, int c_in, int c_out, int* splits, int* cps) {
   const int64_t n_chunks = (n_out + 63) >> 6;
   const int tiles = (c_in / 128) * (c_out / 128);
-  int64_t s = (W3_TARGET + tiles - 1) / tiles;
+  const int target = w3_target < 0 ? w3_dflt_target() : w3_target, min_chunks = w3_min_chunks < 0 ? 4 : w3_min_chunks;
+  int64_t s = (target + tiles - 1) / tiles;
   const int64_t min_s = (n_chunks + 127) / 128;
   if (s < min_s) s = min_s;
-  if (s > 64) s = 64;
-  const int64_t max_s = (n_chunks + 3) / 4;
+  if (s > W3_MAX_SPLITS) s = W3_MAX_SPLITS;
+  const int64_t max_s = (n_chunks + min_chunks - 1) / min_chunks;
   if (s > max_s) s = max_s;
   if (s < 1) s = 1;
   const int64_t c = (n_chunks + s - 1) / s;
   *cps = (int)c;
   *splits = (int)((n_chunks + c - 1) / c);
+}
+extern "C" int ptc_wgrad3_splits(int64_t n_out, int c_in, int c_out) {
+  int splits = 0, cps = 0;
+  if (n_out >= 1 && c_in >= 128 && c_in % 128 == 0 && c_out >= 128 && c_out % 128 == 0) ptc_wgrad3_plan(n_out, c_in, c_out, &splits, &cps);
+  return splits;
 }
 
 int ptc_wgrad3_launch(int dtype, const W3Group& g, hipStream_t s) {
diff --git a/pointcept_amd/functional.py b/pointcept_amd/functional.py
--- a/pointcept_amd/functional.py
+++ b/pointcept_amd/functional.py
@@ -878,7 +878,7 @@
         if plan["ws"] is None:
             plan["ws"] = int(ops.lib().ptc_ptv3_block_workspace_bytes(n, npad, c, heads))
         nbytes = plan["ws"]
-        ws = torch.empty(nbytes, dtype=torch.uint8, device=dev)
+        ws = ops._ws_counted(nbytes, dev)
         _lib.check(ops.lib().ptc_ptv3_block_bwd(iv, fv, pin, psv, pg, ws.data_ptr(), nbytes, ops.stream_ptr()), "ptc_ptv3_block_bwd")
         dx0 = (gscr if x0.dtype == torch.float32 else sbuf)[plan["gx0"]:plan["gx0"] + n * c].view(n, c)
         dxc = sbuf[plan["gxc"]:plan["gxc"] + n * c].view(n, c)
diff --git a/pointcept_amd/ops.py b/pointcept_amd/ops.py
--- a/pointcept_amd/ops.py
+++ b/pointcept_amd/ops.py
@@ -1,6 +1,7 @@
 from __future__ import annotations
 
 import ctypes
+import threading
 from typing import Optional, Sequence
 
 import torch
@@ -11,6 +12,17 @@
 
 def _ws(nbytes: int, device) -> torch.Tensor:
     return torch.empty(max(int(nbytes), 1), dtype=torch.uint8, device=device)
+
+
+_ws_kept = {}
+
+
+def _ws_counted(nbytes: int, device) -> torch.Tensor:
+    key = (str(device), stream_ptr(), threading.get_ident())
+    ws = _ws_kept.get(key)
+    if ws is None or ws.numel() < nbytes:
+        ws = _ws_kept[key] = torch.zeros(max(int(nbytes), 1), dtype=torch.uint8, device=device)
+    return ws
 
 
 def serialize_encode(grid_coord: torch.Tensor, batch: Optional[torch.Tensor], depth: int,
@@ -543,17 +555,38 @@
         if blk.nbr.data_ptr() != nbr.data_ptr() or tuple(blk.nbr.shape) != tuple(nbr.shape):
             raise PtcoreError("blk was built from another gather table")
         nbytes = lib().ptc_spconv_wgrad_blk_workspace_bytes(n_out, kv, c_in, c_out)
-        ws = _ws(nbytes, feat.device)
+        ws = _ws_counted(nbytes, feat.device)
         check(lib().ptc_spconv_wgrad_blk(ptr(feat), feat.shape[0], ptr(dout), ptr(nbr), ptr(blk.tab), ptr(blk.hid), ptr(blk.hcnt),
                                          ptr(blk.n_overflow), blk.bm, blk.hcap, n_out, kv, c_in, c_out, dtype_code(feat), ptr(dw), ptr(ws),
                                          nbytes, stream_ptr()), "ptc_spconv_wgrad_blk")
         return dw
     db = torch.empty(c_out, dtype=torch.float32, device=feat.device) if want_bias else None
     nbytes = lib().ptc_spconv_wgrad_workspace_bytes(n_out, kv, c_in, c_out)
-    ws = _ws(nbytes, feat.device)
+    ws = _ws_counted(nbytes, feat.device)
     check(lib().ptc_spconv_wgrad(ptr(feat), feat.shape[0], ptr(dout), ptr(nbr), n_out, kv, c_in, c_out,
                                  dtype_code(feat), ptr(dw), ptr(db), ptr(ws), nbytes, stream_ptr()), "ptc_spconv_wgrad")
     return (dw, db) if want_bias else dw
+
+
+def linear_wgrad_group(feats: Sequence[torch.Tensor], douts: Sequence[torch.Tensor]):
+    require_cuda(*feats, *douts)
+    k = len(feats)
+    feats = [f.contiguous() for f in feats]
+    douts = [d.contiguous() for d in douts]
+    rows = feats[0].shape[0]
+    if any(f.shape[0] != rows or d.shape[0] != rows or f.dtype != feats[0].dtype or d.dtype != feats[0].dtype for f, d in zip(feats, douts)):
+        raise PtcoreError("linear_wgrad_group: every operand needs the same rows and dtype")
+    dev = feats[0].device
+    dws = [torch.empty((d.shape[1], 1, f.shape[1]), dtype=torch.float32, device=dev) for f, d in zip(feats, douts)]
+    dbs = [torch.empty(d.shape[1], dtype=torch.float32, device=dev) for d in douts]
+    ci = (ctypes.c_int * k)(*[f.shape[1] for f in feats])
+    co = (ctypes.c_int * k)(*[d.shape[1] for d in douts])
+    pa = lambda ts: ctypes.cast((ctypes.c_void_p * k)(*[ptr(t) for t in ts]), ctypes.c_void_p)
+    nbytes = lib().ptc_linear_wgrad_group_workspace_bytes(k, rows, ctypes.cast(ci, ctypes.c_void_p), ctypes.cast(co, ctypes.c_void_p))
+    ws = _ws_counted(nbytes, dev)
+    check(lib().ptc_linear_wgrad_group(k, rows, pa(feats), pa(douts), ctypes.cast(ci, ctypes.c_void_p), ctypes.cast(co, ctypes.c_void_p),
+                                       dtype_code(feats[0]), pa(dws), pa(dbs), ptr(ws), nbytes, stream_ptr()), "ptc_linear_wgrad_group")
+    return list(zip(dws, dbs))
 
 
 def seg_eval_hist(logits: Optional[torch.Tensor], target: torch.Tensor, k: int, ignore_index: int = -1,
```
